# ucuapps/OpenGlue

Hardware: AMD Instinct MI355X
Metric: image-pairs/sec (1024 kpts, 256-dim, 9 GNN layers) (higher is better)
Workload: dtype f32; 1 GPU; BASELINE configs[1]: 1024x1024 kpts, 256-dim, 9 self+cross stages, 4 heads, 100 Sinkhorn iters, batch=32 pairs/GPU, random-init weights, seeded synthetic keypoints/descriptors; global_batch=32, pairs_per_gpu=32, parallelism=pairs sharded over 1 GPU(s), 1 RCCL gather

## Files before the change

include/openglue_amd.h:

```cpp
#ifndef OPENGLUE_AMD_H
#define OPENGLUE_AMD_H

#include <stddef.h>
#include <stdint.h>

#ifdef __cplusplus
extern "C" {
#endif

#define OG_ABI_VERSION 14

#define OG_E_INVALID   (-1)
#define OG_E_SHAPE     (-2)
#define OG_E_ALIGN     (-3)
#define OG_E_FLAG      (-4)
#define OG_E_RANGE     (-5)

#define OG_FLAG_RESIDUAL        1
#define OG_FLAG_USE_OFFSET      2
#define OG_FLAG_NO_DESCRIPTORS  4
#define OG_FLAG_LINEAR_ATTENTION 16
#define OG_FLAG_FAVOR_RELU      32
#define OG_FLAG_SIREN_ENCODER   8

// ... 79 lines not shown
    int64_t enc_w[OG_MAX_HIDDEN + 1], enc_b[OG_MAX_HIDDEN + 1];
    int64_t layer0, layer_stride, o_wqkv, o_bqkv, o_w0, o_b0, o_w3, o_b3;
    int64_t wp, bp, alpha, dustbin, total;
    int64_t o_scale;
    int64_t scales;
    int64_t o_wmlp;
    int64_t o_wqkvs;
    int64_t o_wqkvb;
} og_packed_layout_t;
int og_packed_layout(const og_shape* shape, og_packed_layout_t* layout);

int og_forward(const og_shape* shape, const og_inputs* in, const void* packed_dev,
               void* workspace_dev, const og_outputs* out, void* stream);

int og_forward_tap(const og_shape* shape, const og_inputs* in, const void* packed_dev, void* workspace_dev,
                   const og_outputs* out, void* stream, int32_t tap, float* tap_x);

int og_keypoint_encoder(const og_shape* shape, const og_inputs* in, const void* packed_dev, void* workspace_dev, float* x_out, void* stream);
int og_scores(const float* g0, const float* g1, int32_t batch, int32_t m, int32_t n, int32_t D, float* S, int64_t lds, void* stream);

#define OG_MAX_RAGGED 64
int og_forward_ragged(const og_shape* shape, const int32_t* lens0, const int32_t* lens1, const float* image0_wh,
                      const float* image1_wh, const og_inputs* in, const void* packed_dev, void* workspace_dev,
                      const og_outputs* out, void* stream);

#define OG_STAGE_ENCODER_INPUT 0
#define OG_STAGE_GEMM          1
#define OG_STAGE_ATTENTION     2
#define OG_STAGE_SINKHORN      3
#define OG_STAGE_MATCHES       4
#define OG_STAGE_GEMM_F16X3    5
#define OG_STAGE_MLP_FUSED     6
#define OG_NUM_STAGES          7
int og_forward_profiled(const og_shape* shape, const og_inputs* in, const void* packed_dev,
                        void* workspace_dev, const og_outputs* out, void* stream,
                        float* stage_ms , int32_t* stage_launches );
int og_forward_ragged_profiled(const og_shape* shape, const int32_t* lens0, const int32_t* lens1, const float* image0_wh,
                               const float* image1_wh, const og_inputs* in, const void* packed_dev, void* workspace_dev,
                               const og_outputs* out, void* stream, float* stage_ms, int32_t* stage_launches);


int og_gemm_nt(const float* A, int64_t lda, int64_t strideA, const float* B, int64_t ldb, int64_t strideB,
               float* C, int64_t ldc, int64_t strideC, int32_t M, int32_t N, int32_t K, int32_t batch,
               const float* bias, int32_t relu, const float* res, int64_t ldr, const float* alpha,
               float scale, void* stream);

int og_gemm_kmajor(const float* A, int64_t lda, int64_t strideA, int32_t a_kmajor, const float* B, int64_t ldb, int64_t strideB,
                   float* C, int64_t ldc, int64_t strideC, int32_t M, int32_t N, int32_t K, int32_t batch, int32_t k_total,
                   int32_t a_colsum, float scale, void* stream);

int og_split_f16(const float* x, int64_t n, void* hi, void* lo, void* stream);
int og_split_f16_hl(const float* x, int64_t rows, int32_t cols, int64_t ldx, void* out, int64_t ldo, void* stream);

int og_gemm_nt_f16x3(const void* A, int64_t lda, const void* B, int64_t ldb, int32_t M, int32_t N, int32_t K,
                     float scale, const float* bias, int32_t relu, const float* res, int64_t ldr, float* C32, int64_t ldc,
                     void* Ch, void* Cl, int64_t ldch, int32_t c_hl, void* stream);
int og_gemm_nt_f16x3_reshl(const void* A, int64_t lda, const void* B, int64_t ldb, int32_t M, int32_t N, int32_t K,
                           float scale, const float* bias, int32_t relu, const void* res_hl, int64_t ldrh, float* C32, int64_t ldc,
                           void* Ch, void* Cl, int64_t ldch, int32_t c_hl, void* stream);

size_t og_proj_block_stream_bytes(int32_t N, int32_t K);
int og_proj_block_pack(int32_t N, int32_t K, const float* W, void* stream_host);
int og_proj_block(const void* x_rows, int64_t ld, int32_t M, int32_t K, int32_t N, const void* stream_dev, const float* bias, const float* inv_scale_dev,
                  void* yh, void* yl, int64_t ldy, int32_t split_row, int32_t a0, int32_t a1, int32_t b0, int32_t b1, void* stream);

size_t og_mlp_block_stream_bytes(int32_t D);
int og_mlp_block_pack(int32_t D, const float* W0, const float* W3, void* stream_host);
int og_mlp_block(int32_t D, void* xo_rows, int64_t ld, int32_t M, const void* stream_dev, const float* b0, const float* b3,
                 void* stream);

int og_attention(const void* qh, const void* ql, int64_t ldq, const void* kh, const void* kl, int64_t ldk,
                 const void* vh, const void* vl, int64_t ldv, void* oh, void* ol, int64_t ldo, int32_t batch,
                 int32_t nq, int32_t nk, int32_t num_heads, int32_t dh, float* lse, void* stream);

size_t og_sinkhorn_workspace_bytes(int32_t batch, int32_t m, int32_t n);
int og_sinkhorn(const float* S, int64_t lds, float dustbin, int32_t batch, int32_t m, int32_t n,
                int32_t iters, float reg, float* scores, void* workspace_dev, void* stream);

int og_sinkhorn_status(const void* sinkhorn_workspace_dev, int32_t batch, int32_t m, int32_t n);
int og_sinkhorn_schedule(int32_t batch, int32_t m, int32_t n, int32_t iters);
int og_sinkhorn_schedule_ragged(int32_t batch, const int32_t* lens0, const int32_t* lens1, int32_t iters);
int og_sinkhorn_resident_geometry(int32_t m, int32_t n, int32_t* out4);
int og_sinkhorn_resident_rows_per_wave(int32_t batch, int32_t m, int32_t n);
int og_sinkhorn_resident_ragged_footprint(int32_t batch, const int32_t* lens0, const int32_t* lens1, int64_t* out2);
int og_forward_status(const og_shape* shape, const void* workspace_dev);

size_t og_sinkhorn_train_workspace_bytes(int32_t batch, int32_t m, int32_t n, int32_t iters);
int og_sinkhorn_train_forward(const float* S, int64_t lds, float dustbin, const float* dustbin_dev, int32_t batch, int32_t m, int32_t n,
                              int32_t iters, float reg, float* scores, void* train_workspace_dev, void* stream);
int og_sinkhorn_backward(const float* S, int64_t lds, float dustbin, const float* dustbin_dev, int32_t batch, int32_t m, int32_t n, int32_t iters,
                         float reg, const float* grad_scores, void* train_workspace_dev, float* dS, int64_t ldds,
                         float* d_dustbin, void* stream);

size_t og_batchnorm_train_workspace_bytes(int64_t rows, int32_t channels);
int og_batchnorm_train_forward(const float* x, int64_t ldx, int64_t rows, int32_t channels, const float* weight,
                               const float* bias, float eps, float momentum, float* running_mean, float* running_var,
                               float* y, int64_t ldy, float* save_mean, float* save_invstd, void* workspace_dev,
                               void* stream);

int og_batchnorm_train_backward(const float* a, int64_t lda, const float* dy, int64_t lddy, int64_t rows, int32_t channels,
                                const float* weight, const float* save_mean, const float* save_invstd, int32_t relu_mask,
                                float* dz, int64_t lddz, float* dweight, float* dbias, void* workspace_dev, void* stream);
int og_transpose_f32(const float* src, int64_t ld_src, int64_t rows, int32_t cols, float* dst, int64_t ld_dst, void* stream);
int og_colsum_f32(const float* x, int64_t ldx, int64_t rows, int32_t channels, float* out, void* workspace_dev, void* stream);

int og_transpose_f32_batched(const float* src, int64_t ld_src, int64_t stride_src, int64_t rows, int32_t cols, float* dst,
                             int64_t ld_dst, int64_t stride_dst, int32_t batch, void* stream);
int og_softmax_rows(float* S, int64_t ld, int64_t rows, int32_t cols, void* stream);
int og_softmax_rows_backward(const float* P, float* dP, int64_t ld, int64_t rows, int32_t cols, float scale, void* stream);

int og_attention_train_lse(const float* q, const float* k, int32_t batch, int32_t nq, int32_t nk, int32_t num_heads, int32_t dh,
                           float scale, float* lse, void* stream);
int og_attention_backward_parts(int32_t nk);
int og_attention_backward(const float* q, const float* k, const float* v, const float* dout, const float* lse, const float* delta,
                          int32_t batch, int32_t nq, int32_t nk, int32_t num_heads, int32_t dh, float scale, float* dq_part, float* dk,
                          float* dv, void* stream);
int og_attention_backward_ld(const float* q, int64_t ldq, const float* k, int64_t ldk, const float* v, int64_t ldv, const float* dout,
                             const float* lse, const float* delta, int32_t batch, int32_t nq, int32_t nk, int32_t num_heads, int32_t dh,
                             float scale, float* dq_part, float* dk, int64_t lddk, float* dv, int64_t lddv, void* stream);
int og_attention_delta(const float* dout, const float* out, int64_t rows, int32_t num_heads, int32_t dh, float* delta, void* stream);
int og_split_f16_rows(const float* x, int64_t ldx, int64_t rows, int32_t cols, int32_t scale_cols, float s1, float s2, void* hi, void* lo,
                      int64_t ldo, void* stream);
int og_merge_f16(const void* hi, const void* lo, int64_t n, float* out, void* stream);
int og_splitk_reduce(const float* part, int32_t parts, int32_t rows, int64_t ld, int32_t cols, float* dW, float* db, void* stream);

size_t og_matches_workspace_bytes(int32_t batch, int32_t m, int32_t n);
int og_extract_matches(const float* scores, int32_t batch, int32_t m, int32_t n, float match_threshold,
                       int64_t* matches0, float* matching_scores0, int64_t* matches1,
                       float* matching_scores1, void* workspace_dev, void* stream);


int og_prepare_features(const float* lafs, const float* responses, int64_t tokens, int32_t method, int32_t log_response,
                        float* keypoints, float* side_info, void* stream);

size_t og_compact_workspace_bytes(int32_t batch, int32_t m);
int og_compact_matches(const int64_t* matches0, const float* matching_scores0, const float* lafs0, const float* lafs1,
                       int32_t batch, int32_t m, int32_t n, int64_t* matching_idxs, int64_t* batch_indexes,
                       float* confidence, float* mlafs0, float* mlafs1, float* keypoints0, float* keypoints1,
                       int32_t* count_dev, void* workspace_dev, void* stream);


size_t og_gt_matches_workspace_bytes(int32_t batch, int32_t m, int32_t n);
int og_gt_matches(int32_t batch, int32_t m, int32_t n, const float* keypoints0, const float* keypoints1, int32_t transform,
                  const float* H, const float* K0, const float* K1, const float* R, const float* T,
                  const float* depth0, int32_t depth0_h, int32_t depth0_w, const float* depth1, int32_t depth1_h, int32_t depth1_w,
                  int32_t apply_thresholds, double positive_threshold, double negative_threshold,
                  int64_t* gt_matches0, int64_t* gt_matches1, int32_t* status_dev, void* workspace_dev, void* stream);

size_t og_criterion_workspace_bytes(int32_t batch, int32_t m, int32_t n, int32_t with_margin);
int og_criterion_forward(const float* scores, const int64_t* gt_matches0, const int64_t* gt_matches1,
                         const float* context_descriptors0, const float* context_descriptors1,
                         int32_t batch, int32_t m, int32_t n, int32_t D, int32_t with_margin, float margin,
                         float* losses, void* workspace_dev, void* stream);
int og_criterion_backward(const int64_t* gt_matches0, const int64_t* gt_matches1,
                          const float* context_descriptors0, const float* context_descriptors1,
                          int32_t batch, int32_t m, int32_t n, int32_t D, int32_t with_margin, float margin,
                          const float* grad_losses, const void* workspace_dev, float* grad_scores,
                          float* grad_context_descriptors0, float* grad_context_descriptors1, void* stream);

int og_epipolar_precision(int32_t batch, int32_t m, int32_t n, const float* keypoints0, const float* keypoints1,
                          const int64_t* matches0, const int32_t* num_keypoints0, const float* K0, const float* K1,
                          const float* R, const float* T, double threshold, float* precision, float* matching_score,
                          int32_t* num_correct, void* stream);
int og_essential_5pt(int32_t count, const double* x0, const double* x1, double* E, int32_t* num_solutions, void* stream);
size_t og_relative_pose_workspace_bytes(int32_t batch, int32_t m, int32_t hypotheses);
int og_relative_pose(int32_t batch, int32_t m, int32_t n, const float* keypoints0, const float* keypoints1,
                     const int64_t* matches0, const int32_t* num_keypoints0, const float* K0, const float* K1,
                     const float* R, const float* T, float ransac_threshold, int32_t hypotheses, uint64_t seed,
                     int64_t pair_offset, float* error, float* R_pred, float* t_pred, uint8_t* inliers,
                     int32_t* num_inliers, void* workspace_dev, void* stream);

int og_fundamental_7pt(int32_t count, const double* x0, const double* x1, double* F, int32_t* num_solutions, void* stream);
size_t og_fundamental_matrix_workspace_bytes(int32_t batch, int32_t m, int32_t hypotheses);
int og_fundamental_matrix(int32_t batch, int32_t m, int32_t n, const float* keypoints0, const float* keypoints1,
                          const int64_t* matches0, const int32_t* num_keypoints0, float threshold, int32_t hypotheses,
                          int32_t refine, uint64_t seed, int64_t pair_offset, double* F, uint8_t* inliers,
                          int32_t* num_inliers, int32_t* best_model, void* workspace_dev, void* stream);

size_t og_superpoint_packed_bytes(int32_t descriptor_dim);
int og_superpoint_pack(int32_t descriptor_dim, int32_t batch_norm, float bn_eps, const float* const* params, void* packed_host);
int og_superpoint_capacity(int32_t H, int32_t W, int32_t max_kpts);
size_t og_superpoint_workspace_bytes(int32_t batch, int32_t H, int32_t W, int32_t nms_kernel, int32_t max_kpts);
int og_superpoint_dense(int32_t batch, int32_t H, int32_t W, const float* image, const void* packed_dev, float* heatmap,
                        float* coarse_desc, void* workspace_dev, void* stream);
int og_superpoint_detect(int32_t batch, int32_t Hh, int32_t Wh, int32_t nms_kernel, int32_t border, float threshold, int32_t max_kpts,
                         const float* heatmap, int32_t* counts, int32_t* sel_idx, float* sel_score, int64_t sel_ld,
                         void* workspace_dev, void* stream);
int og_superpoint_describe(int32_t batch, int32_t Hc, int32_t Wc, int32_t n, const int32_t* sel_idx, const float* sel_score,
                           int64_t sel_ld, const float* coarse_desc, float* lafs, float* scores, float* descriptors, void* stream);

#define OG_ADAM_CHUNK         4096
#define OG_ADAM_NORM_CHUNK    8192
#define OG_ADAM_SCALARS       8
#define OG_ADAM_TOTAL_NORM    0
#define OG_ADAM_CLIP_COEF     1
#define OG_ADAM_STEP          2
#define OG_ADAM_LR            3
#define OG_ADAM_STEP_SIZE     4
#define OG_ADAM_INV_SQRT_BC2  5
typedef struct og_adam_layout_t {
    int64_t total;
    int64_t table_bytes;
    int64_t workspace_bytes;
    int32_t num_chunks;
    int32_t num_partials;
    int32_t chunk;
    int32_t reserved;
} og_adam_layout_t;
int og_adam_layout(int32_t count, const int64_t* numel, int64_t* offsets, int32_t* chunk_map, og_adam_layout_t* layout);
int og_adam_step(int32_t count, const void* const* params, const void* table_dev, const int32_t* chunk_map_dev, int32_t num_chunks,
                 int64_t total, float* grad, float* exp_avg, float* exp_avg_sq, double* workspace_dev, double lr, double gamma,
                 double beta1, double beta2, double eps, int32_t clip, double max_norm, void* stream);
// ... 30 lines not shown
```

openglue_amd/_lib.py:

```python
from __future__ import annotations

import ctypes as C
import os
from typing import Optional, Tuple

import torch

HERE = os.path.dirname(os.path.abspath(__file__))
LIB_PATH = os.environ.get("OPENGLUE_AMD_LIB") or os.path.join(HERE, "lib", "libopenglue_amd.so")

OG_ABI_VERSION = 14
OG_FLAG_RESIDUAL, OG_FLAG_USE_OFFSET, OG_FLAG_NO_DESCRIPTORS, OG_FLAG_SIREN_ENCODER, OG_FLAG_LINEAR_ATTENTION = 1, 2, 4, 8, 16
OG_FLAG_FAVOR_RELU = 32
OG_MAX_HIDDEN = 8
OG_MAX_RAGGED = 64
OG_ADAM_CHUNK, OG_ADAM_NORM_CHUNK, OG_ADAM_SCALARS = 4096, 8192, 8
OG_ADAM_TOTAL_NORM, OG_ADAM_CLIP_COEF, OG_ADAM_STEP, OG_ADAM_LR, OG_ADAM_STEP_SIZE, OG_ADAM_INV_SQRT_BC2 = range(6)
OG_STAGES = ("encoder_input", "gemm_f32", "attention", "sinkhorn", "matches", "gemm_f16x3", "mlp_fused")

_ERRORS = {-1: "OG_E_INVALID (null pointer / bad size)", -2: "OG_E_SHAPE (unsupported shape)",
           -3: "OG_E_ALIGN (pointer or leading dimension not 16-byte aligned)", -4: "OG_E_FLAG (unknown flag)",
           -5: "OG_E_RANGE (a folded weight is not finite)"}

c_float_p = C.POINTER(C.c_float)
# ... 21 lines not shown


class og_params(C.Structure):
    _fields_ = [("enc_conv", og_conv * (OG_MAX_HIDDEN + 1)), ("enc_bn", og_bn * OG_MAX_HIDDEN),
                ("layers", C.POINTER(og_layer_params)), ("linear_proj", og_conv), ("mix_coefs", C.c_void_p),
                ("dustbin_score", C.c_float)]


class og_inputs(C.Structure):
    _fields_ = [("keypoints0", C.c_void_p), ("keypoints1", C.c_void_p), ("descriptors0", C.c_void_p),
                ("descriptors1", C.c_void_p), ("side_info0", C.c_void_p), ("side_info1", C.c_void_p),
                ("image0_wh", C.c_float * 2), ("image1_wh", C.c_float * 2)]


class og_outputs(C.Structure):
    _fields_ = [("scores", C.c_void_p), ("context_descriptors0", C.c_void_p), ("context_descriptors1", C.c_void_p),
                ("matches0", C.c_void_p), ("matching_scores0", C.c_void_p), ("matches1", C.c_void_p),
                ("matching_scores1", C.c_void_p)]


class og_packed_layout_t(C.Structure):
    _fields_ = [("n_enc", C.c_int32), ("enc_k", C.c_int32 * (OG_MAX_HIDDEN + 1)), ("enc_out", C.c_int32 * (OG_MAX_HIDDEN + 1)),
                ("enc_w", C.c_int64 * (OG_MAX_HIDDEN + 1)), ("enc_b", C.c_int64 * (OG_MAX_HIDDEN + 1))] + \
               [(k, C.c_int64) for k in ("layer0", "layer_stride", "o_wqkv", "o_bqkv", "o_w0", "o_b0", "o_w3", "o_b3",
                                         "wp", "bp", "alpha", "dustbin", "total", "o_scale", "scales", "o_wmlp", "o_wqkvs", "o_wqkvb")]


class og_adam_layout_t(C.Structure):
    _fields_ = [("total", C.c_int64), ("table_bytes", C.c_int64), ("workspace_bytes", C.c_int64), ("num_chunks", C.c_int32),
                ("num_partials", C.c_int32), ("chunk", C.c_int32), ("reserved", C.c_int32)]


_i32, _i64, _f, _vp, _sz = C.c_int32, C.c_int64, C.c_float, C.c_void_p, C.c_size_t
SYMBOLS = {
    "og_abi_version": (C.c_int, []),
    "og_check_shape": (C.c_int, [C.POINTER(og_shape)]),
    "og_packed_weights_bytes": (_sz, [C.POINTER(og_shape)]),
    "og_workspace_bytes": (_sz, [C.POINTER(og_shape)]),
    "og_packed_layout": (C.c_int, [C.POINTER(og_shape), C.POINTER(og_packed_layout_t)]),
    "og_pack_weights": (C.c_int, [C.POINTER(og_shape), C.POINTER(og_params), _vp]),
    "og_forward": (C.c_int, [C.POINTER(og_shape), C.POINTER(og_inputs), _vp, _vp, C.POINTER(og_outputs), _vp]),
    "og_forward_tap": (C.c_int, [C.POINTER(og_shape), C.POINTER(og_inputs), _vp, _vp, C.POINTER(og_outputs), _vp, _i32, _vp]),
    "og_forward_ragged": (C.c_int, [C.POINTER(og_shape), C.POINTER(C.c_int32), C.POINTER(C.c_int32), C.POINTER(C.c_float),
                                    C.POINTER(C.c_float), C.POINTER(og_inputs), _vp, _vp, C.POINTER(og_outputs), _vp]),
    "og_forward_profiled": (C.c_int, [C.POINTER(og_shape), C.POINTER(og_inputs), _vp, _vp, C.POINTER(og_outputs), _vp,
                                      C.POINTER(C.c_float), C.POINTER(C.c_int32)]),
    "og_forward_ragged_profiled": (C.c_int, [C.POINTER(og_shape), C.POINTER(C.c_int32), C.POINTER(C.c_int32), C.POINTER(C.c_float),
                                             C.POINTER(C.c_float), C.POINTER(og_inputs), _vp, _vp, C.POINTER(og_outputs), _vp,
                                             C.POINTER(C.c_float), C.POINTER(C.c_int32)]),
    "og_gemm_nt": (C.c_int, [_vp, _i64, _i64, _vp, _i64, _i64, _vp, _i64, _i64, _i32, _i32, _i32, _i32, _vp, _i32,
                             _vp, _i64, _vp, _f, _vp]),
    "og_gemm_kmajor": (C.c_int, [_vp, _i64, _i64, _i32, _vp, _i64, _i64, _vp, _i64, _i64, _i32, _i32, _i32, _i32, _i32, _i32, _f, _vp]),
    "og_attention_train_lse": (C.c_int, [_vp, _vp, _i32, _i32, _i32, _i32, _i32, _f, _vp, _vp]),
    "og_attention_backward_parts": (C.c_int, [_i32]),
    "og_attention_backward": (C.c_int, [_vp, _vp, _vp, _vp, _vp, _vp, _i32, _i32, _i32, _i32, _i32, _f, _vp, _vp, _vp, _vp]),
    "og_attention_backward_ld": (C.c_int, [_vp, _i64, _vp, _i64, _vp, _i64, _vp, _vp, _vp, _i32, _i32, _i32, _i32, _i32, _f, _vp, _vp, _i64, _vp, _i64, _vp]),
    "og_attention_delta": (C.c_int, [_vp, _vp, _i64, _i32, _i32, _vp, _vp]),
    "og_split_f16_rows": (C.c_int, [_vp, _i64, _i64, _i32, _i32, _f, _f, _vp, _vp, _i64, _vp]),
    "og_merge_f16": (C.c_int, [_vp, _vp, _i64, _vp, _vp]),
    "og_splitk_reduce": (C.c_int, [_vp, _i32, _i32, _i64, _i32, _vp, _vp, _vp]),
    "og_split_f16": (C.c_int, [_vp, _i64, _vp, _vp, _vp]),
    "og_split_f16_hl": (C.c_int, [_vp, _i64, _i32, _i64, _vp, _i64, _vp]),
    "og_gemm_nt_f16x3": (C.c_int, [_vp, _i64, _vp, _i64, _i32, _i32, _i32, _f, _vp, _i32, _vp, _i64, _vp, _i64,
                                   _vp, _vp, _i64, _i32, _vp]),
    "og_gemm_nt_f16x3_reshl": (C.c_int, [_vp, _i64, _vp, _i64, _i32, _i32, _i32, _f, _vp, _i32, _vp, _i64, _vp, _i64,
                                         _vp, _vp, _i64, _i32, _vp]),
    "og_proj_block_stream_bytes": (_sz, [_i32, _i32]),
    "og_proj_block_pack": (C.c_int, [_i32, _i32, _vp, _vp]),
    "og_proj_block": (C.c_int, [_vp, _i64, _i32, _i32, _i32, _vp, _vp, _vp, _vp, _vp, _i64, _i32, _i32, _i32, _i32, _i32, _vp]),
    "og_mlp_block_stream_bytes": (_sz, [_i32]),
    "og_mlp_block_pack": (C.c_int, [_i32, _vp, _vp, _vp]),
    "og_mlp_block": (C.c_int, [_i32, _vp, _i64, _i32, _vp, _vp, _vp, _vp]),
    "og_attention": (C.c_int, [_vp, _vp, _i64, _vp, _vp, _i64, _vp, _vp, _i64, _vp, _vp, _i64, _i32, _i32, _i32, _i32,
                               _i32, _vp, _vp]),
    "og_keypoint_encoder": (C.c_int, [_vp, _vp, _vp, _vp, _vp, _vp]),
    "og_scores": (C.c_int, [_vp, _vp, _i32, _i32, _i32, _i32, _vp, _i64, _vp]),
    "og_sinkhorn_workspace_bytes": (_sz, [_i32, _i32, _i32]),
    "og_sinkhorn_status": (C.c_int, [_vp, _i32, _i32, _i32]),
    "og_sinkhorn_schedule": (C.c_int, [_i32, _i32, _i32, _i32]),
    "og_sinkhorn_schedule_ragged": (C.c_int, [_i32, _vp, _vp, _i32]),
    "og_sinkhorn_resident_geometry": (C.c_int, [_i32, _i32, _vp]),
    "og_sinkhorn_resident_ragged_footprint": (C.c_int, [_i32, _vp, _vp, _vp]),
    "og_sinkhorn_resident_rows_per_wave": (C.c_int, [_i32, _i32, _i32]),
    "og_forward_status": (C.c_int, [_vp, _vp]),
    "og_sinkhorn_train_workspace_bytes": (_sz, [_i32, _i32, _i32, _i32]),
    "og_sinkhorn_train_forward": (C.c_int, [_vp, _i64, _f, _vp, _i32, _i32, _i32, _i32, _f, _vp, _vp, _vp]),
    "og_sinkhorn_backward": (C.c_int, [_vp, _i64, _f, _vp, _i32, _i32, _i32, _i32, _f, _vp, _vp, _vp, _i64, _vp, _vp]),
    "og_batchnorm_train_workspace_bytes": (_sz, [_i64, _i32]),
    "og_batchnorm_train_forward": (C.c_int, [_vp, _i64, _i64, _i32, _vp, _vp, _f, _f, _vp, _vp, _vp, _i64, _vp, _vp, _vp, _vp]),
    "og_batchnorm_train_backward": (C.c_int, [_vp, _i64, _vp, _i64, _i64, _i32, _vp, _vp, _vp, _i32, _vp, _i64, _vp, _vp, _vp, _vp]),
    "og_transpose_f32": (C.c_int, [_vp, _i64, _i64, _i32, _vp, _i64, _vp]),
    "og_colsum_f32": (C.c_int, [_vp, _i64, _i64, _i32, _vp, _vp, _vp]),
    "og_transpose_f32_batched": (C.c_int, [_vp, _i64, _i64, _i64, _i32, _vp, _i64, _i64, _i32, _vp]),
    "og_softmax_rows": (C.c_int, [_vp, _i64, _i64, _i32, _vp]),
    "og_softmax_rows_backward": (C.c_int, [_vp, _vp, _i64, _i64, _i32, _f, _vp]),
    "og_sinkhorn": (C.c_int, [_vp, _i64, _f, _i32, _i32, _i32, _i32, _f, _vp, _vp, _vp]),
    "og_matches_workspace_bytes": (_sz, [_i32, _i32, _i32]),
    "og_prepare_features": (C.c_int, [_vp, _vp, _i64, _i32, _i32, _vp, _vp, _vp]),
    "og_compact_workspace_bytes": (_sz, [_i32, _i32]),
    "og_compact_matches": (C.c_int, [_vp, _vp, _vp, _vp, _i32, _i32, _i32, _vp, _vp, _vp, _vp, _vp, _vp, _vp, _vp, _vp, _vp]),
    "og_extract_matches": (C.c_int, [_vp, _i32, _i32, _i32, _f, _vp, _vp, _vp, _vp, _vp, _vp]),
    "og_gt_matches_workspace_bytes": (_sz, [_i32, _i32, _i32]),
    "og_gt_matches": (C.c_int, [_i32, _i32, _i32, _vp, _vp, _i32, _vp, _vp, _vp, _vp, _vp, _vp, _i32, _i32, _vp, _i32, _i32,
                                _i32, C.c_double, C.c_double, _vp, _vp, _vp, _vp, _vp]),
    "og_criterion_workspace_bytes": (_sz, [_i32, _i32, _i32, _i32]),
    "og_criterion_forward": (C.c_int, [_vp, _vp, _vp, _vp, _vp, _i32, _i32, _i32, _i32, _i32, _f, _vp, _vp, _vp]),
    "og_criterion_backward": (C.c_int, [_vp, _vp, _vp, _vp, _i32, _i32, _i32, _i32, _i32, _f, _vp, _vp, _vp, _vp, _vp, _vp]),
    "og_epipolar_precision": (C.c_int, [_i32, _i32, _i32, _vp, _vp, _vp, _vp, _vp, _vp, _vp, _vp, C.c_double, _vp, _vp, _vp, _vp]),
    "og_essential_5pt": (C.c_int, [_i32, _vp, _vp, _vp, _vp, _vp]),
    "og_relative_pose_workspace_bytes": (_sz, [_i32, _i32, _i32]),
    "og_relative_pose": (C.c_int, [_i32, _i32, _i32, _vp, _vp, _vp, _vp, _vp, _vp, _vp, _vp, _f, _i32, C.c_uint64, _i64,
                                   _vp, _vp, _vp, _vp, _vp, _vp, _vp]),
    "og_fundamental_7pt": (C.c_int, [_i32, _vp, _vp, _vp, _vp, _vp]),
    "og_fundamental_matrix_workspace_bytes": (_sz, [_i32, _i32, _i32]),
    "og_fundamental_matrix": (C.c_int, [_i32, _i32, _i32, _vp, _vp, _vp, _vp, _f, _i32, _i32, C.c_uint64, _i64,
                                        _vp, _vp, _vp, _vp, _vp, _vp]),
    "og_superpoint_packed_bytes": (_sz, [_i32]),
    "og_superpoint_pack": (C.c_int, [_i32, _i32, _f, _vp, _vp]),
    "og_superpoint_capacity": (C.c_int, [_i32, _i32, _i32]),
    "og_superpoint_workspace_bytes": (_sz, [_i32, _i32, _i32, _i32, _i32]),
    "og_superpoint_dense": (C.c_int, [_i32, _i32, _i32, _vp, _vp, _vp, _vp, _vp, _vp]),
    "og_superpoint_detect": (C.c_int, [_i32, _i32, _i32, _i32, _i32, _f, _i32, _vp, _vp, _vp, _vp, _i64, _vp, _vp]),
    "og_superpoint_describe": (C.c_int, [_i32, _i32, _i32, _i32, _vp, _vp, _i64, _vp, _vp, _vp, _vp, _vp]),
    "og_sift_geometry": (C.c_int, [_i32, _i32, C.POINTER(C.c_int32)]),
    "og_sift_workspace_bytes": (_sz, [_i32, _i32, _i32]),
    "og_sift_pyramid": (C.c_int, [_i32, _i32, _i32, _vp, _vp, _vp, _vp, _vp]),
    "og_sift_detect": (C.c_int, [_i32, _i32, _i32, _vp, _vp, _vp, _vp, _vp, _vp]),
    "og_sift_orient": (C.c_int, [_i32, _i32, _i32, _i32, _vp, _vp, _vp, _vp, _vp, _vp, _vp, _vp]),
    "og_sift_describe": (C.c_int, [_i32, _i32, _i32, _i32, _i32, _vp, _vp, _vp, _vp, _vp, _vp]),
    "og_sift_select": (C.c_int, [_i32, _i32, _i32, _f, _i32, _vp, _vp, _vp, _vp, _vp, _vp]),
    "og_sift_gather": (C.c_int, [_i32, _i32, _i32, _i32, _vp, _vp, _vp, _vp, _vp, _vp, _vp]),
    "og_patch_geometry": (C.c_int, [_i32, _i32, C.POINTER(C.c_int32)]),
    "og_patch_workspace_bytes": (_sz, [_i32, _i32, _i32, _i32]),
    "og_patch_pyramid": (C.c_int, [_i32, _i32, _i32, _vp, _vp, _vp, _vp]),
    "og_patch_extract": (C.c_int, [_i32, _i32, _i32, _i32, _vp, _vp, _i32, _i32, _vp, _vp]),
    "og_patchnet_packed_bytes": (_sz, [_i32]),
    "og_patchnet_pack": (C.c_int, [_i32, _f, _vp, _vp]),
    "og_patchnet_forward": (C.c_int, [_i32, _i32, _vp, _i32, _vp, _vp, _vp, _vp, _vp]),
    "og_adam_layout": (C.c_int, [_i32, C.POINTER(C.c_int64), C.POINTER(C.c_int64), C.POINTER(C.c_int32), C.POINTER(og_adam_layout_t)]),
    "og_adam_step": (C.c_int, [_i32, C.POINTER(C.c_void_p), _vp, _vp, _i32, _i64, _vp, _vp, _vp, _vp, C.c_double, C.c_double, C.c_double,
                               C.c_double, C.c_double, _i32, C.c_double, _vp]),
}

_lib: Optional[C.CDLL] = None


def load() -> C.CDLL:
    global _lib
    if _lib is not None:
        return _lib
    if not os.path.exists(LIB_PATH):
        raise RuntimeError(
            f"{LIB_PATH} not found: build it with `python -m openglue_amd.build` "
            "(hipcc --offload-arch=gfx950).  openglue_amd has no CPU / eager fallback.")
    lib = C.CDLL(LIB_PATH)
    for name, (restype, argtypes) in SYMBOLS.items():
        fn = getattr(lib, name)
        fn.restype, fn.argtypes = restype, argtypes
    if lib.og_abi_version() != OG_ABI_VERSION:
        raise RuntimeError(f"libopenglue_amd ABI {lib.og_abi_version()} != binding {OG_ABI_VERSION}; rebuild")
    _lib = lib
    return lib


def check(rc: int, what: str) -> None:
    if rc == 0:
        return
    if rc < 0:
        raise RuntimeError(f"{what}: {_ERRORS.get(rc, rc)}")
    raise RuntimeError(f"{what}: HIP error {rc} at kernel launch")


STREAM = object()


def call(name: str, dev: torch.device, *args) -> None:
    fn = getattr(load(), name)
    with torch.cuda.device(dev):
        stream = torch.cuda.current_stream(dev).cuda_stream
# ... 22 lines not shown
```

openglue_amd/csrc/api.hip:

```cpp
#include <math.h>
#include <cmath>
#include <stdlib.h>
#include <string.h>
#include <vector>
#include <dlfcn.h>
#include <stdio.h>

#include "og_common.h"

namespace {

constexpr double BN_EPS = 1e-5;

struct PackedLayout {
    int n_enc;
    int enc_k[OG_MAX_HIDDEN + 1];
    int enc_out[OG_MAX_HIDDEN + 1];
    int64_t enc_w[OG_MAX_HIDDEN + 1], enc_b[OG_MAX_HIDDEN + 1];
    int64_t enc_whl;
    int64_t layer0, layer_stride;
    int64_t o_wqkv, o_bqkv, o_w0, o_b0, o_w3, o_b3;
    int64_t o_wmlp;
    int64_t o_wqkvs;
    int64_t o_wqkvb;
// ... 368 lines not shown
    }
};
struct Range {
    static const Roctx& rt() { static const Roctx r; return r; }
    bool on;
    explicit Range(const char* name) : on(rt().push != nullptr) { if (on) rt().push(name); }
    Range(const char* name, int idx) : on(rt().push != nullptr) {
        if (on) { char buf[48]; snprintf(buf, sizeof buf, "%s %d", name, idx); rt().push(buf); }
    }
    ~Range() { if (on) rt().pop(); }
    Range(const Range&) = delete;
};
struct Scope {
    Profiler* p; int i;
    Scope(Profiler* pp, int c) : p(pp), i(pp ? pp->begin(c) : -1) {}
    ~Scope() { if (p) p->end(i); }
};

int forward_impl(const og_shape* shape, const og_inputs* in, const void* packed_dev, void* workspace_dev,
                 const og_outputs* outp, void* stream, Profiler* prof, const RaggedDesc* rag = nullptr,
                 const EncoderRagged* er0 = nullptr, const EncoderRagged* er1 = nullptr, int tap = -1, float* tap_x = nullptr,
                 bool encoder_only = false) {
    static const og_outputs no_outputs{};
    if (encoder_only && !outp) outp = &no_outputs;
    if (!shape || !in || !packed_dev || !workspace_dev || !outp) return OG_E_INVALID;
    if (int e = check_shape(shape)) return e;
    og_clear_status();
    const og_shape& s = *shape;
    if (!in->keypoints0 || !in->keypoints1 || !in->descriptors0 || !in->descriptors1 || (!outp->scores && !encoder_only)) return OG_E_INVALID;
    if (s.side_info > 0 && (!in->side_info0 || !in->side_info1)) return OG_E_INVALID;
    if ((outp->matches0 == nullptr) != (outp->matching_scores0 == nullptr)) return OG_E_INVALID;
    if ((outp->matches1 == nullptr) != (outp->matching_scores1 == nullptr)) return OG_E_INVALID;
    if (outp->matches1 && !outp->matches0) return OG_E_INVALID;
    if (((uintptr_t)packed_dev & 15) || ((uintptr_t)workspace_dev & 15) || ((uintptr_t)in->descriptors0 & 15) ||
        ((uintptr_t)in->descriptors1 & 15))
        return OG_E_ALIGN;
    hipStream_t st = (hipStream_t)stream;
    const PackedLayout L = packed_layout(s);
    const WorkspaceLayout W = workspace_layout(s);
    const float* pk = (const float*)packed_dev;
    float* ws = (float*)workspace_dev;
    const int D = s.desc_dim, D2 = 2 * D, B = s.batch, m = s.m, n = s.n;
    const bool favor = s.flags & OG_FLAG_FAVOR_RELU;
    const int WQ = qk_width(s), QW = qkv_width(s);
    const int64_t T0 = rag ? rag->off0[B] : (int64_t)B * m, T1 = rag ? rag->off1[B] : (int64_t)B * n, T = T0 + T1;
    float* X32 = ws + W.x32; float* G = ws + W.g; float* Sb = ws + W.sbuf;
    const int D4 = 4 * D;
    _Float16* XO = (_Float16*)(ws + W.xo);
    _Float16* QKVh = (_Float16*)(ws + W.qkvh); _Float16* QKVl = (_Float16*)(ws + W.qkvl);
    _Float16* Hb = (_Float16*)(ws + W.h);
    int rc;

    auto gemm = [&](const float* A, int64_t lda, const float* Bm, int64_t ldb, float* C, int64_t ldc, int64_t M, int N, int K,
                    const float* bias, int relu, const float* res, int64_t ldr, _Float16* Chl, int64_t ldch) -> int {
        GemmArgs g{};
        g.A = A; g.lda = lda; g.strideA = 0; g.B = Bm; g.ldb = ldb; g.strideB = 0; g.C = C; g.ldc = ldc; g.strideC = 0;
        g.M = (int)M; g.N = N; g.K = K; g.batch = 1; g.bias = bias; g.relu = relu; g.res = res; g.ldr = ldr; g.strideR = 0;
        g.alpha = nullptr; g.scale = 1.f; g.Ct = nullptr; g.ldct = 0; g.strideCt = 0; g.ct_rows = 1;
        g.Ch = Chl; g.Cl = Chl ? Chl + 32 : nullptr; g.ldch = ldch; g.c_hl = 1;
        Scope sc(prof, OG_STAGE_GEMM);
        return og_launch_gemm(g, st);
    };
    auto gemmh = [&](const _Float16* A, const float* wbase, int64_t o_w, int64_t wrow0, int64_t M, int N, int K,
                     const float* bias, int relu, const _Float16* res_hl, float* C32, _Float16* Ch, _Float16* Cl, int64_t ldch,
                     int c_hl) -> int {
        GemmHArgs g{};
        g.scale_dev = wbase + L.o_scale + (o_w == L.o_wqkv ? 0 : o_w == L.o_w0 ? 1 : 2);
        g.A = A; g.lda = D4;
        g.B = (const _Float16*)(wbase + o_w) + wrow0 * 2 * K; g.ldb = 2 * K;
        g.M = (int)M; g.N = N; g.K = K; g.scale = (float)(1.0 / OG_W_SCALE); g.bias = bias; g.relu = relu; g.res = nullptr; g.ldr = D; g.res_hl = res_hl; g.ldrh = D4;
        g.C32 = C32; g.ldc = D; g.Ch = Ch; g.Cl = Cl; g.ldch = ldch; g.c_hl = c_hl;
        Scope sc(prof, OG_STAGE_GEMM_F16X3);
        return og_launch_gemm_f16x3(g, st);
    };

    Range r_forward("og_forward");
    {
        Range r_stage("encoder");
        float* EI = ws + W.ei;
        float* Ea = ws + W.ea;
        float* Eb = ws + W.eb;
        {
            Scope sc(prof, OG_STAGE_ENCODER_INPUT);
            if ((rc = og_launch_encoder_input(in->keypoints0, in->side_info0, T0, s.side_info, in->image0_wh[0], in->image0_wh[1], EI, st, er0))) return rc;
            if ((rc = og_launch_encoder_input(in->keypoints1, in->side_info1, T1, s.side_info, in->image1_wh[0], in->image1_wh[1], EI + T0 * 32, st, er1))) return rc;
        }
        const float* cur = EI; int64_t ldcur = 32;
        const bool tail_f16 = L.enc_whl >= 0;
        const int last = L.n_enc - 1;
        _Float16* Ehl = (_Float16*)G;
        for (int i = 0; i < L.n_enc; ++i) {
            const float* Wi = pk + L.enc_w[i]; const float* bi = pk + L.enc_b[i];
            if (i < last) {
                float* dst = (i & 1) ? Eb : Ea;
                const int act = (s.flags & OG_FLAG_SIREN_ENCODER) ? 2 : 1;
                const bool to_hl = tail_f16 && i == last - 1;
                if ((rc = gemm(cur, ldcur, Wi, L.enc_k[i], to_hl ? nullptr : dst, L.enc_maxw, T, L.enc_out[i], L.enc_k[i], bi, act, nullptr, 0,
                               to_hl ? Ehl : nullptr, to_hl ? 2 * L.enc_out[i] : 0))) return rc;
                cur = dst; ldcur = L.enc_maxw;
            } else {
                const bool nd = s.flags & OG_FLAG_NO_DESCRIPTORS;
                const float* res[2] = {nd ? nullptr : in->descriptors0, nd ? nullptr : in->descriptors1};
                const int64_t r0[2] = {0, T0}, R[2] = {T0, T1};
                for (int side = 0; side < 2; ++side) {
                    if (tail_f16) {
                        const int K = L.enc_k[i];
                        GemmHArgs g{};
                        g.A = Ehl + r0[side] * 2 * K; g.lda = 2 * K;
                        g.B = (const _Float16*)(pk + L.enc_whl); g.ldb = 2 * K;
                        g.M = (int)R[side]; g.N = D; g.K = K; g.scale = (float)(1.0 / OG_W_SCALE); g.scale_dev = pk + L.scales + 1; g.bias = bi; g.relu = 0;
                        g.res = res[side]; g.ldr = D; g.res_hl = nullptr; g.ldrh = 0;
                        g.C32 = nullptr; g.ldc = D; g.Ch = XO + r0[side] * D4; g.Cl = g.Ch + 32; g.ldch = D4; g.c_hl = 1;
                        Scope sc(prof, OG_STAGE_GEMM_F16X3);
                        if ((rc = og_launch_gemm_f16x3(g, st))) return rc;
                    } else {
                        if ((rc = gemm(cur + r0[side] * ldcur, ldcur, Wi, L.enc_k[i], X32 + r0[side] * D, D, R[side], D, L.enc_k[i], bi, 0, res[side], D,
                                       XO + r0[side] * D4, D4))) return rc;
                    }
                }
            }
        }
    }

    auto tap_here = [&](int idx) -> int {
        if (tap != idx || !tap_x) return 0;
        return og_launch_merge_f16_hl(XO, T, D, D4, tap_x, D, st);
    };
    if ((rc = tap_here(0))) return rc;
    if (encoder_only) return og_launch_status();

    const int dh = D / s.num_heads;
    if (hipMemsetAsync(ws + W.attn, 0, OG_ATTN_COUNTERS * sizeof(int), st) != hipSuccess) return OG_E_INVALID;
    auto attention = [&](int nz, int split, int64_t qb0, int64_t qs0, int nq0, int64_t kb0, int64_t ks0, int nk0,
                         int64_t qb1, int64_t qs1, int nq1, int64_t kb1, int64_t ks1, int nk1, int rag_mode) -> int {
        AttnArgs a{};
        a.rag = rag; a.rag_mode = rag_mode;
        a.qh = QKVh; a.ql = QKVl; a.ldq = QW; a.kh = QKVh + WQ; a.kl = QKVl + WQ; a.ldk = QW;
        a.vh = QKVh + 2 * WQ; a.vl = QKVl + 2 * WQ; a.ldv = QW;
        a.feat = favor ? WQ : 0;
        a.oh = XO + D2; a.ol = XO + D2 + 32; a.ldo = D4; a.o_hl = 1;
        a.nz = nz; a.num_heads = s.num_heads; a.dh = dh; a.split = split;
        a.counters = reinterpret_cast<int*>(ws + W.attn); a.partial = ws + W.attn + OG_ATTN_COUNTERS;
        a.q_base[0] = qb0; a.q_step[0] = qs0; a.nq[0] = nq0; a.kv_base[0] = kb0; a.kv_step[0] = ks0; a.nk[0] = nk0;
        a.q_base[1] = qb1; a.q_step[1] = qs1; a.nq[1] = nq1; a.kv_base[1] = kb1; a.kv_step[1] = ks1; a.nk[1] = nk1;
        Scope sc(prof, OG_STAGE_ATTENTION);
        if (favor) return og_launch_favor_attention(a, st);
        return (s.flags & OG_FLAG_LINEAR_ATTENTION) ? og_launch_linear_attention(a, st) : og_launch_attention(a, st);
    };
    auto proj_small_ok = [&](int64_t R) {
        static const int mode = [] { const char* e = getenv("OG_PROJ_SMALL"); return e ? atoi(e) : -1; }();
        return L.o_wqkvs >= 0 && !favor && (mode >= 0 ? mode != 0 : R <= 8192) && R < ((int64_t)1 << 30);
    };
    auto proj_small = [&](const float* lw, int64_t r0, int64_t R, int split_row, int a0, int a1, int b0, int b1) -> int {
        Scope sc(prof, OG_STAGE_GEMM_F16X3);
        return og_launch_proj_small(XO + r0 * D4, D4, (int)R, D, (const char*)(lw + L.o_wqkvs), lw + L.o_bqkv, lw + L.o_scale,
                                    QKVh + r0 * QW, QKVl + r0 * QW, QW, split_row, a0, a1, b0, b1, st);
    };
    auto proj_stream_ok = [&](int64_t R, bool full = false) {
        return L.o_wqkvb >= 0 && !favor && og_proj_stream_wanted((int)(R < ((int64_t)1 << 30) ? R : 0), D, full) && R < ((int64_t)1 << 30) && QW % 64 == 0 &&
               !(((uintptr_t)QKVh | (uintptr_t)QKVl) & 127);
    };
    auto proj_stream = [&](const float* lw, int64_t r0, int64_t R, int split_row, int a0, int a1, int b0, int b1) -> int {
        Scope sc(prof, OG_STAGE_GEMM_F16X3);
        return og_launch_proj_stream(XO + r0 * D4, D4, (int)R, D, (const char*)(lw + L.o_wqkvb), lw + L.o_bqkv, lw + L.o_scale,
                                     QKVh + r0 * QW, QKVl + r0 * QW, QW, split_row, a0 / 128, a1 / 128, b0 / 128, b1 / 128, st);
    };
    auto qkv_proj = [&](const float* lw, int64_t r0, int64_t R, int c0, int c1) -> int {
        if (proj_small_ok(R) && c0 % 32 == 0 && c1 % 32 == 0) return proj_small(lw, r0, R, 0, 0, 0, c0 / 32, c1 / 32);
        if (proj_stream_ok(R, c0 == 0 && c1 == QW) && c0 % 128 == 0 && c1 % 128 == 0 && ((r0 * QW * 2) % 128 == 0)) return proj_stream(lw, r0, R, 0, 0, 0, c0, c1);
        const int cut = favor ? 2 * WQ : c1;
        const int ca[2] = {c0, c0 < cut && cut < c1 ? cut : c1}, cb[2] = {ca[1], c1};
        for (int part = 0; part < 2; ++part) {
            const int a0 = part ? cb[0] : ca[0], a1 = part ? cb[1] : ca[1];
            if (a1 <= a0) continue;
            const int relu = favor && a0 < 2 * WQ;
            if (int e = gemmh(XO + r0 * D4, lw, L.o_wqkv, a0, R, a1 - a0, D, lw + L.o_bqkv + a0, relu, nullptr, nullptr, QKVh + r0 * QW + a0,
                              QKVl + r0 * QW + a0, QW, 0)) return e;
        }
        return 0;
    };
    const bool fused_mlp = og_mlp_fused_enabled(D) && L.o_wmlp >= 0;
    auto mlp = [&](const float* lw, int64_t r0, int64_t R) -> int {
        if (fused_mlp) {
            MlpFusedArgs a{};
            a.XO = XO + r0 * D4; a.ld = D4; a.M = (int)R; a.wstream = (const char*)(lw + L.o_wmlp);
            a.b0 = lw + L.o_b0; a.b3 = lw + L.o_b3; a.scale = (float)(1.0 / OG_W_SCALE); a.scales_dev = lw + L.o_scale + 1;
            Scope sc(prof, OG_STAGE_MLP_FUSED);
            return og_launch_mlp_fused(a, D, st);
        }
        int e = gemmh(XO + r0 * D4, lw, L.o_w0, 0, R, D2, D2, lw + L.o_b0, 1, nullptr, nullptr, Hb + r0 * D4, nullptr, D4, 1);
        if (e) return e;
        return gemmh(Hb + r0 * D4, lw, L.o_w3, 0, R, D, D2, lw + L.o_b3, 0, XO + r0 * D4, nullptr, XO + r0 * D4, nullptr, D4, 1);
    };
    for (int l = 0; l < s.num_stages; ++l) {
        const float* lw = pk + L.layer0 + (int64_t)(2 * l) * L.layer_stride;
        {
            Range r_stage("gnn self", l);
            if ((rc = qkv_proj(lw, 0, T, 0, QW))) return rc;
            if ((rc = attention(2 * B, B, 0, m, m, 0, m, m, T0, n, n, T0, n, n, 1))) return rc;
            if ((rc = mlp(lw, 0, T))) return rc;
        }
        if ((rc = tap_here(2 * l + 1))) return rc;
        lw = pk + L.layer0 + (int64_t)(2 * l + 1) * L.layer_stride;
        Range r_stage("gnn cross", l);
        for (int side = 0; side < 2; ++side) {
            const int64_t qr0 = side ? T0 : 0, qR = side ? T1 : T0;
            if (side == 0) {
                GemmHArgs g{};
                g.A = XO; g.lda = D4; g.B = (const _Float16*)(lw + L.o_wqkv); g.ldb = 2 * D;
                g.M = (int)T; g.N = QW; g.K = D; g.scale = (float)(1.0 / OG_W_SCALE); g.scale_dev = lw + L.o_scale; g.bias = lw + L.o_bqkv;
                g.Ch = QKVh; g.Cl = QKVl; g.ldch = QW; g.c_hl = 0; g.ldc = D; g.ldr = D; g.ldrh = D4;
                g.split_row = (int)T0; g.split_n = WQ;
                if (proj_small_ok(T) && T0 % 32 == 0 && WQ % 32 == 0) {
                    if ((rc = proj_small(lw, 0, T, (int)T0, 0, WQ / 32, 0, QW / 32))) return rc;
                } else if (proj_stream_ok(T) && T0 % 128 == 0 && WQ % 128 == 0) {
                    if ((rc = proj_stream(lw, 0, T, (int)T0, 0, WQ, 0, QW))) return rc;
                } else if (!favor && !rag && T < (int64_t)1 << 30 && og_gemm_f16x3_row_split_ok(g)) {
                    Scope sc(prof, OG_STAGE_GEMM_F16X3);
                    if ((rc = og_launch_gemm_f16x3(g, st))) return rc;
                } else {
                    if ((rc = qkv_proj(lw, T0, T1, 0, QW))) return rc;
                    if ((rc = qkv_proj(lw, 0, T0, 0, WQ))) return rc;
                }
            } else {
                if ((rc = qkv_proj(lw, 0, T0, WQ, QW))) return rc;
            }
            if (side == 0) rc = attention(B, B, 0, m, m, T0, n, n, 0, 0, 0, 0, 0, 0, 2);
            else rc = attention(B, B, T0, n, n, 0, m, m, 0, 0, 0, 0, 0, 0, 3);
            if (rc) return rc;
            if ((rc = mlp(lw, qr0, qR))) return rc;
        }
        if ((rc = tap_here(2 * l + 2))) return rc;
    }

    _Float16* Gh = (_Float16*)G;
    for (int side = 0; side < 2; ++side) {
        Range r_stage("final_proj", side);
        const int64_t r0 = side ? T0 : 0, R = side ? T1 : T0;
        const bool resid = s.flags & OG_FLAG_RESIDUAL;
        GemmHArgs g{};
        g.A = XO + r0 * D4; g.lda = D4; g.B = (const _Float16*)(pk + L.wp); g.ldb = D2;
        g.M = (int)R; g.N = D; g.K = D; g.scale = (float)(1.0 / OG_W_SCALE); g.scale_dev = pk + L.scales; g.bias = pk + L.bp; g.relu = 0;
        g.res = resid ? (side ? in->descriptors1 : in->descriptors0) : nullptr; g.ldr = D;
        g.alpha = resid ? pk + L.alpha : nullptr;
        g.Ch = Gh + r0 * D2; g.Cl = g.Ch + 32; g.ldch = D2; g.c_hl = 1;
        g.Ct = side ? outp->context_descriptors1 : outp->context_descriptors0;
        g.ct_rows = side ? n : m; g.ldct = g.ct_rows;
        if (rag && g.Ct) { g.rag = rag; g.ct_rag = side ? 2 : 1; }
        Scope sc(prof, OG_STAGE_GEMM_F16X3);
        if ((rc = og_launch_gemm_f16x3(g, st))) return rc;
    }

    {
        GemmHArgs g{};
        g.A = Gh; g.lda = D2; g.strideA = (int64_t)m * D2; g.B = Gh + T0 * D2; g.ldb = D2; g.strideB = (int64_t)n * D2;
        g.C32 = Sb; g.ldc = W.lds; g.strideC32 = (int64_t)m * W.lds; g.M = m; g.N = n; g.K = D; g.batch = B;
        g.scale = (float)pow((double)D, -0.5);
        g.rag = rag;
        if (rag) g.B = Gh;
        Range r_stage("scores");
        Scope sc(prof, OG_STAGE_GEMM_F16X3);
        if (B > 1 || rag) rc = og_launch_gemm_f16x3(g, st);
        else { g.batch = 0; rc = og_launch_gemm_f16x3(g, st); }
        if (rc) return rc;
    }

    {
        Range r_stage("sinkhorn");
        Scope sc(prof, OG_STAGE_SINKHORN);
        RowBest rb{nullptr, nullptr, 0};
        if (outp->matches0) rb = og_matches_row_best(ws + W.match, B, m, n);
        if ((rc = og_launch_sinkhorn(Sb, W.lds, pk + L.dustbin, 0.f, B, m, n, s.sinkhorn_iters, s.sinkhorn_reg, outp->scores,
                                     ws + W.sink, st, rag, outp->matches0 ? &rb : nullptr))) return rc;
    }

    if (outp->matches0) {
        Range r_stage("matches");
        Scope sc(prof, OG_STAGE_MATCHES);
        if ((rc = og_launch_matches(outp->scores, B, m, n, s.match_threshold, outp->matches0, outp->matching_scores0,
                                    outp->matches1, outp->matching_scores1, ws + W.match, st, rag, true))) return rc;
    }
    return 0;
}

}

extern "C" int og_forward(const og_shape* shape, const og_inputs* in, const void* packed_dev, void* workspace_dev,
                          const og_outputs* outp, void* stream) {
    return forward_impl(shape, in, packed_dev, workspace_dev, outp, stream, nullptr);
}

extern "C" int og_forward_ragged(const og_shape* shape, const int32_t* lens0, const int32_t* lens1, const float* image0_wh,
                                 const float* image1_wh, const og_inputs* in, const void* packed_dev, void* workspace_dev,
                                 const og_outputs* outp, void* stream);

extern "C" int og_forward_tap(const og_shape* shape, const og_inputs* in, const void* packed_dev, void* workspace_dev,
                              const og_outputs* outp, void* stream, int32_t tap, float* tap_x) {
    if (!shape || tap < 0 || tap > 2 * shape->num_stages || !tap_x || ((uintptr_t)tap_x & 15)) return OG_E_INVALID;
    return forward_impl(shape, in, packed_dev, workspace_dev, outp, stream, nullptr, nullptr, nullptr, nullptr, tap, tap_x);
}

extern "C" int og_keypoint_encoder(const og_shape* shape, const og_inputs* in, const void* packed_dev, void* workspace_dev, float* x_out,
                                   void* stream) {
    if (!shape || !x_out || ((uintptr_t)x_out & 15)) return OG_E_INVALID;
    return forward_impl(shape, in, packed_dev, workspace_dev, nullptr, stream, nullptr, nullptr, nullptr, nullptr, 0, x_out, true);
}

extern "C" int og_scores(const float* g0, const float* g1, int32_t batch, int32_t m, int32_t n, int32_t D, float* S, int64_t lds, void* stream) {
    if (!g0 || !g1 || !S || batch <= 0 || m <= 0 || n <= 0 || D <= 0) return OG_E_INVALID;
    if ((D & 3) || lds < n || (lds & 3)) return OG_E_SHAPE;
    return og_gemm_nt(g0, D, (int64_t)m * D, g1, D, (int64_t)n * D, S, lds, (int64_t)m * lds, m, n, D, batch, nullptr, 0, nullptr, 0, nullptr,
                      (float)pow((double)D, -0.5), stream);
// ... 75 lines not shown
```

openglue_amd/csrc/attention.hip:

```cpp
#include <atomic>
#include <cstdlib>
#include <type_traits>

#include "og_common.h"

namespace {

typedef short s16x4 __attribute__((__vector_size__(4 * sizeof(short))));
typedef __attribute__((address_space(3))) s16x4 og_lds_s16x4;
typedef __attribute__((address_space(3))) void og_lds_void;
typedef __attribute__((address_space(1))) const void og_glb_void;

constexpr int KV_TILE = 64;
constexpr int Q_TILE = 128;
constexpr float RESCALE_THR = 11.f;
#ifndef OG_ATTN_SUMLIMIT
#define OG_ATTN_SUMLIMIT 32768.f
#endif
constexpr float SUM_LIMIT = OG_ATTN_SUMLIMIT;

#ifndef OG_ATTN_PKSUM
#define OG_ATTN_PKSUM 0
#endif
#ifndef OG_ATTN_MAXFIRST
// ... 1630 lines not shown
            static_for<48>([&](auto M) { behind(std::integral_constant<int, 48 + decltype(M)::value>{}); });
#pragma unroll
            for (int i = 0; i < 4; ++i) asm volatile("" : "=v"(sn[i][0]), "=v"(sn[i][1]));
        }
        if (has_soft) {
            if (moved) {
#pragma unroll
                for (int tt = 0; tt < 4; ++tt)
#pragma unroll
                    for (int r = 0; r < 4; ++r) { oacc[tt][0][r] *= alpha[0]; oacc[tt][1][r] *= alpha[1]; }
            }
            l_run[0] = l_run[0] * alpha[0] + (psum[0][0] + psum[0][1]);
            l_run[1] = l_run[1] * alpha[1] + (psum[1][0] + psum[1][1]);
        }
        if (t < ntiles) {
            set_v_slot(vslot_off(vslot_next));
            static_for<8>([&](auto Q) { read_v(std::integral_constant<int, 0>{}, Q); });
            fence();
            vslot_cur = vslot_next;
            asm volatile("s_waitcnt vmcnt(0)" ::: "memory");
            __syncthreads();
        }
    };

    qk_alone(0, sB, 0);
    {
        const float mt0 = row_max(sB, 0), mt1 = row_max(sB, 1);
        m_run[0] = mt0; m_run[1] = mt1;
#pragma unroll
        for (int i = 0; i < 4; ++i)
#pragma unroll
            for (int r = 0; r < 4; ++r) { sB[i][0][r] -= mt0; sB[i][1][r] -= mt1; }
        exp_split_all(sB, pfA, plA, l_run);
    }
    if (ntiles > 1) {
        __syncthreads();
        if (ntiles > 2) static_for<NPI>([&](auto I) { dma(2, I, std::integral_constant<int, 0>{}, 0); });
        qk_alone(2 * PLANE, sA, 1);
    }
    set_v_slot(vslot_off(0));
    static_for<8>([&](auto Q) { read_v(std::integral_constant<int, 0>{}, Q); });
    fence();
    if (ntiles > 1) {
        asm volatile("s_waitcnt vmcnt(0)" ::: "memory");
        __syncthreads();
    }
    int t = 1;
    for (; t + 1 <= ntiles; t += 2) {
        step(t, sA, pfA, plA, sB, pfB, plB);
        step(t + 1, sB, pfB, plB, sA, pfA, plA);
    }
    if (t <= ntiles) step(t, sA, pfA, plA, sB, pfB, plB);

#pragma unroll
    for (int j = 0; j < 2; ++j) {
        const float l_tot = sum_over_groups(l_run[j]);
        const float inv = 1.f / l_tot;
        const int qi = q0 + wave * 32 + 16 * j + c16;
        if (a.lse && g == 0 && qi < nq) a.lse[((int64_t)z * a.num_heads + h) * nq + qi] = (m_run[j] + __builtin_amdgcn_logf(l_tot)) * 0.6931471805599453f;
        if (qi < nq) {
            const int64_t orow = (q_row0 + qi) * a.ldo;
#pragma unroll
            for (int tt = 0; tt < 4; ++tt) {
                const int dv = 16 * tt + 4 * g;
                f16x4 vh, vl;
#pragma unroll
                for (int e = 0; e < 4; ++e) {
                    float o = oacc[tt][j][e] * inv;
                    asm("" : "+v"(o));
                    _Float16 th, tl;
                    og_split(o, th, tl);
                    vh[e] = th; vl[e] = tl;
                }
                const int64_t oo = orow + (a.o_hl ? og_hl_col(h * DH + dv) : (int64_t)(h * DH + dv));
                *reinterpret_cast<f16x4*>(a.oh + oo) = vh;
                *reinterpret_cast<f16x4*>(a.ol + oo) = vl;
            }
        }
    }
}

}

int og_launch_attention(const AttnArgs& a, hipStream_t stream) {
    if (!a.qh || !a.ql || !a.kh || !a.kl || !a.vh || !a.vl || !a.oh || !a.ol || a.nz <= 0 || a.num_heads <= 0) return OG_E_INVALID;
    if ((a.ldq & 7) || (a.ldk & 7) || (a.ldv & 7) || (a.ldo & 3)) return OG_E_ALIGN;
    const void* ps[8] = {a.qh, a.ql, a.kh, a.kl, a.vh, a.vl, a.oh, a.ol};
    for (int i = 0; i < 8; ++i)
        if ((uintptr_t)ps[i] & 15) return OG_E_ALIGN;
    int nqmax = 0;
    for (int g = 0; g < 2; ++g) {
        const bool used = g == 0 ? a.split > 0 : a.split < a.nz;
        if (!used) continue;
        if (a.nq[g] <= 0 || a.nk[g] <= 0) return OG_E_INVALID;
        if (a.nq[g] > nqmax) nqmax = a.nq[g];
    }
    AttnArgs a2 = a;
    a2.qtiles = (nqmax + Q_TILE - 1) / Q_TILE;
    RaggedDesc rd;
    rd.B = 0;
    if (a.rag) rd = *a.rag;
    a2.rag = nullptr;
    static const bool dma_on = [] { const char* e = getenv("OG_ATTN_DMA"); return !(e && e[0] == '0'); }();
    const bool dma = dma_on && (a.dh == 64 || a.dh == 32);
    const int groups8 = (a.nz * a.num_heads + 7) / 8 * 8;
    dim3 grid(groups8 * a2.qtiles), block(256);
    static const int ks_mode = [] { const char* e = getenv("OG_ATTN_KSPLIT"); return e ? atoi(e) : -1; }();
    int nkmin = 1 << 30;
    for (int g = 0; g < 2; ++g) {
        const bool used = g == 0 ? a.split > 0 : a.split < a.nz;
        if (used && a.nk[g] < nkmin) nkmin = a.nk[g];
    }
    static const int gs_mode = [] { const char* e = getenv("OG_ATTN_GSPLIT"); return e ? atoi(e) : -1; }();
    int gs = 1;
    if (!a.mx && dma && (a.dh == 64 || a.dh == 32) && a.partial && a.counters && (int)grid.x <= OG_ATTN_COUNTERS) {
        static const int maxwg_env = [] { const char* e = getenv("OG_ATTN_GS_MAXWG"); return e ? atoi(e) : 0; }();
        const int maxwg = maxwg_env > 0 ? maxwg_env : (a.dh == 32 ? 512 : 256);
        if (gs_mode >= 0) gs = gs_mode == 2 || gs_mode == 4 ? gs_mode : 1;
        else if ((int)grid.x * 4 <= maxwg && (a.rag || nkmin >= 16 * KV_TILE)) gs = 4;
        else if ((int)grid.x * 2 <= maxwg && (a.rag || nkmin >= 8 * KV_TILE)) gs = 2;
        if ((int)grid.x * gs > maxwg && gs_mode < 0) gs = 1;
        if ((int64_t)grid.x * gs * 4 * 34 * 64 > OG_ATTN_PARTIAL_FLOATS) gs = 1;
    }
    if (gs > 1) {
        dim3 g2(grid.x * gs);
        const char* const sc = getenv("OG_ATTN_GS_SCATTER");
        a2.gs_scatter = sc && sc[0] == '1' ? 1 : 0;
        if (a.dh == 64) {
            if (a.rag) {
                if (gs == 4) hipLaunchKernelGGL((attention_dma_kernel<64, RaggedDesc, 1, 4>), g2, block, 0, stream, a2, rd);
                else hipLaunchKernelGGL((attention_dma_kernel<64, RaggedDesc, 1, 2>), g2, block, 0, stream, a2, rd);
            } else {
                if (gs == 4) hipLaunchKernelGGL((attention_dma_kernel<64, RaggedNone, 1, 4>), g2, block, 0, stream, a2, RaggedNone{});
                else hipLaunchKernelGGL((attention_dma_kernel<64, RaggedNone, 1, 2>), g2, block, 0, stream, a2, RaggedNone{});
            }
        } else {
            if (a.rag) {
                if (gs == 4) hipLaunchKernelGGL((attention_dma_kernel<32, RaggedDesc, 1, 4>), g2, block, 0, stream, a2, rd);
                else hipLaunchKernelGGL((attention_dma_kernel<32, RaggedDesc, 1, 2>), g2, block, 0, stream, a2, rd);
            } else {
                if (gs == 4) hipLaunchKernelGGL((attention_dma_kernel<32, RaggedNone, 1, 4>), g2, block, 0, stream, a2, RaggedNone{});
                else hipLaunchKernelGGL((attention_dma_kernel<32, RaggedNone, 1, 2>), g2, block, 0, stream, a2, RaggedNone{});
            }
        }
        return og_launch_status();
    }
    const bool ksplit = !a.mx && dma && a.dh == 64 && (ks_mode >= 0 ? ks_mode != 0 : ((int)grid.x <= 256 && (a.rag || nkmin >= 4 * KV_TILE)));
    if (ksplit) {
        if (a.rag) hipLaunchKernelGGL((attention_dma_kernel<64, RaggedDesc, 2>), grid, dim3(512), 0, stream, a2, rd);
        else hipLaunchKernelGGL((attention_dma_kernel<64, RaggedNone, 2>), grid, dim3(512), 0, stream, a2, RaggedNone{});
        return og_launch_status();
    }
    if (a.mx) {
        if (!dma) return OG_E_SHAPE;
        const int e = 127 + a.mx_sv - 11;
        a2.mx_scale_a = e | (e << 8) | (e << 16) | (e << 24);
        if (a.rag) {
            if (a.dh == 64) hipLaunchKernelGGL((attention_dma_kernel<64, RaggedDesc, 1, 1, 1>), grid, block, 0, stream, a2, rd);
            else hipLaunchKernelGGL((attention_dma_kernel<32, RaggedDesc, 1, 1, 1>), grid, block, 0, stream, a2, rd);
        } else {
            if (a.dh == 64) hipLaunchKernelGGL((attention_dma_kernel<64, RaggedNone, 1, 1, 1>), grid, block, 0, stream, a2, RaggedNone{});
            else hipLaunchKernelGGL((attention_dma_kernel<32, RaggedNone, 1, 1, 1>), grid, block, 0, stream, a2, RaggedNone{});
        }
        return og_launch_status();
    }
    static const int p16_mode = [] { const char* e = getenv("OG_ATTN_P16"); return e ? atoi(e) : -1; }();
    if (dma && a.dh == 64 && (p16_mode >= 0 ? p16_mode != 0 : false)) {
        if (a.rag) hipLaunchKernelGGL((attention_p16_kernel<RaggedDesc>), grid, block, 0, stream, a2, rd);
        else hipLaunchKernelGGL((attention_p16_kernel<RaggedNone>), grid, block, 0, stream, a2, RaggedNone{});
        return og_launch_status();
    }
    static const int pipe_mode = [] { const char* e = getenv("OG_ATTN_PIPE"); return e ? atoi(e) : -1; }();
    const bool pipe = dma && (pipe_mode >= 0 ? pipe_mode != 0 : false);
#ifndef OG_ATTN_PIPE8
#define OG_ATTN_PIPE8 0
#endif
#if OG_ATTN_PIPE8
    if (pipe && pipe_mode == 2 && a.dh == 64) {
        a2.qtiles = (nqmax + 2 * Q_TILE - 1) / (2 * Q_TILE);
        dim3 grid8(groups8 * a2.qtiles);
        if (a.rag) hipLaunchKernelGGL((attention_dma_kernel<64, RaggedDesc, 1, 1, 0, 2>), grid8, dim3(512), 0, stream, a2, rd);
        else hipLaunchKernelGGL((attention_dma_kernel<64, RaggedNone, 1, 1, 0, 2>), grid8, dim3(512), 0, stream, a2, RaggedNone{});
        return og_launch_status();
    }
#endif
    if (pipe) {
        if (a.rag) {
            if (a.dh == 64) hipLaunchKernelGGL((attention_dma_kernel<64, RaggedDesc, 1, 1, 0, 1>), grid, block, 0, stream, a2, rd);
            else hipLaunchKernelGGL((attention_dma_kernel<32, RaggedDesc, 1, 1, 0, 1>), grid, block, 0, stream, a2, rd);
        } else {
            if (a.dh == 64) hipLaunchKernelGGL((attention_dma_kernel<64, RaggedNone, 1, 1, 0, 1>), grid, block, 0, stream, a2, RaggedNone{});
            else hipLaunchKernelGGL((attention_dma_kernel<32, RaggedNone, 1, 1, 0, 1>), grid, block, 0, stream, a2, RaggedNone{});
        }
        return og_launch_status();
    }
    if (a.rag) {
        switch (a.dh) {
            case 16: hipLaunchKernelGGL((attention_kernel<16, RaggedDesc>), grid, block, 0, stream, a2, rd); break;
            case 128: hipLaunchKernelGGL((attention_kernel<128, RaggedDesc>), grid, block, 0, stream, a2, rd); break;
            case 32:
                if (dma) hipLaunchKernelGGL((attention_dma_kernel<32, RaggedDesc>), grid, block, 0, stream, a2, rd);
                else hipLaunchKernelGGL((attention_kernel<32, RaggedDesc>), grid, block, 0, stream, a2, rd);
                break;
            case 64:
                if (dma) hipLaunchKernelGGL((attention_dma_kernel<64, RaggedDesc>), grid, block, 0, stream, a2, rd);
                else hipLaunchKernelGGL((attention_kernel<64, RaggedDesc>), grid, block, 0, stream, a2, rd);
                break;
            default: return OG_E_SHAPE;
        }
    } else {
        switch (a.dh) {
            case 16: hipLaunchKernelGGL((attention_kernel<16, RaggedNone>), grid, block, 0, stream, a2, RaggedNone{}); break;
            case 128: hipLaunchKernelGGL((attention_kernel<128, RaggedNone>), grid, block, 0, stream, a2, RaggedNone{}); break;
            case 32:
                if (dma) hipLaunchKernelGGL((attention_dma_kernel<32, RaggedNone>), grid, block, 0, stream, a2, RaggedNone{});
                else hipLaunchKernelGGL((attention_kernel<32, RaggedNone>), grid, block, 0, stream, a2, RaggedNone{});
                break;
            case 64:
                if (dma) hipLaunchKernelGGL((attention_dma_kernel<64, RaggedNone>), grid, block, 0, stream, a2, RaggedNone{});
                else hipLaunchKernelGGL((attention_kernel<64, RaggedNone>), grid, block, 0, stream, a2, RaggedNone{});
                break;
            default: return OG_E_SHAPE;
        }
    }
    return og_launch_status();
}

#if OG_ATTN_TRACE
extern "C" int og_debug_attn_trace(void* host_dst, size_t bytes) {
    if (bytes > sizeof(og_attn_trace_buf)) bytes = sizeof(og_attn_trace_buf);
    return (int)hipMemcpyFromSymbol(host_dst, HIP_SYMBOL(og_attn_trace_buf), bytes);
}
#endif

extern "C" int og_attention(const void* qh, const void* ql, int64_t ldq, const void* kh, const void* kl, int64_t ldk,
                            const void* vh, const void* vl, int64_t ldv, void* oh, void* ol, int64_t ldo, int32_t batch,
                            int32_t nq, int32_t nk, int32_t num_heads, int32_t dh, float* lse, void* stream) {
    og_clear_status();
    AttnArgs a{};
    a.lse = lse;
    a.qh = (const _Float16*)qh; a.ql = (const _Float16*)ql; a.ldq = ldq;
    a.kh = (const _Float16*)kh; a.kl = (const _Float16*)kl; a.ldk = ldk;
    a.vh = (const _Float16*)vh; a.vl = (const _Float16*)vl; a.ldv = ldv;
    a.oh = (_Float16*)oh; a.ol = (_Float16*)ol; a.ldo = ldo; a.o_hl = 0;
    a.nz = batch; a.num_heads = num_heads; a.dh = dh; a.split = batch;
    a.q_base[0] = 0; a.q_step[0] = nq; a.kv_base[0] = 0; a.kv_step[0] = nk;
    a.nq[0] = nq; a.nk[0] = nk;
    a.q_base[1] = a.q_step[1] = a.kv_base[1] = a.kv_step[1] = 0; a.nq[1] = a.nk[1] = 0;
    if (const char* e = getenv("OG_ATTN_MX_SV")) { a.mx = 1; a.mx_sv = atoi(e); }
    return og_launch_attention(a, (hipStream_t)stream);
}
```

openglue_amd/csrc/matches.hip:

```cpp
#include "og_common.h"

namespace {

struct MatchWs {
    int* idx0;
    float* max0;
    unsigned long long* colbest;
};

static MatchWs mw_layout(void* ws, int B, int m, int n) {
    MatchWs w{};
    char* p = (char*)ws;
    w.colbest = (unsigned long long*)p; p += sizeof(unsigned long long) * (size_t)B * n;
    w.idx0 = (int*)p; p += sizeof(int) * (size_t)B * m;
    w.max0 = (float*)p;
    return w;
}

__device__ __forceinline__ unsigned int orderable(float v) {
    const unsigned int b = __float_as_uint(v);
    return (b & 0x80000000u) ? ~b : (b | 0x80000000u);
}
__device__ __forceinline__ float unorderable(unsigned int k) {
    return __uint_as_float((k & 0x80000000u) ? (k & 0x7FFFFFFFu) : ~k);
}

template <class RD>
__global__ __launch_bounds__(256) void row_argmax_kernel(const float* __restrict__ scores, int M, int N,
                                                         int* __restrict__ idx0, float* __restrict__ max0, RD rd) {
    const int b = blockIdx.y;
    const int row = blockIdx.x * 4 + (threadIdx.x >> 6);
    const int lane = threadIdx.x & 63;
    const int Mmax = M;
    int64_t so = (int64_t)b * (M + 1) * (N + 1);
    if (rd.B > 0) { M = rd.off0[b + 1] - rd.off0[b]; N = rd.off1[b + 1] - rd.off1[b]; so = rd.soff[b]; }
    if (row >= M) return;
    const float* sp = scores + so + (int64_t)row * (N + 1);
    float best = OG_NEG_INF;
    int bi = 0x7FFFFFFF;
    for (int j = lane; j < N; j += 64) {
        const float v = sp[j];
        if (v > best || bi == 0x7FFFFFFF) { best = v; bi = j; }
    }
#pragma unroll
    for (int o = 32; o > 0; o >>= 1) {
        const float ov = __shfl_xor(best, o, 64);
        const int oi = __shfl_xor(bi, o, 64);
        if (ov > best || (ov == best && oi < bi)) { best = ov; bi = oi; }
    }
    if (lane == 0) { idx0[(int64_t)b * Mmax + row] = bi; max0[(int64_t)b * Mmax + row] = best; }
}

template <class RD>
__global__ __launch_bounds__(256) void col_argmax_kernel(const float* __restrict__ scores, int M, int N,
                                                         unsigned long long* __restrict__ colbest, RD rd) {
    const int b = blockIdx.z;
    const int j = blockIdx.x * 256 + threadIdx.x;
    const int Nmax = N;
    int64_t so = (int64_t)b * (M + 1) * (N + 1);
    if (rd.B > 0) { M = rd.off0[b + 1] - rd.off0[b]; N = rd.off1[b + 1] - rd.off1[b]; so = rd.soff[b]; }
    const int i0 = blockIdx.y * 64;
    if (j >= N || i0 >= M) return;
    const int i1 = min(i0 + 64, M);
    const float* sp = scores + so + j;
    float best = sp[(int64_t)i0 * (N + 1)];
    int bi = i0;
    int i = i0 + 1;
    for (; i + 8 <= i1; i += 8) {
        float v[8];
#pragma unroll
        for (int k = 0; k < 8; ++k) v[k] = sp[(int64_t)(i + k) * (N + 1)];
#pragma unroll
        for (int k = 0; k < 8; ++k)
            if (v[k] > best) { best = v[k]; bi = i + k; }
    }
    for (; i < i1; ++i) {
        const float v = sp[(int64_t)i * (N + 1)];
        if (v > best) { best = v; bi = i; }
    }
    const unsigned long long key = ((unsigned long long)orderable(best) << 32) | (unsigned long long)(0xFFFFFFFFu - (unsigned)bi);
    atomicMax(colbest + (int64_t)b * Nmax + j, key);
}

template <class RD>
__global__ __launch_bounds__(256) void mutual_kernel(int M, int N, float thr, const int* __restrict__ idx0,
                                                     const float* __restrict__ max0,
                                                     const unsigned long long* __restrict__ colbest,
                                                     int64_t* __restrict__ matches0, float* __restrict__ ms0,
                                                     int64_t* __restrict__ matches1, float* __restrict__ ms1, RD rd) {
    const int b = blockIdx.y;
    const int t = blockIdx.x * 256 + threadIdx.x;
    const int Mmax = M, Nmax = N;
    int64_t o0 = (int64_t)b * M, o1 = (int64_t)b * N;
    if (rd.B > 0) { M = rd.off0[b + 1] - rd.off0[b]; N = rd.off1[b + 1] - rd.off1[b]; o0 = rd.off0[b]; o1 = rd.off1[b]; }
    if (t < M) {
        const int j = idx0[(int64_t)b * Mmax + t];
        const int i1 = (int)(0xFFFFFFFFu - (unsigned)(colbest[(int64_t)b * Nmax + j] & 0xFFFFFFFFull));
        const bool mutual = i1 == t;
        const float s = mutual ? expf(max0[(int64_t)b * Mmax + t]) : 0.f;
        const bool valid = mutual && s > thr;
        matches0[o0 + t] = valid ? (int64_t)j : (int64_t)-1;
        ms0[o0 + t] = s;
    }
    if (matches1 && t < N) {
        const int i = (int)(0xFFFFFFFFu - (unsigned)(colbest[(int64_t)b * Nmax + t] & 0xFFFFFFFFull));
        const bool mutual = idx0[(int64_t)b * Mmax + i] == t;
        const float s = mutual ? expf(max0[(int64_t)b * Mmax + i]) : 0.f;
        const bool valid = mutual && s > thr;
        matches1[o1 + t] = valid ? (int64_t)i : (int64_t)-1;
        ms1[o1 + t] = s;
    }
}

__global__ __launch_bounds__(256) void encoder_input_kernel(const float* __restrict__ kpts, const float* __restrict__ side,
                                                            int64_t tokens, int s, float wm1, float hm1,
                                                            float* __restrict__ out, EncoderRagged er) {
    const int64_t g = (int64_t)blockIdx.x * 256 + threadIdx.x;
    const int64_t t = g >> 3;
    const int c4 = (int)(g & 7) * 4;
    if (t >= tokens) return;
    if (er.B > 0) {
        int lo = 0, hi = er.B - 1;
        while (lo < hi) {
            const int mid = (lo + hi + 1) >> 1;
            if (er.off[mid] <= (int)t) lo = mid; else hi = mid - 1;
        }
        wm1 = er.wm1[lo]; hm1 = er.hm1[lo];
    }
    f32x4 o;
#pragma unroll
    for (int e = 0; e < 4; ++e) {
        const int c = c4 + e;
        float v = 0.f;
        if (c == 0) v = 2.f * kpts[2 * t] / wm1 - 1.f;
        else if (c == 1) v = 2.f * kpts[2 * t + 1] / hm1 - 1.f;
        else if (c < 2 + s) v = side[t * s + (c - 2)];
        o[e] = v;
    }
    *reinterpret_cast<f32x4*>(out + t * 32 + c4) = o;
}

}

extern "C" size_t og_matches_workspace_bytes(int32_t batch, int32_t m, int32_t n) {
    if (batch <= 0 || m <= 0 || n <= 0) return 0;
    return sizeof(unsigned long long) * (size_t)batch * n + (sizeof(int) + sizeof(float)) * (size_t)batch * m + 16;
}

namespace {
template <class RD>
int matches_run(const float* scores, int B, int m, int n, float thr, int64_t* matches0, float* ms0,
                int64_t* matches1, float* ms1, void* workspace, hipStream_t st, const RD& rd, bool rows_done) {
    if (!scores || !matches0 || !ms0 || !workspace || B <= 0 || m <= 0 || n <= 0) return OG_E_INVALID;
    if ((matches1 == nullptr) != (ms1 == nullptr)) return OG_E_INVALID;
    if ((uintptr_t)workspace & 15) return OG_E_ALIGN;
    const MatchWs w = mw_layout(workspace, B, m, n);
    hipError_t e = hipMemsetAsync(w.colbest, 0, sizeof(unsigned long long) * (size_t)B * n, st);
    if (e != hipSuccess) return (int)e;
    if (!rows_done) hipLaunchKernelGGL(row_argmax_kernel<RD>, dim3((m + 3) / 4, B), dim3(256), 0, st, scores, m, n, w.idx0, w.max0, rd);
    hipLaunchKernelGGL(col_argmax_kernel<RD>, dim3((n + 255) / 256, (m + 63) / 64, B), dim3(256), 0, st, scores, m, n, w.colbest, rd);
    const int mx = m > n ? m : n;
    hipLaunchKernelGGL(mutual_kernel<RD>, dim3((mx + 255) / 256, B), dim3(256), 0, st, m, n, thr, w.idx0, w.max0, w.colbest,
                       matches0, ms0, matches1, ms1, rd);
    return og_launch_status();
}
}

int og_launch_matches(const float* scores, int B, int m, int n, float thr, int64_t* matches0, float* ms0,
                      int64_t* matches1, float* ms1, void* workspace, hipStream_t st, const RaggedDesc* rag, bool rows_done) {
    if (rag) {
        if (rag->B != B) return OG_E_INVALID;
        return matches_run<RaggedDesc>(scores, B, m, n, thr, matches0, ms0, matches1, ms1, workspace, st, *rag, rows_done);
    }
    return matches_run<RaggedNone>(scores, B, m, n, thr, matches0, ms0, matches1, ms1, workspace, st, RaggedNone{}, rows_done);
}

RowBest og_matches_row_best(void* matches_workspace, int B, int m, int n) {
    const MatchWs w = mw_layout(matches_workspace, B, m, n);
    return RowBest{w.idx0, w.max0, m};
}

extern "C" int og_extract_matches(const float* scores, int32_t batch, int32_t m, int32_t n, float match_threshold,
                                  int64_t* matches0, float* matching_scores0, int64_t* matches1,
                                  float* matching_scores1, void* workspace_dev, void* stream) {
    og_clear_status();
    return og_launch_matches(scores, batch, m, n, match_threshold, matches0, matching_scores0, matches1,
                             matching_scores1, workspace_dev, (hipStream_t)stream, nullptr, false);
}

int og_launch_encoder_input(const float* kpts, const float* side, int64_t tokens, int s, float wx, float wy,
                            float* out, hipStream_t st, const EncoderRagged* er) {
    if (!kpts || !out || tokens <= 0 || s < 0 || 2 + s > 32 || (s > 0 && !side)) return OG_E_INVALID;
    const int64_t threads = tokens * 8;
    EncoderRagged e;
    e.B = 0;
    if (er) e = *er;
    hipLaunchKernelGGL(encoder_input_kernel, dim3((unsigned)((threads + 255) / 256)), dim3(256), 0, st, kpts, side, tokens,
                       s, wx - 1.f, wy - 1.f, out, e);
    return og_launch_status();
}
```

openglue_amd/csrc/og_common.h:

```cpp
#pragma once
#include <hip/hip_runtime.h>
#include <stdint.h>
#include "../../include/openglue_amd.h"

typedef float f32x4 __attribute__((ext_vector_type(4)));
typedef float f32x16 __attribute__((ext_vector_type(16)));
typedef _Float16 f16x4 __attribute__((ext_vector_type(4)));
typedef _Float16 f16x8 __attribute__((ext_vector_type(8)));

#define OG_WAVE 64
#define OG_NEG_INF (-__builtin_huge_valf())

__device__ __forceinline__ int mfma32_row(int r, int lane) { return (r & 3) + 8 * (r >> 2) + 4 * (lane >> 5); }

__device__ __forceinline__ float wave_max(float v) {
#pragma unroll
    for (int o = 32; o > 0; o >>= 1) v = fmaxf(v, __shfl_xor(v, o, 64));
    return v;
}
__device__ __forceinline__ float wave_sum(float v) {
#pragma unroll
    for (int o = 32; o > 0; o >>= 1) v += __shfl_xor(v, o, 64);
    return v;
}
// ... 81 lines not shown
    int ta, tb;
    int a_colsum;
    int ktot;
};
int og_launch_gemm(const GemmArgs& a, hipStream_t stream);

struct GemmHArgs {
    const _Float16* A; int64_t lda;
    const _Float16* B; int64_t ldb;
    int M, N, K;
    float scale;
    float inv_scale;
    const float* scale_dev;
    const float* bias; int relu;
    const float* res; int64_t ldr;
    const _Float16* res_hl; int64_t ldrh;
    float* C32; int64_t ldc;
    _Float16* Ch; _Float16* Cl; int64_t ldch;
    int c_hl;
    const float* alpha;
    float* Ct; int64_t ldct; int ct_rows;
    int ct_rag;
    int batch;
    int64_t strideA, strideB, strideC32;
    const RaggedDesc* rag;
    int split_row, split_n;
};
int og_launch_gemm_f16x3(const GemmHArgs& a, hipStream_t stream);
bool og_gemm_f16x3_row_split_ok(const GemmHArgs& a);
int og_launch_split_f16(const float* x, int64_t n, void* hi, void* lo, hipStream_t stream);
int og_launch_split_f16_hl(const float* x, int64_t rows, int cols, int64_t ldx, void* out, int64_t ldo, hipStream_t stream);
int og_launch_merge_f16_hl(const void* in, int64_t rows, int cols, int64_t ldi, float* out, int64_t ldo, hipStream_t stream);

struct MlpFusedArgs {
    _Float16* XO; int64_t ld;
    int M;
    const char* wstream;
    const float* b0;
    const float* b3;
    float scale;
    const float* scales_dev;
};
bool og_mlp_fused_supported(int D);
bool og_mlp_fused_enabled(int D);
size_t og_mlp_stream_bytes(int D);
bool og_pack_mlp_stream(int D, const double* W0, const double* W3, void* out, double S0 = OG_W_SCALE, double S3 = OG_W_SCALE);
int og_launch_mlp_fused(const MlpFusedArgs& a, int D, hipStream_t stream);
bool og_mlp_small_wanted(int M);
size_t og_proj_stream_bytes(int N, int K);
bool og_pack_proj_stream(int N, int K, const double* W, void* out, double S);
size_t og_proj_stream_big_bytes(int N, int K);
bool og_pack_proj_stream_big(int N, int K, const double* W, void* out, double S);
bool og_proj_stream_wanted(int M, int K, bool full);
int og_launch_proj_stream(const _Float16* X, int64_t ld, int M, int K, const char* wstream, const float* bias, const float* scale_dev,
                          _Float16* Ch, _Float16* Cl, int64_t ldc, int split_row, int a0, int a1, int b0, int b1, hipStream_t stream);
int og_launch_proj_small(const _Float16* X, int64_t ld, int M, int K, const char* wstream, const float* bias, const float* scale_dev,
                         _Float16* Ch, _Float16* Cl, int64_t ldc, int split_row, int a0, int a1, int b0, int b1, hipStream_t stream);

constexpr int OG_ATTN_COUNTERS = 256;
constexpr int64_t OG_ATTN_PARTIAL_FLOATS = (int64_t)512 * 4 * 34 * 64;
struct AttnArgs {
    const _Float16* qh; const _Float16* ql; int64_t ldq;
    const _Float16* kh; const _Float16* kl; int64_t ldk;
    const _Float16* vh; const _Float16* vl; int64_t ldv;
    _Float16* oh; _Float16* ol; int64_t ldo;
    int o_hl;
    int nz, num_heads, dh;
    int split;
    int64_t q_base[2], q_step[2], kv_base[2], kv_step[2];
    int nq[2], nk[2];
    int qtiles;
    const RaggedDesc* rag;
    int rag_mode;
    int feat;
    float* lse;
    float* partial;
    int* counters;
    int gs_scatter;
    int mx;
    int mx_scale_a;
    int mx_sv;
};
int og_launch_attention(const AttnArgs& a, hipStream_t stream);
int og_launch_linear_attention(const AttnArgs& a, hipStream_t stream);
int og_launch_favor_attention(const AttnArgs& a, hipStream_t stream);

struct RowBest { int* idx; float* val; int stride; };
int og_launch_sinkhorn(const float* S, int64_t lds, const float* dustbin_dev , float dustbin_host, int batch, int m, int n, int iters,
                       float reg, float* scores, void* workspace, hipStream_t stream, const RaggedDesc* rag = nullptr,
                       const RowBest* row_best = nullptr, bool trusted_padding = true);
bool og_sinkhorn_resident_shape_ok(int B, int m, int n);
size_t og_sinkhorn_resident_ws_bytes(int B, int m, int n);
bool og_sinkhorn_resident_wanted(int B, int m, int n, int mode);
int og_sinkhorn_resident_rounds(int B, int m, int n);
bool og_sinkhorn_resident_ragged_wanted(const RaggedDesc& rd, int mode);
int og_launch_sinkhorn_resident_ragged(const float* S, int64_t lds, const float* zdev, float zhost, const RaggedDesc& rd, int m_max, int n_max, int iters,
                                       float inv_reg, float* u, int ldu, const float* v_in, float* v_out, int ldv, void* xws, unsigned* status,
                                       hipStream_t st, bool trusted_padding = true, int* count_only = nullptr);
static inline bool og_sinkhorn_resident_ragged_wanted(const RaggedNone&, int) { return false; }
int og_launch_sinkhorn_resident(const float* S, int64_t lds, const float* zdev, float zhost, int B, int m, int n, int iters,
                                float inv_reg, float la, float la_bin, float lb, float lb_bin, float* u, int ldu, const float* v_in,
                                float* v_out, int ldv, void* xws, unsigned* status , hipStream_t st, bool trusted_padding = true);
int og_launch_matches(const float* scores, int batch, int m, int n, float thr, int64_t* matches0,
                      float* ms0, int64_t* matches1, float* ms1, void* workspace, hipStream_t stream,
                      const RaggedDesc* rag = nullptr, bool rows_done = false);
RowBest og_matches_row_best(void* matches_workspace, int batch, int m, int n);
struct EncoderRagged {
    int B;
    int off[OG_MAX_RAGGED + 1];
    float wm1[OG_MAX_RAGGED], hm1[OG_MAX_RAGGED];
};
int og_launch_encoder_input(const float* kpts, const float* side, int64_t tokens, int s, float wx, float wy,
                            float* out , hipStream_t stream, const EncoderRagged* er = nullptr);
```

openglue_amd/csrc/sinkhorn.hip:

```cpp
#include <stdlib.h>
#include <type_traits>

#include "og_common.h"

namespace {

constexpr int SK_ROWS = 32;

struct SinkhornGeom { int CPL, WPR; };
inline SinkhornGeom sk_geom(int n) {
    if (n <= 256) return {1, 1};
    if (n <= 512) return {2, 1};
    if (n <= 1024) return {4, 1};
    if (n <= 2048) return {4, 2};
    if (n <= 4096) return {4, 4};
    return {8, 4};
}

struct SinkhornWs {
    float* u;
    float* v[2];
    unsigned* flags;
    float* pm;
    float* ps;
    int ldu, ldv, ldp, RB;
};

static SinkhornWs sk_layout(void* ws, int B, int m, int n) {
    SinkhornWs w{};
    w.RB = (m + SK_ROWS - 1) / SK_ROWS;
    w.ldu = (int)og_round_up(m + 1, 4);
    w.ldv = (int)og_round_up(n + 1, 4);
    w.ldp = (int)og_round_up(n, 4);
    float* p = (float*)ws;
    w.u = p; p += (int64_t)B * w.ldu;
    w.v[0] = p; p += (int64_t)B * w.ldv;
    w.v[1] = p; p += (int64_t)B * w.ldv;
    w.flags = (unsigned*)p; p += 4;
    w.pm = p; p += (int64_t)B * w.RB * w.ldp;
    w.ps = p;
    return w;
}

__device__ __forceinline__ float block_max(float v, float* sm) {
    v = wave_max(v);
    if ((threadIdx.x & 63) == 0) sm[threadIdx.x >> 6] = v;
    __syncthreads();
    v = fmaxf(fmaxf(sm[0], sm[1]), fmaxf(sm[2], sm[3]));
    __syncthreads();
    return v;
}
__device__ __forceinline__ float block_sum(float v, float* sm) {
    v = wave_sum(v);
    if ((threadIdx.x & 63) == 0) sm[threadIdx.x >> 6] = v;
    __syncthreads();
    v = (sm[0] + sm[1]) + (sm[2] + sm[3]);
    __syncthreads();
    return v;
}

__device__ __forceinline__ float exp_rel(float a, float b) { return a == OG_NEG_INF ? 0.f : __expf(a - b); }

template <int CPL, int RG, int WPR, class RD>
__global__ __launch_bounds__(256) void sinkhorn_sweep_kernel(const float* __restrict__ S, int64_t lds, int M, int N,
                                                             const float* __restrict__ zdev, float zhost, float inv_reg,
                                                             float la, const float* __restrict__ v_in, int ldv,
                                                             float* __restrict__ u, int ldu, float* __restrict__ pm,
                                                             float* __restrict__ ps, int ldp, int RB, int64_t strideS,
                                                             RD rd) {
    constexpr int NRS = 4 / WPR;
    constexpr int RW = SK_ROWS / NRS;
    constexpr int NCW = 256 * CPL;
    constexpr int NCB = NCW * WPR;
    extern __shared__ __attribute__((aligned(16))) float sm[];
    float* xch = sm + NRS * 2 * NCB;

    const int b = blockIdx.y, rb = blockIdx.x;
    if (rd.B > 0) {
        M = rd.off0[b + 1] - rd.off0[b];
        N = rd.off1[b + 1] - rd.off1[b];
        if (rb * SK_ROWS >= M) return;
        la = -__logf((float)(M + N));
    }
    S += (int64_t)b * strideS;
    const int tid = threadIdx.x, lane = tid & 63, wave = tid >> 6;
    const int cp = wave % WPR, rs = wave / WPR;
    const int cbase = cp * NCW + 4 * lane;
    const float zr = (zdev ? zdev[0] : zhost) * inv_reg;
    const float* vb = v_in + (int64_t)b * ldv;
    const float dcol = zr + vb[N];

    float vv[CPL][4], cm[CPL][4], cs[CPL][4];
#pragma unroll
    for (int k = 0; k < CPL; ++k) {
        const int c0 = cbase + 256 * k;
        f32x4 t = {0.f, 0.f, 0.f, 0.f};
        if (c0 < N) t = *reinterpret_cast<const f32x4*>(vb + c0);
#pragma unroll
        for (int e = 0; e < 4; ++e) { vv[k][e] = t[e]; cm[k][e] = OG_NEG_INF; cs[k][e] = 0.f; }
    }

    const int srow0 = rb * SK_ROWS + rs * RW;
    int parity = 0;
    f32x4 nx[RG][CPL];
    auto fetch = [&](int row0) {
#pragma unroll
        for (int r = 0; r < RG; ++r) {
            const int row = row0 + r;
            const float* sp = S + (int64_t)row * lds;
#pragma unroll
            for (int k = 0; k < CPL; ++k) {
                const int c0 = cbase + 256 * k;
                if (row < M && c0 < N) nx[r][k] = *reinterpret_cast<const f32x4*>(sp + c0);
                else nx[r][k] = f32x4{OG_NEG_INF, OG_NEG_INF, OG_NEG_INF, OG_NEG_INF};
            }
        }
    };
    fetch(srow0);
#pragma unroll 1
    for (int g0 = 0; g0 < RW; g0 += RG) {
        const int row0 = srow0 + g0;
        float x[RG][CPL][4];
#pragma unroll
// ... 40 lines not shown
                for (int w = 0; w < WPR; ++w) st += xs[(r * WPR + w) * 2 + 1] * exp_rel(xs[(r * WPR + w) * 2], mt);
                ur[r] = la - (mt + __logf(st));
            }
            parity ^= 1;
        } else {
#pragma unroll
            for (int r = 0; r < RG; ++r) {
                const float mt = fmaxf(mx[r], dcol);
                const float st = sum[r] * exp_rel(mx[r], mt) + __expf(dcol - mt);
                ur[r] = la - (mt + __logf(st));
            }
        }
        if (cp == 0 && lane == 0) {
#pragma unroll
            for (int r = 0; r < RG; ++r)
                if (row0 + r < M) u[(int64_t)b * ldu + row0 + r] = ur[r];
        }
#pragma unroll
        for (int k = 0; k < CPL; ++k)
#pragma unroll
            for (int e = 0; e < 4; ++e) {
                float gm = cm[k][e];
#pragma unroll
                for (int r = 0; r < RG; ++r) gm = fmaxf(gm, x[r][k][e] + ur[r]);
                const float gs = gm == OG_NEG_INF ? 0.f : gm;
                float acc = cs[k][e] * exp_rel(cm[k][e], gs);
#pragma unroll
                for (int r = 0; r < RG; ++r) acc += __expf(x[r][k][e] + ur[r] - gs);
                cm[k][e] = gm; cs[k][e] = acc;
            }
    }

    float* pmb = pm + ((int64_t)b * RB + rb) * ldp;
    float* psb = ps + ((int64_t)b * RB + rb) * ldp;
    if (NRS == 1) {
#pragma unroll
        for (int k = 0; k < CPL; ++k) {
            const int c0 = cbase + 256 * k;
            if (c0 < N) {
                *reinterpret_cast<f32x4*>(pmb + c0) = f32x4{cm[k][0], cm[k][1], cm[k][2], cm[k][3]};
                *reinterpret_cast<f32x4*>(psb + c0) = f32x4{cs[k][0], cs[k][1], cs[k][2], cs[k][3]};
            }
        }
        return;
    }
    float* smm = sm + (size_t)rs * 2 * NCB;
#pragma unroll
    for (int k = 0; k < CPL; ++k) {
        const int c0 = cbase + 256 * k;
        *reinterpret_cast<f32x4*>(smm + c0) = f32x4{cm[k][0], cm[k][1], cm[k][2], cm[k][3]};
        *reinterpret_cast<f32x4*>(smm + NCB + c0) = f32x4{cs[k][0], cs[k][1], cs[k][2], cs[k][3]};
    }
    __syncthreads();
    for (int c0 = 4 * tid; c0 < N; c0 += 1024) {
        f32x4 wm[NRS], wsum[NRS];
#pragma unroll
        for (int w = 0; w < NRS; ++w) {
            wm[w] = *reinterpret_cast<const f32x4*>(sm + (size_t)w * 2 * NCB + c0);
            wsum[w] = *reinterpret_cast<const f32x4*>(sm + (size_t)w * 2 * NCB + NCB + c0);
        }
        f32x4 om, os;
#pragma unroll
        for (int e = 0; e < 4; ++e) {
            float mxe = wm[0][e];
#pragma unroll
            for (int w = 1; w < NRS; ++w) mxe = fmaxf(mxe, wm[w][e]);
            float acc = 0.f;
#pragma unroll
            for (int w = 0; w < NRS; ++w) acc += wsum[w][e] * exp_rel(wm[w][e], mxe);
            om[e] = mxe; os[e] = acc;
        }
        *reinterpret_cast<f32x4*>(pmb + c0) = om;
        *reinterpret_cast<f32x4*>(psb + c0) = os;
    }
}

template <class RD>
__global__ __launch_bounds__(256) void sinkhorn_combine_kernel(int M, int N, const float* __restrict__ zdev,
                                                               float zhost, float inv_reg, float la_bin, float lb,
                                                               float lb_bin, const float* __restrict__ v_in,
                                                               float* __restrict__ v_out, int ldv,
                                                               float* __restrict__ u, int ldu,
                                                               const float* __restrict__ pm,
                                                               const float* __restrict__ ps, int ldp, int RB, RD rd) {
    __shared__ float sm[4];
    const int b = blockIdx.y, tid = threadIdx.x;
    int RBv = RB;
    if (rd.B > 0) {
        M = rd.off0[b + 1] - rd.off0[b];
        N = rd.off1[b + 1] - rd.off1[b];
        if ((int)blockIdx.x * 256 > N) return;
        RBv = (M + SK_ROWS - 1) / SK_ROWS;
        const float norm = -__logf((float)(M + N));
        lb = norm; la_bin = norm + __logf((float)N); lb_bin = norm + __logf((float)M);
    }
    const float zr = (zdev ? zdev[0] : zhost) * inv_reg;
    const float* vb = v_in + (int64_t)b * ldv;
    float m = OG_NEG_INF;
    for (int j = tid; j <= N; j += 256) m = fmaxf(m, vb[j]);
    m = block_max(m, sm);
    float s = 0.f;
    for (int j = tid; j <= N; j += 256) s += __expf(vb[j] - m);
    s = block_sum(s, sm);
    const float uM = la_bin - (zr + m + __logf(s));
    if (blockIdx.x == 0 && tid == 0) u[(int64_t)b * ldu + M] = uM;

    const int j = blockIdx.x * 256 + tid;
    if (j < N) {
        const float* pmb = pm + (int64_t)b * RB * ldp + j;
        const float* psb = ps + (int64_t)b * RB * ldp + j;
        float cm = zr + uM;
        float cs = 1.f;
        for (int rb0 = 0; rb0 < RBv; rb0 += 8) {
            float pmv[8], psv[8];
#pragma unroll
            for (int q = 0; q < 8; ++q) {
                const bool ok = rb0 + q < RBv;
                pmv[q] = ok ? pmb[(int64_t)(rb0 + q) * ldp] : OG_NEG_INF;
                psv[q] = ok ? psb[(int64_t)(rb0 + q) * ldp] : 0.f;
            }
            float mx = cm;
#pragma unroll
            for (int q = 0; q < 8; ++q) mx = fmaxf(mx, pmv[q]);
            cs *= __expf(cm - mx);
#pragma unroll
            for (int q = 0; q < 8; ++q) cs += psv[q] * __expf(pmv[q] - mx);
            cm = mx;
        }
        v_out[(int64_t)b * ldv + j] = lb - (cm + __logf(cs));
    }
    if ((int)blockIdx.x == N / 256) {
        const float* ub = u + (int64_t)b * ldu;
        float um = uM;
        for (int i = tid; i < M; i += 256) um = fmaxf(um, ub[i]);
        um = block_max(um, sm);
        float us = 0.f;
        for (int i = tid; i < M; i += 256) us += __expf(ub[i] - um);
        us = block_sum(us, sm) + __expf(uM - um);
        if (tid == 0) v_out[(int64_t)b * ldv + N] = lb_bin - (zr + um + __logf(us));
    }
}

constexpr float LOG2E = 1.4426950408889634f;
constexpr float LN2 = 0.6931471805599453f;

template <int CPL, int RG, int WPR, class RD, int ROWS = SK_ROWS, bool NT = false>
__global__ __launch_bounds__(256) void sinkhorn_sweep_fast_kernel(const float* __restrict__ S, int64_t lds, int M, int N,
                                                                  const float* __restrict__ zdev, float zhost, float inv_reg,
                                                                  float la, const float* __restrict__ v_in, int ldv,
                                                                  float* __restrict__ u, int ldu, float* __restrict__ ps,
                                                                  int ldp, int RB, int64_t strideS, float in_scale,
                                                                  float out_scale, RD rd) {
    constexpr int rows = ROWS;
    constexpr int NRS = 4 / WPR;
    constexpr int RW = ROWS / NRS;
    constexpr int NCW = 256 * CPL;
    constexpr int NCB = NCW * WPR;
    extern __shared__ __attribute__((aligned(16))) float sm[];
    float* xch = sm + NRS * NCB;

    const int b = blockIdx.y, rb = blockIdx.x;
    if (rd.B > 0) {
        M = rd.off0[b + 1] - rd.off0[b];
        N = rd.off1[b + 1] - rd.off1[b];
        if (rb * rows >= M) return;
        la = -__logf((float)(M + N));
    }
    S += (int64_t)b * strideS;
    const int tid = threadIdx.x, lane = tid & 63, wave = tid >> 6;
    const int cp = wave % WPR, rs = wave / WPR;
    const int cbase = cp * NCW + 4 * lane;
    const float c2 = inv_reg * LOG2E;
    const float zr2 = (zdev ? zdev[0] : zhost) * c2;
    const float* vb = v_in + (int64_t)b * ldv;
    float* ub = u + (int64_t)b * ldu;
    const float dcol2 = zr2 + vb[N] * in_scale;
    const float la2 = la * LOG2E;

    float vv[CPL][4], cs[CPL][4];
#pragma unroll
    for (int k = 0; k < CPL; ++k) {
        const int c0 = cbase + 256 * k;
        f32x4 t = {0.f, 0.f, 0.f, 0.f};
        if (c0 < N) t = *reinterpret_cast<const f32x4*>(vb + c0);
#pragma unroll
        for (int e = 0; e < 4; ++e) { vv[k][e] = t[e] * in_scale; cs[k][e] = 0.f; }
    }

    const int srow0 = rb * rows + rs * RW;
    int parity = 0;
    f32x4 nx[RG][CPL];
    float nu[RG];
    auto fetch = [&](int row0) {
#pragma unroll
        for (int r = 0; r < RG; ++r) {
            const int row = row0 + r;
            const float* sp = S + (int64_t)row * lds;
            nu[r] = row < M ? ub[row] : 0.f;
#pragma unroll
            for (int k = 0; k < CPL; ++k) {
                const int c0 = cbase + 256 * k;
                if (row < M && c0 < N) nx[r][k] = NT ? __builtin_nontemporal_load(reinterpret_cast<const f32x4*>(sp + c0))
                                                     : *reinterpret_cast<const f32x4*>(sp + c0);
                else nx[r][k] = f32x4{OG_NEG_INF, OG_NEG_INF, OG_NEG_INF, OG_NEG_INF};
            }
        }
    };
    fetch(srow0);
#pragma unroll 1
    for (int g0 = 0; g0 < RW; g0 += RG) {
        const int row0 = srow0 + g0;
        float p[RG][CPL][4], uo[RG], sum[RG];
// ... 65 lines not shown
    }
    __syncthreads();
    for (int c0 = 4 * tid; c0 < N; c0 += 1024) {
        f32x4 acc = *reinterpret_cast<const f32x4*>(sm + c0);
#pragma unroll
        for (int w = 1; w < NRS; ++w) acc += *reinterpret_cast<const f32x4*>(sm + (size_t)w * NCB + c0);
        *reinterpret_cast<f32x4*>(psb + c0) = acc;
    }
}

template <class RD>
__global__ __launch_bounds__(256) void sinkhorn_combine_fast_kernel(int M, int N, const float* __restrict__ zdev, float zhost,
                                                                    float inv_reg, float la_bin, float lb, float lb_bin,
                                                                    const float* __restrict__ v_in, float* __restrict__ v_out,
                                                                    int ldv, float* __restrict__ u, int ldu,
                                                                    const float* __restrict__ ps, int ldp, int RB, float in_scale,
                                                                    float out_scale, int rows, RD rd) {
    const int b = blockIdx.y, tid = threadIdx.x;
    const float u_scale = out_scale == 1.f ? 1.f : LOG2E;
    int RBv = RB;
    if (rd.B > 0) {
        M = rd.off0[b + 1] - rd.off0[b];
        N = rd.off1[b + 1] - rd.off1[b];
        if ((int)blockIdx.x * 256 > N) return;
        RBv = (M + rows - 1) / rows;
        const float norm = -__logf((float)(M + N));
        lb = norm; la_bin = norm + __logf((float)N); lb_bin = norm + __logf((float)M);
    }
    const float zr2 = (zdev ? zdev[0] : zhost) * inv_reg * LOG2E;
    const float* vb = v_in + (int64_t)b * ldv;
    float* ub = u + (int64_t)b * ldu;
    __shared__ float smx[3][4];
    const int lane = tid & 63, wave = tid >> 6;
    const bool owns_bin = (int)blockIdx.x == N / 256;

    const int j = blockIdx.x * 256 + tid;
    float colsum = 0.f, vo = 0.f;
    if (j < N) {
        const float* psb = ps + (int64_t)b * RB * ldp + j;
        vo = vb[j] * in_scale;
        for (int rb0 = 0; rb0 < RBv; rb0 += 8) {
            float t[8];
#pragma unroll
            for (int q = 0; q < 8; ++q) t[q] = rb0 + q < RBv ? psb[(int64_t)(rb0 + q) * ldp] : 0.f;
#pragma unroll
            for (int q = 0; q < 8; ++q) colsum += t[q];
        }
    }
    const float vNo = vb[N] * in_scale;
    float us = 0.f;
    if (owns_bin)
        for (int i = tid; i < M; i += 256) us += __builtin_amdgcn_exp2f(zr2 + vNo + ub[i] * u_scale);

    float m = OG_NEG_INF;
    for (int jj = tid; jj <= N; jj += 256) m = fmaxf(m, vb[jj]);
    m = wave_max(m) * in_scale;
    float sv = 0.f;
    if (m != OG_NEG_INF)
        for (int jj = tid; jj <= N; jj += 256) sv += __builtin_amdgcn_exp2f(vb[jj] * in_scale - m);
    sv = wave_sum(sv);
    us = wave_sum(us);
    if (lane == 0) { smx[0][wave] = m; smx[1][wave] = sv; smx[2][wave] = us; }
    __syncthreads();
    const float mm = fmaxf(fmaxf(smx[0][0], smx[0][1]), fmaxf(smx[0][2], smx[0][3]));
    float st = 0.f, ust = 0.f;
#pragma unroll
    for (int w = 0; w < 4; ++w) {
        st += smx[0][w] == OG_NEG_INF ? 0.f : smx[1][w] * __builtin_amdgcn_exp2f(smx[0][w] - mm);
        ust += smx[2][w];
    }
    const float uM = la_bin * LOG2E - (zr2 + mm + __builtin_amdgcn_logf(st));
    if (blockIdx.x == 0 && tid == 0) ub[M] = uM * out_scale;

    if (j < N) {
        const float cs = colsum + __builtin_amdgcn_exp2f(zr2 + vo + uM);
        v_out[(int64_t)b * ldv + j] = (vo + lb * LOG2E - __builtin_amdgcn_logf(cs)) * out_scale;
    }
    if (owns_bin && tid == 0) {
        const float tot = ust + __builtin_amdgcn_exp2f(zr2 + vNo + uM);
        v_out[(int64_t)b * ldv + N] = (vNo + lb_bin * LOG2E - __builtin_amdgcn_logf(tot)) * out_scale;
    }
}

template <class RD>
__global__ __launch_bounds__(256) void sinkhorn_scores_kernel(const float* __restrict__ S, int64_t lds, int M, int N,
                                                              const float* __restrict__ zdev, float zhost,
                                                              float inv_reg, float norm,
                                                              const float* __restrict__ u, int ldu,
                                                              const float* __restrict__ v, int ldv,
                                                              float* __restrict__ scores, int64_t strideS, RD rd, RowBest rb,
                                                              unsigned* __restrict__ nonfinite) {
    const int b = blockIdx.y;
    int64_t so = (int64_t)b * (M + 1) * (N + 1);
    if (rd.B > 0) {
        M = rd.off0[b + 1] - rd.off0[b];
        N = rd.off1[b + 1] - rd.off1[b];
        norm = -__logf((float)(M + N));
        so = rd.soff[b];
    }
    S += (int64_t)b * strideS;
    const int row = blockIdx.x * 4 + (threadIdx.x >> 6);
    const int lane = threadIdx.x & 63;
    if (row > M) return;
    const float zr = (zdev ? zdev[0] : zhost) * inv_reg;
    const float ui = u[(int64_t)b * ldu + row];
    const float* vb = v + (int64_t)b * ldv;
    float* out = scores + so + (int64_t)row * (N + 1);
    float chk = 0.f;
    if (row < M) {
        const float* sp = S + (int64_t)row * lds;
        if (rb.idx) {
            float best = OG_NEG_INF;
            int bi = 0x7FFFFFFF;
            for (int j = lane; j < N; j += 64) {
                const float val = ((sp[j] * inv_reg + ui) + vb[j]) - norm;
                out[j] = val;
                chk = fmaf(val, 0.f, chk);
                if (val > best || bi == 0x7FFFFFFF) { best = val; bi = j; }
            }
#pragma unroll
            for (int o = 32; o > 0; o >>= 1) {
                const float ov = __shfl_xor(best, o, 64);
                const int oi = __shfl_xor(bi, o, 64);
                if (ov > best || (ov == best && oi < bi)) { best = ov; bi = oi; }
            }
            if (lane == 0) { rb.idx[(int64_t)b * rb.stride + row] = bi; rb.val[(int64_t)b * rb.stride + row] = best; }
        } else {
            for (int j = lane; j < N; j += 64) { const float val = ((sp[j] * inv_reg + ui) + vb[j]) - norm; out[j] = val; chk = fmaf(val, 0.f, chk); }
        }
    } else {
        for (int j = lane; j < N; j += 64) { const float val = ((zr + ui) + vb[j]) - norm; out[j] = val; chk = fmaf(val, 0.f, chk); }
    }
    if (lane == 0) { const float val = ((zr + ui) + vb[N]) - norm; out[N] = val; chk = fmaf(val, 0.f, chk); }
    if (nonfinite && __any(chk != chk) && lane == 0) atomicOr(nonfinite, 1u);
}

template <int CPL, int RG, int WPR, class RD>
void launch_sweep(const float* S, int64_t lds, int B, int m, int n, const float* zdev, float zhost, float inv_reg, float la,
                  const float* v_in, const SinkhornWs& w, hipStream_t st, const RD& rd) {
    constexpr int NRS = 4 / WPR;
    const size_t shmem = sizeof(float) * ((size_t)NRS * 2 * 256 * CPL * WPR + 2 * NRS * RG * WPR * 2);
    hipLaunchKernelGGL((sinkhorn_sweep_kernel<CPL, RG, WPR, RD>), dim3(w.RB, B), dim3(256), shmem, st, S, lds, m, n, zdev, zhost,
                       inv_reg, la, v_in, w.ldv, w.u, w.ldu, w.pm, w.ps, w.ldp, w.RB, (int64_t)m * lds, rd);
}

template <int CPL, int RG, int WPR, class RD, int ROWS, bool NT>
void launch_sweep_fast_g(const float* S, int64_t lds, int B, int m, int n, const float* zdev, float zhost, float inv_reg, float la,
                         const float* v_in, const SinkhornWs& w, hipStream_t st, const RD& rd, float in_scale, float out_scale) {
    constexpr int NRS = 4 / WPR;
    const size_t shmem = sizeof(float) * ((size_t)NRS * 256 * CPL * WPR + 2 * NRS * RG * WPR);
    const int RB = (m + ROWS - 1) / ROWS;
    hipLaunchKernelGGL((sinkhorn_sweep_fast_kernel<CPL, RG, WPR, RD, ROWS, NT>), dim3(RB, B), dim3(256), shmem, st, S, lds, m, n, zdev, zhost,
                       inv_reg, la, v_in, w.ldv, w.u, w.ldu, w.ps, w.ldp, RB, (int64_t)m * lds, in_scale, out_scale, rd);
}
template <int CPL, int RG, int WPR, class RD>
void launch_sweep_fast(const float* S, int64_t lds, int B, int m, int n, const float* zdev, float zhost, float inv_reg, float la,
                       const float* v_in, const SinkhornWs& w, hipStream_t st, const RD& rd, float in_scale, float out_scale, int rows,
                       int nt) {
#define OG_SKF(ROWS_, NT_) launch_sweep_fast_g<CPL, RG, WPR, RD, ROWS_, NT_>(S, lds, B, m, n, zdev, zhost, inv_reg, la, v_in, w, st, rd, in_scale, out_scale)
    if constexpr (std::is_same<RD, RaggedNone>::value && WPR > 1) {
        if (rows == 128) { if (nt) OG_SKF(128, true); else OG_SKF(128, false); return; }
        if (rows == 64) { if (nt) OG_SKF(64, true); else OG_SKF(64, false); return; }
        if (nt) { OG_SKF(SK_ROWS, true); return; }
    }
    OG_SKF(SK_ROWS, false);
#undef OG_SKF
}

template <class RD>
__global__ __launch_bounds__(1024) void sinkhorn_fallback_kernel(const float* __restrict__ S, int64_t lds, int64_t strideS, int M, int N,
                                                                 const float* __restrict__ zdev, float zhost, float inv_reg, float la,
                                                                 float la_bin, float lb, float lb_bin, float* __restrict__ u, int ldu,
                                                                 float* __restrict__ v, int ldv, int iters, unsigned* status, RD rd) {
    if (__hip_atomic_load(status, __ATOMIC_RELAXED, __HIP_MEMORY_SCOPE_AGENT) == 0u) return;
    __shared__ float uL[8196];
    __shared__ float vL[4100];
    __shared__ float red[2][16];
    const int b = blockIdx.x, tid = threadIdx.x, lane = tid & 63, wave = tid >> 6;
    if (rd.B > 0) {
        M = rd.off0[b + 1] - rd.off0[b];
        N = rd.off1[b + 1] - rd.off1[b];
        const float norm = -__logf((float)(M + N));
        la = norm; lb = norm; la_bin = norm + __logf((float)N); lb_bin = norm + __logf((float)M);
    }
    const float* Sb = S + (int64_t)b * strideS;
    float* ub = u + (int64_t)b * ldu;
    float* vb = v + (int64_t)b * ldv;
    float* uw = M + 1 <= 8196 ? uL : ub;
    const float zr = (zdev ? zdev[0] : zhost) * inv_reg;
    for (int j = tid; j <= N; j += 1024) vL[j] = 0.f;
    __syncthreads();
    auto block_lse = [&](float mx, float sm) -> float {
        float m2 = wave_max(mx);
        sm = wave_sum(sm * (mx == OG_NEG_INF ? 0.f : expf(mx - m2)));
        if (lane == 0) { red[0][wave] = m2; red[1][wave] = sm; }
        __syncthreads();
        float bm = OG_NEG_INF, bs = 0.f;
        for (int w = 0; w < 16; ++w) bm = fmaxf(bm, red[0][w]);
        for (int w = 0; w < 16; ++w) bs += red[1][w] * (red[0][w] == OG_NEG_INF ? 0.f : expf(red[0][w] - bm));
        __syncthreads();
        return bm + logf(bs);
    };
    for (int it = 0; it < iters; ++it) {
        for (int i = wave; i < M; i += 16) {
            const float* sp = Sb + (int64_t)i * lds;
            float mx = OG_NEG_INF;
            for (int j = lane; j < N; j += 64) mx = fmaxf(mx, sp[j] * inv_reg + vL[j]);
            mx = wave_max(fmaxf(mx, zr + vL[N]));
            float sm = 0.f;
            for (int j = lane; j < N; j += 64) sm += expf(sp[j] * inv_reg + vL[j] - mx);
            sm = wave_sum(sm) + expf(zr + vL[N] - mx);
            if (lane == 0) uw[i] = la - (mx + logf(sm));
        }
        {
            float mx = OG_NEG_INF, sm = 0.f;
            for (int j = tid; j <= N; j += 1024) { const float x = zr + vL[j]; const float nm = fmaxf(mx, x); sm = sm * (mx == OG_NEG_INF ? 0.f : expf(mx - nm)) + expf(x - nm); mx = nm; }
            const float l = block_lse(mx, sm);
            if (tid == 0) uw[M] = la_bin - l;
        }
        __syncthreads();
        for (int j = tid; j < N; j += 1024) {
            float mx = zr + uw[M], sm = 1.f;
            for (int i = 0; i < M; ++i) {
                const float x = Sb[(int64_t)i * lds + j] * inv_reg + uw[i];
                const float nm = fmaxf(mx, x);
                sm = sm * expf(mx - nm) + expf(x - nm);
                mx = nm;
            }
            vb[j] = lb - (mx + logf(sm));
        }
        float nv;
        {
            float mx = OG_NEG_INF, sm = 0.f;
            for (int i = tid; i <= M; i += 1024) { const float x = zr + uw[i]; const float nm = fmaxf(mx, x); sm = sm * (mx == OG_NEG_INF ? 0.f : expf(mx - nm)) + expf(x - nm); mx = nm; }
            nv = lb_bin - block_lse(mx, sm);
        }
        __syncthreads();
        for (int j = tid; j < N; j += 1024) vL[j] = vb[j];
        if (tid == 0) { vL[N] = nv; vb[N] = nv; }
        __syncthreads();
    }
    if (uw != ub) for (int i = tid; i <= M; i += 1024) ub[i] = uw[i];
    __syncthreads();
    if (tid == 0 && b == 0) { __threadfence(); __hip_atomic_store(status, 2u, __ATOMIC_RELAXED, __HIP_MEMORY_SCOPE_AGENT); }
}

}

extern "C" size_t og_sinkhorn_workspace_bytes(int32_t batch, int32_t m, int32_t n) {
    if (batch <= 0 || m <= 0 || n <= 0 || n > 8192) return 0;
    const int64_t RB = (m + SK_ROWS - 1) / SK_ROWS;
    const int64_t ldu = og_round_up(m + 1, 4), ldv = og_round_up(n + 1, 4), ldp = og_round_up(n, 4);
    const int64_t floats = (int64_t)batch * (ldu + 2 * ldv) + 4 + 2 * (int64_t)batch * RB * ldp;
    return (size_t)og_round_up(floats * (int64_t)sizeof(float), 256) + og_sinkhorn_resident_ws_bytes(batch, m, n);
}

static inline void* sk_resident_ws(void* ws, int B, int m, int n) {
    const int64_t RB = (m + SK_ROWS - 1) / SK_ROWS;
    const int64_t ldu = og_round_up(m + 1, 4), ldv = og_round_up(n + 1, 4), ldp = og_round_up(n, 4);
    const int64_t floats = (int64_t)B * (ldu + 2 * ldv) + 4 + 2 * (int64_t)B * RB * ldp;
    return (char*)ws + og_round_up(floats * (int64_t)sizeof(float), 256);
}

namespace {
template <class RD>
int sinkhorn_run(const float* S, int64_t lds, const float* zdev, float dustbin, int B, int m, int n, int iters, float reg,
                 float* scores, void* workspace, hipStream_t st, const RD& rd, const RowBest* row_best, bool trusted_padding) {
    if (!S || !scores || !workspace || B <= 0 || m <= 0 || n <= 0 || iters < 0 || !(reg > 0.f)) return OG_E_INVALID;
    if (n > 8192) return OG_E_SHAPE;
    if ((lds & 3) || ((uintptr_t)S & 15) || ((uintptr_t)workspace & 15)) return OG_E_ALIGN;
    const SinkhornWs w = sk_layout(workspace, B, m, n);
    const float inv_reg = 1.f / reg;
    const double norm = -log((double)m + (double)n);
    const float la = (float)norm, lb = (float)norm;
    const float la_bin = (float)norm + (float)log((double)n);
    const float lb_bin = (float)norm + (float)log((double)m);
    hipError_t e = hipMemsetAsync(w.u, 0, sizeof(float) * ((size_t)B * (w.ldu + 2 * (size_t)w.ldv) + 4), st);
    if (e != hipSuccess) return (int)e;
    const SinkhornGeom g = sk_geom(n);
    int cur = 0;
    static const bool robust_only = [] { const char* e = getenv("OG_SINKHORN_ROBUST"); return e && atoi(e) != 0; }();
    const char* rm_env = getenv("OG_SINKHORN_RESIDENT");
    const int resident_mode = rm_env ? atoi(rm_env) : 1;
    bool resident = !robust_only && iters > 1;
    if constexpr (std::is_same<RD, RaggedNone>::value) resident = resident && og_sinkhorn_resident_wanted(B, m, n, resident_mode);
    else resident = resident && og_sinkhorn_resident_ws_bytes(B, m, n) > 0 && og_sinkhorn_resident_ragged_wanted(rd, resident_mode);
    int fast_rows = SK_ROWS, fast_nt = 0;
    if (std::is_same<RD, RaggedNone>::value) {
        for (int r = 2 * SK_ROWS; r <= 4 * SK_ROWS; r *= 2)
            if ((int64_t)((m + r - 1) / r) * B >= 512) fast_rows = r;
        fast_nt = (int64_t)B * m * lds * (int64_t)sizeof(float) > ((int64_t)256 << 20);
    }
    { const char* e = getenv("OG_SK_FAST_ROWS"); if (e && (atoi(e) == 32 || atoi(e) == 64 || atoi(e) == 128)) fast_rows = atoi(e); }
    { const char* e = getenv("OG_SK_FAST_NT"); if (e) fast_nt = atoi(e) != 0; }
    for (int it = 0; it < iters; ++it) {
        const float* vin = w.v[cur];
        if (it > 0 && resident) {
            unsigned* status = w.flags + 1;
            void* xws = sk_resident_ws(workspace, B, m, n);
            const char* ft = getenv("OG_SINKHORN_FORCE_TIMEOUT");
            if (ft && atoi(ft) != 0) {
                e = hipMemsetAsync(status, 1, sizeof(unsigned), st);
                if (e != hipSuccess) return (int)e;
            } else {
                int rc;
                if constexpr (std::is_same<RD, RaggedNone>::value)
                    rc = og_launch_sinkhorn_resident(S, lds, zdev, dustbin, B, m, n, iters - 1, inv_reg, la, la_bin, lb, lb_bin, w.u, w.ldu, w.v[cur],
                                                     w.v[cur ^ 1], w.ldv, xws, status, st, trusted_padding);
                else
                    rc = og_launch_sinkhorn_resident_ragged(S, lds, zdev, dustbin, rd, m, n, iters - 1, inv_reg, w.u, w.ldu, w.v[cur], w.v[cur ^ 1],
                                                            w.ldv, xws, status, st, trusted_padding);
                if (rc) return rc;
            }
            cur ^= 1;
            hipLaunchKernelGGL(sinkhorn_fallback_kernel<RD>, dim3(B), dim3(1024), 0, st, S, lds, (int64_t)m * lds, m, n, zdev, dustbin, inv_reg, la,
                               la_bin, lb, lb_bin, w.u, w.ldu, w.v[cur], w.ldv, iters, status, rd);
            break;
        }
        if (it > 0 && !robust_only) {
            const float is = it == 1 ? LOG2E : 1.f, os = it == iters - 1 ? LN2 : 1.f;
            const int rows = (std::is_same<RD, RaggedNone>::value && g.WPR > 1) ? fast_rows : SK_ROWS, RBf = (m + rows - 1) / rows;
            if (g.CPL == 1) launch_sweep_fast<1, 4, 1>(S, lds, B, m, n, zdev, dustbin, inv_reg, la, vin, w, st, rd, is, os, rows, fast_nt);
            else if (g.CPL == 2) launch_sweep_fast<2, 4, 1>(S, lds, B, m, n, zdev, dustbin, inv_reg, la, vin, w, st, rd, is, os, rows, fast_nt);
            else if (g.CPL == 8) launch_sweep_fast<8, 1, 4>(S, lds, B, m, n, zdev, dustbin, inv_reg, la, vin, w, st, rd, is, os, rows, fast_nt);
            else if (g.WPR == 1) launch_sweep_fast<4, 2, 1>(S, lds, B, m, n, zdev, dustbin, inv_reg, la, vin, w, st, rd, is, os, rows, fast_nt);
            else if (g.WPR == 2) launch_sweep_fast<4, 2, 2>(S, lds, B, m, n, zdev, dustbin, inv_reg, la, vin, w, st, rd, is, os, rows, fast_nt);
            else launch_sweep_fast<4, 2, 4>(S, lds, B, m, n, zdev, dustbin, inv_reg, la, vin, w, st, rd, is, os, rows, fast_nt);
            hipLaunchKernelGGL(sinkhorn_combine_fast_kernel<RD>, dim3((n + 1 + 255) / 256, B), dim3(256), 0, st, m, n, zdev, dustbin,
                               inv_reg, la_bin, lb, lb_bin, w.v[cur], w.v[cur ^ 1], w.ldv, w.u, w.ldu, w.ps, w.ldp, RBf, is, os, rows, rd);
            cur ^= 1;
            continue;
        }
        if (g.CPL == 1) launch_sweep<1, 4, 1>(S, lds, B, m, n, zdev, dustbin, inv_reg, la, vin, w, st, rd);
        else if (g.CPL == 2) launch_sweep<2, 4, 1>(S, lds, B, m, n, zdev, dustbin, inv_reg, la, vin, w, st, rd);
        else if (g.CPL == 8) launch_sweep<8, 1, 4>(S, lds, B, m, n, zdev, dustbin, inv_reg, la, vin, w, st, rd);
        else if (g.WPR == 1) launch_sweep<4, 2, 1>(S, lds, B, m, n, zdev, dustbin, inv_reg, la, vin, w, st, rd);
        else if (g.WPR == 2) launch_sweep<4, 2, 2>(S, lds, B, m, n, zdev, dustbin, inv_reg, la, vin, w, st, rd);
        else launch_sweep<4, 2, 4>(S, lds, B, m, n, zdev, dustbin, inv_reg, la, vin, w, st, rd);
        hipLaunchKernelGGL(sinkhorn_combine_kernel<RD>, dim3((n + 1 + 255) / 256, B), dim3(256), 0, st, m, n, zdev, dustbin, inv_reg, la_bin,
                           lb, lb_bin, w.v[cur], w.v[cur ^ 1], w.ldv, w.u, w.ldu, w.pm, w.ps, w.ldp, w.RB, rd);
        cur ^= 1;
    }
    hipLaunchKernelGGL(sinkhorn_scores_kernel<RD>, dim3((m + 1 + 3) / 4, B), dim3(256), 0, st, S, lds, m, n, zdev, dustbin, inv_reg,
                       (float)norm, w.u, w.ldu, w.v[cur], w.ldv, scores, (int64_t)m * lds, rd, row_best ? *row_best : RowBest{nullptr, nullptr, 0}, w.flags);
    return og_launch_status();
}
}

int og_launch_sinkhorn_trajectory(const float* S, int64_t lds, const float* dustbin_dev, float dustbin, int B, int m, int n, int iters, float reg, float* scores,
                                  void* workspace, float* U, float* V, hipStream_t st) {
    if (n > 8192) return OG_E_SHAPE;
    SinkhornWs w = sk_layout(workspace, B, m, n);
    const float inv_reg = 1.f / reg;
    const double norm = -log((double)m + (double)n);
    const float la = (float)norm, lb = (float)norm;
    const float la_bin = (float)norm + (float)log((double)n), lb_bin = (float)norm + (float)log((double)m);
    hipError_t e = hipMemsetAsync(V, 0, sizeof(float) * (size_t)(iters + 1) * B * w.ldv, st);
    if (e != hipSuccess) return (int)e;
    const SinkhornGeom g = sk_geom(n);
    const RaggedNone rd{};
    for (int it = 0; it < iters; ++it) {
        const float* vin = V + (size_t)it * B * w.ldv;
        float* vout = V + (size_t)(it + 1) * B * w.ldv;
        w.u = U + (size_t)it * B * w.ldu;
        if (g.CPL == 1) launch_sweep<1, 4, 1>(S, lds, B, m, n, dustbin_dev, dustbin, inv_reg, la, vin, w, st, rd);
        else if (g.CPL == 2) launch_sweep<2, 4, 1>(S, lds, B, m, n, dustbin_dev, dustbin, inv_reg, la, vin, w, st, rd);
        else if (g.CPL == 8) launch_sweep<8, 1, 4>(S, lds, B, m, n, dustbin_dev, dustbin, inv_reg, la, vin, w, st, rd);
        else if (g.WPR == 1) launch_sweep<4, 2, 1>(S, lds, B, m, n, dustbin_dev, dustbin, inv_reg, la, vin, w, st, rd);
        else if (g.WPR == 2) launch_sweep<4, 2, 2>(S, lds, B, m, n, dustbin_dev, dustbin, inv_reg, la, vin, w, st, rd);
        else launch_sweep<4, 2, 4>(S, lds, B, m, n, dustbin_dev, dustbin, inv_reg, la, vin, w, st, rd);
        hipLaunchKernelGGL(sinkhorn_combine_kernel<RaggedNone>, dim3((n + 1 + 255) / 256, B), dim3(256), 0, st, m, n, dustbin_dev, dustbin,
                           inv_reg, la_bin, lb, lb_bin, vin, vout, w.ldv, w.u, w.ldu, w.pm, w.ps, w.ldp, w.RB, rd);
    }
    hipLaunchKernelGGL(sinkhorn_scores_kernel<RaggedNone>, dim3((m + 1 + 3) / 4, B), dim3(256), 0, st, S, lds, m, n, dustbin_dev, dustbin,
                       inv_reg, (float)norm, U + (size_t)(iters - 1) * B * w.ldu, w.ldu, V + (size_t)iters * B * w.ldv, w.ldv, scores,
                       (int64_t)m * lds, rd, RowBest{nullptr, nullptr, 0}, (unsigned*)nullptr);
    return og_launch_status();
}

int og_launch_sinkhorn(const float* S, int64_t lds, const float* zdev, float dustbin, int B, int m, int n, int iters, float reg,
                       float* scores, void* workspace, hipStream_t st, const RaggedDesc* rag, const RowBest* row_best, bool trusted_padding) {
    if (rag) {
        if (rag->B != B) return OG_E_INVALID;
        return sinkhorn_run<RaggedDesc>(S, lds, zdev, dustbin, B, m, n, iters, reg, scores, workspace, st, *rag, row_best, trusted_padding);
    }
    return sinkhorn_run<RaggedNone>(S, lds, zdev, dustbin, B, m, n, iters, reg, scores, workspace, st, RaggedNone{}, row_best, trusted_padding);
}

extern "C" int og_sinkhorn_schedule(int32_t batch, int32_t m, int32_t n, int32_t iters) {
    static const bool robust_only = [] { const char* e = getenv("OG_SINKHORN_ROBUST"); return e && atoi(e) != 0; }();
    const char* rm_env = getenv("OG_SINKHORN_RESIDENT");
    const int resident_mode = rm_env ? atoi(rm_env) : 1;
    return (!robust_only && iters > 1 && og_sinkhorn_resident_wanted(batch, m, n, resident_mode)) ? og_sinkhorn_resident_rounds(batch, m, n) : 0;
}

extern "C" int og_sinkhorn_schedule_ragged(int32_t batch, const int32_t* lens0, const int32_t* lens1, int32_t iters) {
    static const bool robust_only = [] { const char* e = getenv("OG_SINKHORN_ROBUST"); return e && atoi(e) != 0; }();
    if (batch <= 0 || batch > OG_MAX_RAGGED || !lens0 || !lens1 || robust_only || iters <= 1) return 0;
    const char* rm_env = getenv("OG_SINKHORN_RESIDENT");
    const int resident_mode = rm_env ? atoi(rm_env) : 1;
    RaggedDesc rd{};
    rd.B = batch;
    int mmax = 0, nmax = 0;
    for (int b = 0; b < batch; ++b) {
        rd.off0[b + 1] = rd.off0[b] + lens0[b]; rd.off1[b + 1] = rd.off1[b] + lens1[b];
        if (lens0[b] > mmax) mmax = lens0[b];
        if (lens1[b] > nmax) nmax = lens1[b];
    }
    if (og_sinkhorn_resident_ws_bytes(batch, mmax, nmax) == 0 || !og_sinkhorn_resident_ragged_wanted(rd, resident_mode)) return 0;
    int launches = 0;
    if (og_launch_sinkhorn_resident_ragged(nullptr, 0, nullptr, 0.f, rd, mmax, nmax, iters - 1, 1.f, nullptr, 0, nullptr, nullptr, 0, nullptr, nullptr, nullptr, true, &launches)) return 0;
    return launches;
}

extern "C" int og_sinkhorn_status(const void* workspace_dev, int32_t batch, int32_t m, int32_t n) {
    if (!workspace_dev || batch <= 0 || m <= 0 || n <= 0 || n > 8192) return -1;
    const SinkhornWs w = sk_layout(const_cast<void*>(workspace_dev), batch, m, n);
    const bool has_res = og_sinkhorn_resident_ws_bytes(batch, m, n) != 0;
    unsigned words[2] = {0, 0};
    hipStream_t q = nullptr;
    if (hipStreamCreateWithFlags(&q, hipStreamNonBlocking) != hipSuccess) return -1;
    int rc = 0;
    hipEvent_t ev = nullptr;
    if (hipEventCreateWithFlags(&ev, hipEventDisableTiming) != hipSuccess || hipEventRecord(ev, nullptr) != hipSuccess ||
        hipStreamWaitEvent(q, ev, 0) != hipSuccess) rc = -1;
    if (!rc && hipMemcpyAsync(&words[0], w.flags, sizeof(unsigned) * (has_res ? 2 : 1), hipMemcpyDeviceToHost, q) != hipSuccess) rc = -1;
    if (hipStreamSynchronize(q) != hipSuccess) rc = -1;
    if (ev) (void)hipEventDestroy(ev);
    (void)hipStreamDestroy(q);
    if (rc) return rc;
    if (words[0]) return 3;
    if (!has_res) return 0;
    return words[1] == 0 ? 0 : words[1] == 2 ? 2 : 1;
}

extern "C" int og_sinkhorn(const float* S, int64_t lds, float dustbin, int32_t batch, int32_t m, int32_t n,
                           int32_t iters, float reg, float* scores, void* workspace_dev, void* stream) {
    og_clear_status();
    return og_launch_sinkhorn(S, lds, nullptr, dustbin, batch, m, n, iters, reg, scores, workspace_dev, (hipStream_t)stream, nullptr, nullptr, false);
}
```

openglue_amd/csrc/sinkhorn_resident.hip:

```cpp
#include <stdlib.h>
#include <math.h>
#include <type_traits>

#include "og_common.h"

namespace {

constexpr int RS_RW = 16;
constexpr int RS_RR = 12;
constexpr int RS_LR = 4;
static_assert(RS_RR + RS_LR == RS_RW, "sixteen row slots per wave");
constexpr int RS_NW = 8;
constexpr int RS_SEG = 1024;
constexpr int RS_PAD = 64;
constexpr int RS_RREC = 136;
constexpr int RS_MAXWG = 256;
constexpr int RS_MAXPAIRS = 128;
constexpr unsigned RS_SPIN_LIMIT = 1u << 21;
constexpr float RS_DRIFT_BITS = 40.f;
constexpr float RS_LOG2E = 1.4426950408889634f;
constexpr float RS_LN2 = 0.6931471805599453f;

typedef unsigned long long rs_u64;
typedef float rs_f32x2 __attribute__((ext_vector_type(2)));
// ... 710 lines not shown
    RsGeom q{0, 0, 0, 1};
    if (m <= 0 || n <= 0 || n > 4 * RS_SEG) return q;
    auto rows = [&](int W) { const int RB = rw * RS_NW / W; int g = (m + RB - 1) / RB; return g < 2 * W ? 2 * W : g; };
    if (n <= RS_SEG) { q.W = 1; q.X = 1; }
    else if (n <= 2 * RS_SEG) { if (rows(2) <= 32) { q.W = 2; q.X = 1; } else { q.W = 1; q.X = 2; } }
    else { if (rows(4) <= 32) { q.W = 4; q.X = 1; } else if (rows(2) <= 32) { q.W = 2; q.X = 2; } else { q.W = 1; q.X = 4; } }
    q.Gx = rows(q.W);
    if (q.Gx > 32) { q.W = 0; return q; }
    q.G = q.X * q.Gx;
    return q;
}
int rs_pairs_per_round(const RsGeom& q, int cus) {
    if (q.W == 0 || cus < 8) return 0;
    if (cus >= 256) return (8 / q.X) * (32 / q.Gx);
    return q.X == 1 ? cus / q.G : 0;
}

size_t rs_area_bytes(int W, int slots, int groups) {
    const size_t NCX = (size_t)RS_SEG * W + RS_PAD;
    return 256 + (size_t)RS_MAXWG * sizeof(unsigned) + (size_t)2 * slots * NCX * 8 + (size_t)2 * groups * NCX * 8 + (size_t)2 * groups * 32 * RS_RREC * 8;
}

template <int W, class MAP>
void rs_launch(const SkResArgs& a, const MAP& map, int grid, hipStream_t st) {
    hipLaunchKernelGGL((sinkhorn_resident_kernel<W, MAP>), dim3(grid), dim3(512), 0, st, a, map);
}

int rs_rows_per_wave(int B, int m, int n, int cus) {
    if (cus < 256 || n > RS_SEG) return RS_RW;
    const RsGeom q16 = rs_geom(m, n);
    if (q16.W == 0) return RS_RW;
    const char* e = getenv("OG_SINKHORN_FEW");
    const int want = e ? atoi(e) : -1;
    if (want == 0) return RS_RW;
    for (int rw = 4; rw <= 8; rw *= 2) {
        if (want > 1 && want != rw) continue;
        const RsGeom q = rs_geom(m, n, rw);
        if (q.W != 1 || q.X != 1 || (int64_t)B * q.G > 256 || B > rs_pairs_per_round(q, cus)) continue;
        if (want < 0 && (int64_t)B * rs_geom(m, n, 2 * rw).G > 128) continue;
        return rw;
    }
    return RS_RW;
}

}

bool og_sinkhorn_resident_shape_ok(int B, int m, int n) {
    return B > 0 && rs_geom(m, n).W != 0;
}

size_t og_sinkhorn_resident_ws_bytes(int B, int m, int n) {
    if (!og_sinkhorn_resident_shape_ok(B, m, n)) return 0;
    const int Wmax = n <= RS_SEG ? 1 : n <= 2 * RS_SEG ? 2 : 4;
    return rs_area_bytes(Wmax, RS_MAXWG, RS_MAXPAIRS);
}

extern "C" int og_sinkhorn_resident_geometry(int32_t m, int32_t n, int32_t* out4) {
    if (!out4) return OG_E_INVALID;
    const RsGeom q = rs_geom(m, n);
    if (q.W == 0) return OG_E_SHAPE;
    out4[0] = q.W; out4[1] = q.X; out4[2] = q.Gx; out4[3] = rs_pairs_per_round(q, 256);
    return 0;
}

extern "C" int og_sinkhorn_resident_rows_per_wave(int32_t batch, int32_t m, int32_t n) {
    if (batch <= 0 || rs_geom(m, n).W == 0) return 0;
    return rs_rows_per_wave(batch, m, n, 256);
}

int og_sinkhorn_resident_rounds(int B, int m, int n) {
    if (!og_sinkhorn_resident_shape_ok(B, m, n)) return 0;
    const int ppr = rs_pairs_per_round(rs_geom(m, n, rs_rows_per_wave(B, m, n, rs_num_cus())), rs_num_cus());
    return ppr > 0 ? (B + ppr - 1) / ppr : 0;
}

bool og_sinkhorn_resident_wanted(int B, int m, int n, int mode) {
    if (mode <= 0) return false;
    const int rounds = og_sinkhorn_resident_rounds(B, m, n);
    if (rounds <= 0) return false;
    if (mode >= 2) return true;
    return (int64_t)B * m * n >= (int64_t)1 << 18;
}

int og_launch_sinkhorn_resident(const float* S, int64_t lds, const float* zdev, float zhost, int B, int m, int n, int iters,
                                float inv_reg, float la, float la_bin, float lb, float lb_bin, float* u, int ldu, const float* v_in,
                                float* v_out, int ldv, void* xws, unsigned* status, hipStream_t st, bool trusted_padding) {
    if (!S || !u || !v_in || !v_out || !xws || !status || iters < 1 || !og_sinkhorn_resident_shape_ok(B, m, n)) return OG_E_INVALID;
    const int rw = rs_rows_per_wave(B, m, n, rs_num_cus());
    const RsGeom q = rs_geom(m, n, rw);
    const int ppr = rs_pairs_per_round(q, rs_num_cus());
    if (ppr <= 0) return OG_E_SHAPE;
    const int rounds = (B + ppr - 1) / ppr, per = (B + rounds - 1) / rounds;
    hipError_t e = hipSuccess;
    SkResArgs a{};
    a.S = S; a.lds = lds; a.strideS = (int64_t)m * lds;
    a.u = u; a.ldu = ldu; a.v_in = v_in; a.v_out = v_out; a.ldv = ldv;
    a.status = status;
    a.xcc = (unsigned*)((char*)xws + 256);
    a.xa = (char*)xws + 256 + RS_MAXWG * sizeof(unsigned);
    { const char* ev = getenv("OG_SINKHORN_AGENT_SCOPE"); a.force_agent_scope = ev && atoi(ev) != 0; }
    a.zdev = zdev; a.zhost = zhost; a.inv_reg = inv_reg; a.la = la; a.la_bin = la_bin; a.lb = lb; a.lb_bin = lb_bin;
    a.m = m; a.n = n; a.iters = iters;
    a.sanitize_pad = (n & 3) && !trusted_padding;
    const size_t NCX = (size_t)RS_SEG * q.W + RS_PAD;
    const bool xcd_map = rs_num_cus() >= 256;
    for (int b0 = 0; b0 < B; b0 += per) {
        const int np = B - b0 < per ? B - b0 : per;
        a.b0 = b0; a.npairs = np; a.slots = np * q.G; a.groups = np * q.X;
        a.xb = a.xa + (size_t)2 * a.slots * NCX * 8;
        a.xc = a.xb + (size_t)2 * a.groups * NCX * 8;
        e = hipMemsetAsync(a.xcc, 0, RS_MAXWG * sizeof(unsigned) + (size_t)2 * a.slots * NCX * 8 + (size_t)2 * a.groups * NCX * 8 + (size_t)2 * a.groups * 32 * RS_RREC * 8, st);
        if (e != hipSuccess) return (int)e;
        RsUniform map{q.G, q.Gx, q.X, 0};
        int grid = np * q.G;
        a.local_ok = 0;
        if (xcd_map) {
            const int ppl = 8 / q.X;
            map.layers = (np + ppl - 1) / ppl; grid = 8 * map.layers * q.Gx; a.local_ok = 1;
        }
        if (rw == 4) hipLaunchKernelGGL((sinkhorn_resident_kernel<1, RsUniform, 4>), dim3(grid), dim3(512), 0, st, a, map);
        else if (rw == 8) hipLaunchKernelGGL((sinkhorn_resident_kernel<1, RsUniform, 8>), dim3(grid), dim3(512), 0, st, a, map);
        else if (q.W == 1) rs_launch<1>(a, map, grid, st);
        else if (q.W == 2) rs_launch<2>(a, map, grid, st);
        else rs_launch<4>(a, map, grid, st);
    }
    return og_launch_status();
}

namespace {
struct RsPlanPair { int b, W, G; };
bool rs_ragged_plan(const RaggedDesc& rd, RsPlanPair* pp, int cus) {
    if (rd.B <= 0 || rd.B > OG_MAX_RAGGED || cus < 256) return false;
    for (int b = 0; b < rd.B; ++b) {
        const RsGeom q = rs_geom(rd.off0[b + 1] - rd.off0[b], rd.off1[b + 1] - rd.off1[b]);
        if (q.W == 0 || q.X != 1) return false;
        pp[b] = RsPlanPair{b, q.W, q.G};
    }
    return true;
}
size_t rs_ragged_launch_bytes(int W, int slots, int groups) {
    const size_t NCX = (size_t)RS_SEG * W + RS_PAD;
    return 256 + (size_t)RS_MAXWG * sizeof(unsigned) + (size_t)2 * slots * NCX * 8 + (size_t)2 * groups * NCX * 8;
}
template <class F>
void rs_ragged_for_each_launch(const RaggedDesc& rd, RsPlanPair* pp, F&& f) {
    for (int i = 1; i < rd.B; ++i) { const RsPlanPair t = pp[i]; int j = i; while (j > 0 && pp[j - 1].G < t.G) { pp[j] = pp[j - 1]; --j; } pp[j] = t; }
    bool done[OG_MAX_RAGGED] = {};
    for (int W = 4; W >= 1; W /= 2) {
        for (;;) {
            RsRagged map;
            for (int i = 0; i < RS_MAXWG; ++i) map.wg[i] = -1;
            int used[8] = {0, 0, 0, 0, 0, 0, 0, 0}, np = 0, slots = 0, qmax = 0;
            auto place = [&](int i, int G) {
                int x = -1;
                for (int k = 0; k < 8; ++k) if (used[k] + G <= 32 && (x < 0 || used[k] < used[x])) x = k;
                if (x < 0) return;
                const int b = pp[i].b;
                map.gb[np] = b; map.G[np] = G; map.gbase[np] = slots;
                map.m[np] = rd.off0[b + 1] - rd.off0[b]; map.n[np] = rd.off1[b + 1] - rd.off1[b];
                for (int g = 0; g < G; ++g) map.wg[x + 8 * (used[x] + g)] = (np << 8) | g;
                used[x] += G; if (used[x] > qmax) qmax = used[x];
                slots += G; ++np; done[i] = true;
            };
            for (int i = 0; i < rd.B; ++i)
                if (!done[i] && pp[i].W == W) place(i, pp[i].G);
            if (np > 0) {
                const int RB = RS_RW * RS_NW / W;
                for (int i = 0; i < rd.B; ++i) {
                    if (done[i] || pp[i].W >= W) continue;
                    const int b = pp[i].b, mrows = rd.off0[b + 1] - rd.off0[b];
                    int G = (mrows + RB - 1) / RB;
                    if (G < 2 * W) G = 2 * W;
                    if (G <= 32) place(i, G);
                }
            }
            if (np == 0) break;
            f(W, map, np, slots, qmax);
        }
    }
}
}

bool og_sinkhorn_resident_ragged_wanted(const RaggedDesc& rd, int mode) {
    if (mode <= 0) return false;
    RsPlanPair pp[OG_MAX_RAGGED];
    if (!rs_ragged_plan(rd, pp, rs_num_cus())) return false;
    if (mode >= 2) return true;
    int64_t elems = 0;
    for (int b = 0; b < rd.B; ++b) elems += (int64_t)(rd.off0[b + 1] - rd.off0[b]) * (rd.off1[b + 1] - rd.off1[b]);
    return elems >= (int64_t)1 << 18;
}

extern "C" int og_sinkhorn_resident_ragged_footprint(int32_t batch, const int32_t* lens0, const int32_t* lens1, int64_t* out2) {
    if (!lens0 || !lens1 || !out2 || batch <= 0 || batch > OG_MAX_RAGGED) return OG_E_INVALID;
    RaggedDesc rd{};
    rd.B = batch;
    for (int b = 0; b < batch; ++b) {
        if (lens0[b] <= 0 || lens1[b] <= 0) return OG_E_SHAPE;
        rd.off0[b + 1] = rd.off0[b] + lens0[b]; rd.off1[b + 1] = rd.off1[b] + lens1[b];
    }
    RsPlanPair pp[OG_MAX_RAGGED];
    if (!rs_ragged_plan(rd, pp, 256)) return OG_E_SHAPE;
    int64_t launches = 0, bytes = 0;
    rs_ragged_for_each_launch(rd, pp, [&](int W, const RsRagged&, int np, int slots, int) {
        ++launches;
        const int64_t by = (int64_t)rs_ragged_launch_bytes(W, slots, np);
        if (by > bytes) bytes = by;
    });
    out2[0] = launches; out2[1] = bytes;
    return 0;
}

int og_launch_sinkhorn_resident_ragged(const float* S, int64_t lds, const float* zdev, float zhost, const RaggedDesc& rd, int m_max, int n_max, int iters,
                                       float inv_reg, float* u, int ldu, const float* v_in, float* v_out, int ldv, void* xws, unsigned* status,
                                       hipStream_t st, bool trusted_padding, int* count_only) {
    if (!count_only && (!S || !u || !v_in || !v_out || !xws || !status || iters < 1)) return OG_E_INVALID;
    RsPlanPair pp[OG_MAX_RAGGED];
    if (!rs_ragged_plan(rd, pp, rs_num_cus())) return OG_E_SHAPE;
    if (count_only) *count_only = 0;
    const size_t ws_bytes = og_sinkhorn_resident_ws_bytes(rd.B, m_max, n_max);
    SkResArgs a{};
    a.S = S; a.lds = lds; a.strideS = (int64_t)m_max * lds;
    a.u = u; a.ldu = ldu; a.v_in = v_in; a.v_out = v_out; a.ldv = ldv;
    a.status = status;
    a.xcc = (unsigned*)((char*)xws + 256);
    a.xa = (char*)xws + 256 + RS_MAXWG * sizeof(unsigned);
    { const char* ev = getenv("OG_SINKHORN_AGENT_SCOPE"); a.force_agent_scope = ev && atoi(ev) != 0; }
    a.zdev = zdev; a.zhost = zhost; a.inv_reg = inv_reg;
    a.m = m_max; a.n = n_max; a.iters = iters; a.local_ok = 1;
    (void)trusted_padding;
    a.sanitize_pad = 1;
    int rc = 0;
    rs_ragged_for_each_launch(rd, pp, [&](int W, const RsRagged& map, int np, int slots, int qmax) {
        if (count_only) { ++*count_only; return; }
        if (rc) return;
        if (rs_ragged_launch_bytes(W, slots, np) > ws_bytes) { rc = OG_E_SHAPE; return; }
        const size_t NCX = (size_t)RS_SEG * W + RS_PAD;
        a.b0 = 0; a.npairs = np; a.slots = slots; a.groups = np;
        a.xb = a.xa + (size_t)2 * a.slots * NCX * 8;
        a.xc = a.xb + (size_t)2 * a.groups * NCX * 8;
        const hipError_t e = hipMemsetAsync(a.xcc, 0, rs_ragged_launch_bytes(W, slots, np) - 256, st);
        if (e != hipSuccess) { rc = (int)e; return; }
        const int grid = 8 * qmax;
        if (W == 1) rs_launch<1>(a, map, grid, st);
        else if (W == 2) rs_launch<2>(a, map, grid, st);
        else rs_launch<4>(a, map, grid, st);
    });
    if (rc) return rc;
    return count_only ? 0 : og_launch_status();
}
```

openglue_amd/ops.py:

```python
from __future__ import annotations

from typing import Dict, Optional

import torch

from . import _lib


def gemm_nt(a: torch.Tensor, b: torch.Tensor, bias: Optional[torch.Tensor] = None, relu: bool = False,
            res: Optional[torch.Tensor] = None, alpha: Optional[torch.Tensor] = None, scale: float = 1.0) -> torch.Tensor:
    a, b = _lib.gpu_tensor(a, "a"), _lib.gpu_tensor(b, "b")
    batched = a.dim() == 3
    Z = a.shape[0] if batched else 1
    M, K = a.shape[-2:]
    N = b.shape[-2]
    out = torch.empty((Z, M, N) if batched else (M, N), device=a.device, dtype=torch.float32)
    if bias is not None: bias = _lib.gpu_tensor(bias, "bias")
    if res is not None: res = _lib.gpu_tensor(res, "res")
    if alpha is not None: alpha = _lib.gpu_tensor(alpha, "alpha")
    _lib.call("og_gemm_nt", a.device, a.data_ptr(), K, M * K if batched else 0, b.data_ptr(), K, N * K if b.dim() == 3 else 0,
              out.data_ptr(), N, M * N, M, N, K, Z, _lib.ptr(bias), int(relu), _lib.ptr(res), N, _lib.ptr(alpha),
              float(scale), _lib.STREAM)
    return out

# ... 65 lines not shown
    if planes:
        ch = torch.empty(M, N, device=a.device, dtype=torch.float16); cl = torch.empty_like(ch); ldch = N
    else:
        ch = torch.empty(M, 2 * N, device=a.device, dtype=torch.float16); cl = None; ldch = 2 * N
    _lib.call("og_gemm_nt_f16x3_reshl", a.device, a_hl.data_ptr(), 2 * K, b_hl.data_ptr(), 2 * K, M, N, K, 1.0 / 256.0, _lib.ptr(bias), int(relu),
              _lib.ptr(res_hl), 2 * N, None, N, ch.data_ptr(), _lib.ptr(cl), ldch, int(not planes), _lib.STREAM)
    return merge_f16(ch, cl) if planes else merge_f16_hl(ch)


def mlp_block(x: torch.Tensor, o: torch.Tensor, w0: torch.Tensor, b0: torch.Tensor, w3: torch.Tensor, b3: torch.Tensor,
              return_rows: bool = False):
    lib = _lib.load()
    x, o = _lib.gpu_tensor(x, "x"), _lib.gpu_tensor(o, "o")
    M, D = x.shape
    nbytes = lib.og_mlp_block_stream_bytes(D)
    if nbytes == 0:
        raise RuntimeError(f"og_mlp_block: no fused message-MLP kernel for D = {D}")
    w0h, w3h = w0.detach().float().cpu().contiguous(), w3.detach().float().cpu().contiguous()
    stream_host = torch.empty(nbytes, dtype=torch.uint8)
    _lib.check(lib.og_mlp_block_pack(D, w0h.data_ptr(), w3h.data_ptr(), stream_host.data_ptr()), "og_mlp_block_pack")
    stream_dev = stream_host.to(x.device)
    rows = split_f16_hl(torch.cat([x, o], dim=1).contiguous())
    b0, b3 = _lib.gpu_tensor(b0, "b0"), _lib.gpu_tensor(b3, "b3")
    _lib.call("og_mlp_block", x.device, D, rows.data_ptr(), 4 * D, M, stream_dev.data_ptr(), b0.data_ptr(), b3.data_ptr(), _lib.STREAM)
    out = merge_f16_hl(rows)[:, :D].contiguous()
    return (out, rows) if return_rows else out


def proj_block(x: torch.Tensor, w: torch.Tensor, bias: torch.Tensor, split_row: int = 0, cols_a=None, cols_b=None):
    lib = _lib.load()
    x = _lib.gpu_tensor(x, "x")
    M, K = x.shape
    N = w.shape[0]
    nbytes = lib.og_proj_block_stream_bytes(N, K)
    if nbytes == 0:
        raise RuntimeError(f"og_proj_block: no kernel for N = {N}, K = {K}")
    wh = w.detach().float().cpu().contiguous()
    stream_host = torch.empty(nbytes, dtype=torch.uint8)
    _lib.check(lib.og_proj_block_pack(N, K, wh.data_ptr(), stream_host.data_ptr()), "og_proj_block_pack")
    stream_dev = stream_host.to(x.device)
    rows = split_f16_hl(x)
    bias = _lib.gpu_tensor(bias, "bias")
    inv = torch.full((1,), 1.0 / 256.0, device=x.device, dtype=torch.float32)
    yh = torch.zeros(M, N, device=x.device, dtype=torch.float16)
    yl = torch.zeros_like(yh)
    a, b = cols_a or (0, N), cols_b or (0, N)
    _lib.call("og_proj_block", x.device, rows.data_ptr(), 2 * K, M, K, N, stream_dev.data_ptr(), bias.data_ptr(), inv.data_ptr(), yh.data_ptr(), yl.data_ptr(), N,
              split_row, a[0] // 32, a[1] // 32, b[0] // 32, b[1] // 32, _lib.STREAM)
    return merge_f16(yh, yl)


def attention(q: torch.Tensor, k: torch.Tensor, v: torch.Tensor, num_heads: int, return_lse: bool = False):
    q, k, v = _lib.gpu_tensor(q * 1.4426950408889634, "q"), _lib.gpu_tensor(k, "k"), _lib.gpu_tensor(v, "v")
    Z, nq, D = q.shape
    nk = k.shape[1]
    (qh, ql), (kh, kl), (vh, vl) = split_f16(q), split_f16(k), split_f16(v)
    oh = torch.empty(Z, nq, D, device=q.device, dtype=torch.float16)
    ol = torch.empty_like(oh)
    lse = torch.empty(Z, num_heads, nq, device=q.device, dtype=torch.float32) if return_lse else None
    _lib.call("og_attention", q.device, qh.data_ptr(), ql.data_ptr(), D, kh.data_ptr(), kl.data_ptr(), D, vh.data_ptr(), vl.data_ptr(), D,
              oh.data_ptr(), ol.data_ptr(), D, Z, nq, nk, num_heads, D // num_heads, _lib.ptr(lse), _lib.STREAM)
    return (merge_f16(oh, ol), lse) if return_lse else merge_f16(oh, ol)


def sinkhorn(S: torch.Tensor, dustbin: float, iters: int, reg: float = 1.0, return_status: bool = False):
    lib = _lib.load()
    S = _lib.gpu_tensor(S, "S")
    B, m, n = S.shape
    lds = (n + 3) // 4 * 4
    if lds != n:
        Sp = torch.zeros(B, m, lds, device=S.device, dtype=torch.float32)
        Sp[:, :, :n] = S
        S = Sp
    ws = torch.empty(lib.og_sinkhorn_workspace_bytes(B, m, n), device=S.device, dtype=torch.uint8)
    out = torch.empty(B, m + 1, n + 1, device=S.device, dtype=torch.float32)
    _lib.call("og_sinkhorn", S.device, S.data_ptr(), lds, float(dustbin), B, m, n, int(iters), float(reg), out.data_ptr(),
              ws.data_ptr(), _lib.STREAM)
    if return_status:
        torch.cuda.current_stream(S.device).synchronize()
        return out, int(lib.og_sinkhorn_status(ws.data_ptr(), B, m, n))
    return out


def extract_matches(scores: torch.Tensor, match_threshold: float, both_sides: bool = True) -> Dict[str, torch.Tensor]:
    lib = _lib.load()
    scores = _lib.gpu_tensor(scores, "scores")
    B, m1, n1 = scores.shape
    m, n = m1 - 1, n1 - 1
    dev = scores.device
    ws = torch.empty(lib.og_matches_workspace_bytes(B, m, n), device=dev, dtype=torch.uint8)
    out = {"matches0": torch.empty(B, m, device=dev, dtype=torch.int64),
           "matching_scores0": torch.empty(B, m, device=dev, dtype=torch.float32)}
    if both_sides:
        out["matches1"] = torch.empty(B, n, device=dev, dtype=torch.int64)
        out["matching_scores1"] = torch.empty(B, n, device=dev, dtype=torch.float32)
    _lib.call("og_extract_matches", dev, scores.data_ptr(), B, m, n, float(match_threshold), out["matches0"].data_ptr(),
              out["matching_scores0"].data_ptr(), _lib.ptr(out.get("matches1")), _lib.ptr(out.get("matching_scores1")),
              ws.data_ptr(), _lib.STREAM)
    return out
```

Before: 3556 image-pairs/s.

## Cut small launches and memsets across encoder, attention, sinkhorn and matches

```diff
diff --git a/include/openglue_amd.h b/include/openglue_amd.h
--- a/include/openglue_amd.h
+++ b/include/openglue_amd.h
@@ -185,6 +185,7 @@
 int og_sinkhorn_schedule_ragged(int32_t batch, const int32_t* lens0, const int32_t* lens1, int32_t iters);
 int og_sinkhorn_resident_geometry(int32_t m, int32_t n, int32_t* out4);
 int og_sinkhorn_resident_rows_per_wave(int32_t batch, int32_t m, int32_t n);
+int og_sinkhorn_fill_ranges(int32_t batch, int32_t m, int32_t n, int64_t* out6);
 int og_sinkhorn_resident_ragged_footprint(int32_t batch, const int32_t* lens0, const int32_t* lens1, int64_t* out2);
 int og_forward_status(const og_shape* shape, const void* workspace_dev);
 
@@ -231,6 +232,10 @@
 int og_extract_matches(const float* scores, int32_t batch, int32_t m, int32_t n, float match_threshold,
                        int64_t* matches0, float* matching_scores0, int64_t* matches1,
                        float* matching_scores1, void* workspace_dev, void* stream);
+
+int og_sinkhorn_matches(const float* S, int64_t lds, float dustbin, int32_t batch, int32_t m, int32_t n, int32_t iters, float reg,
+                        float match_threshold, float* scores, int64_t* matches0, float* matching_scores0, int64_t* matches1,
+                        float* matching_scores1, void* sinkhorn_workspace_dev, void* matches_workspace_dev, void* stream);
 
 
 int og_prepare_features(const float* lafs, const float* responses, int64_t tokens, int32_t method, int32_t log_response,
diff --git a/openglue_amd/_lib.py b/openglue_amd/_lib.py
--- a/openglue_amd/_lib.py
+++ b/openglue_amd/_lib.py
@@ -127,6 +127,7 @@
     "og_sinkhorn_resident_geometry": (C.c_int, [_i32, _i32, _vp]),
     "og_sinkhorn_resident_ragged_footprint": (C.c_int, [_i32, _vp, _vp, _vp]),
     "og_sinkhorn_resident_rows_per_wave": (C.c_int, [_i32, _i32, _i32]),
+    "og_sinkhorn_fill_ranges": (C.c_int, [_i32, _i32, _i32, _vp]),
     "og_forward_status": (C.c_int, [_vp, _vp]),
     "og_sinkhorn_train_workspace_bytes": (_sz, [_i32, _i32, _i32, _i32]),
     "og_sinkhorn_train_forward": (C.c_int, [_vp, _i64, _f, _vp, _i32, _i32, _i32, _i32, _f, _vp, _vp, _vp]),
@@ -140,6 +141,7 @@
     "og_softmax_rows": (C.c_int, [_vp, _i64, _i64, _i32, _vp]),
     "og_softmax_rows_backward": (C.c_int, [_vp, _vp, _i64, _i64, _i32, _f, _vp]),
     "og_sinkhorn": (C.c_int, [_vp, _i64, _f, _i32, _i32, _i32, _i32, _f, _vp, _vp, _vp]),
+    "og_sinkhorn_matches": (C.c_int, [_vp, _i64, _f, _i32, _i32, _i32, _i32, _f, _f, _vp, _vp, _vp, _vp, _vp, _vp, _vp, _vp]),
     "og_matches_workspace_bytes": (_sz, [_i32, _i32, _i32]),
     "og_prepare_features": (C.c_int, [_vp, _vp, _i64, _i32, _i32, _vp, _vp, _vp]),
     "og_compact_workspace_bytes": (_sz, [_i32, _i32]),
diff --git a/openglue_amd/csrc/api.hip b/openglue_amd/csrc/api.hip
--- a/openglue_amd/csrc/api.hip
+++ b/openglue_amd/csrc/api.hip
@@ -474,8 +474,8 @@
         float* Eb = ws + W.eb;
         {
             Scope sc(prof, OG_STAGE_ENCODER_INPUT);
-            if ((rc = og_launch_encoder_input(in->keypoints0, in->side_info0, T0, s.side_info, in->image0_wh[0], in->image0_wh[1], EI, st, er0))) return rc;
-            if ((rc = og_launch_encoder_input(in->keypoints1, in->side_info1, T1, s.side_info, in->image1_wh[0], in->image1_wh[1], EI + T0 * 32, st, er1))) return rc;
+            if ((rc = og_launch_encoder_input(in->keypoints0, in->side_info0, T0, in->image0_wh[0], in->image0_wh[1], in->keypoints1, in->side_info1, T1,
+                                              in->image1_wh[0], in->image1_wh[1], s.side_info, EI, st, er0, er1))) return rc;
         }
         const float* cur = EI; int64_t ldcur = 32;
         const bool tail_f16 = L.enc_whl >= 0;
@@ -522,9 +522,8 @@
     if (encoder_only) return og_launch_status();
 
     const int dh = D / s.num_heads;
-    if (hipMemsetAsync(ws + W.attn, 0, OG_ATTN_COUNTERS * sizeof(int), st) != hipSuccess) return OG_E_INVALID;
-    auto attention = [&](int nz, int split, int64_t qb0, int64_t qs0, int nq0, int64_t kb0, int64_t ks0, int nk0,
-                         int64_t qb1, int64_t qs1, int nq1, int64_t kb1, int64_t ks1, int nk1, int rag_mode) -> int {
+    auto attention_args = [&](int nz, int split, int64_t qb0, int64_t qs0, int nq0, int64_t kb0, int64_t ks0, int nk0,
+                              int64_t qb1, int64_t qs1, int nq1, int64_t kb1, int64_t ks1, int nk1, int rag_mode) -> AttnArgs {
         AttnArgs a{};
         a.rag = rag; a.rag_mode = rag_mode;
         a.qh = QKVh; a.ql = QKVl; a.ldq = QW; a.kh = QKVh + WQ; a.kl = QKVl + WQ; a.ldk = QW;
@@ -535,10 +534,19 @@
         a.counters = reinterpret_cast<int*>(ws + W.attn); a.partial = ws + W.attn + OG_ATTN_COUNTERS;
         a.q_base[0] = qb0; a.q_step[0] = qs0; a.nq[0] = nq0; a.kv_base[0] = kb0; a.kv_step[0] = ks0; a.nk[0] = nk0;
         a.q_base[1] = qb1; a.q_step[1] = qs1; a.nq[1] = nq1; a.kv_base[1] = kb1; a.kv_step[1] = ks1; a.nk[1] = nk1;
+        return a;
+    };
+    const bool softmax_attention = !favor && !(s.flags & OG_FLAG_LINEAR_ATTENTION);
+    auto attention = [&](const AttnArgs& a) -> int {
         Scope sc(prof, OG_STAGE_ATTENTION);
         if (favor) return og_launch_favor_attention(a, st);
-        return (s.flags & OG_FLAG_LINEAR_ATTENTION) ? og_launch_linear_attention(a, st) : og_launch_attention(a, st);
-    };
+        return softmax_attention ? og_launch_attention(a, st) : og_launch_linear_attention(a, st);
+    };
+    const AttnArgs attn_self = attention_args(2 * B, B, 0, m, m, 0, m, m, T0, n, n, T0, n, n, 1);
+    const AttnArgs attn_cross0 = attention_args(B, B, 0, m, m, T0, n, n, 0, 0, 0, 0, 0, 0, 2);
+    const AttnArgs attn_cross1 = attention_args(B, B, T0, n, n, 0, m, m, 0, 0, 0, 0, 0, 0, 3);
+    if (softmax_attention && (og_attention_key_split(attn_self) > 1 || og_attention_key_split(attn_cross0) > 1 || og_attention_key_split(attn_cross1) > 1))
+        if (hipMemsetAsync(ws + W.attn, 0, OG_ATTN_COUNTERS * sizeof(int), st) != hipSuccess) return OG_E_INVALID;
     auto proj_small_ok = [&](int64_t R) {
         static const int mode = [] { const char* e = getenv("OG_PROJ_SMALL"); return e ? atoi(e) : -1; }();
         return L.o_wqkvs >= 0 && !favor && (mode >= 0 ? mode != 0 : R <= 8192) && R < ((int64_t)1 << 30);
@@ -589,7 +597,7 @@
         {
             Range r_stage("gnn self", l);
             if ((rc = qkv_proj(lw, 0, T, 0, QW))) return rc;
-            if ((rc = attention(2 * B, B, 0, m, m, 0, m, m, T0, n, n, T0, n, n, 1))) return rc;
+            if ((rc = attention(attn_self))) return rc;
             if ((rc = mlp(lw, 0, T))) return rc;
         }
         if ((rc = tap_here(2 * l + 1))) return rc;
@@ -617,9 +625,7 @@
             } else {
                 if ((rc = qkv_proj(lw, 0, T0, WQ, QW))) return rc;
             }
-            if (side == 0) rc = attention(B, B, 0, m, m, T0, n, n, 0, 0, 0, 0, 0, 0, 2);
-            else rc = attention(B, B, T0, n, n, 0, m, m, 0, 0, 0, 0, 0, 0, 3);
-            if (rc) return rc;
+            if ((rc = attention(side == 0 ? attn_cross0 : attn_cross1))) return rc;
             if ((rc = mlp(lw, qr0, qR))) return rc;
         }
         if ((rc = tap_here(2 * l + 2))) return rc;
diff --git a/openglue_amd/csrc/attention.hip b/openglue_amd/csrc/attention.hip
--- a/openglue_amd/csrc/attention.hip
+++ b/openglue_amd/csrc/attention.hip
@@ -1736,46 +1736,68 @@
 
 }
 
+namespace {
+struct AttnGeom { int qtiles, nqmax, nkmin; unsigned grid; bool dma; };
+int attn_geom(const AttnArgs& a, AttnGeom& g) {
+    if (a.nz <= 0 || a.num_heads <= 0) return OG_E_INVALID;
+    int nqmax = 0;
+    g.nkmin = 1 << 30;
+    for (int i = 0; i < 2; ++i) {
+        const bool used = i == 0 ? a.split > 0 : a.split < a.nz;
+        if (!used) continue;
+        if (a.nq[i] <= 0 || a.nk[i] <= 0) return OG_E_INVALID;
+        if (a.nq[i] > nqmax) nqmax = a.nq[i];
+        if (a.nk[i] < g.nkmin) g.nkmin = a.nk[i];
+    }
+    g.nqmax = nqmax;
+    g.qtiles = (nqmax + Q_TILE - 1) / Q_TILE;
+    static const bool dma_on = [] { const char* e = getenv("OG_ATTN_DMA"); return !(e && e[0] == '0'); }();
+    g.dma = dma_on && (a.dh == 64 || a.dh == 32);
+    const int groups8 = (a.nz * a.num_heads + 7) / 8 * 8;
+    g.grid = (unsigned)(groups8 * g.qtiles);
+    return 0;
+}
+}
+
+int og_attention_key_split(const AttnArgs& a) {
+    AttnGeom g;
+    if (attn_geom(a, g)) return 1;
+    const unsigned grid = g.grid;
+    const int nkmin = g.nkmin;
+    const bool dma = g.dma;
+    static const int gs_mode = [] { const char* e = getenv("OG_ATTN_GSPLIT"); return e ? atoi(e) : -1; }();
+    int gs = 1;
+    if (!a.mx && dma && (a.dh == 64 || a.dh == 32) && a.partial && a.counters && (int)grid <= OG_ATTN_COUNTERS) {
+        static const int maxwg_env = [] { const char* e = getenv("OG_ATTN_GS_MAXWG"); return e ? atoi(e) : 0; }();
+        const int maxwg = maxwg_env > 0 ? maxwg_env : (a.dh == 32 ? 512 : 256);
+        if (gs_mode >= 0) gs = gs_mode == 2 || gs_mode == 4 ? gs_mode : 1;
+        else if ((int)grid * 4 <= maxwg && (a.rag || nkmin >= 16 * KV_TILE)) gs = 4;
+        else if ((int)grid * 2 <= maxwg && (a.rag || nkmin >= 8 * KV_TILE)) gs = 2;
+        if ((int)grid * gs > maxwg && gs_mode < 0) gs = 1;
+        if ((int64_t)grid * gs * 4 * 34 * 64 > OG_ATTN_PARTIAL_FLOATS) gs = 1;
+    }
+    return gs;
+}
+
 int og_launch_attention(const AttnArgs& a, hipStream_t stream) {
     if (!a.qh || !a.ql || !a.kh || !a.kl || !a.vh || !a.vl || !a.oh || !a.ol || a.nz <= 0 || a.num_heads <= 0) return OG_E_INVALID;
     if ((a.ldq & 7) || (a.ldk & 7) || (a.ldv & 7) || (a.ldo & 3)) return OG_E_ALIGN;
     const void* ps[8] = {a.qh, a.ql, a.kh, a.kl, a.vh, a.vl, a.oh, a.ol};
     for (int i = 0; i < 8; ++i)
         if ((uintptr_t)ps[i] & 15) return OG_E_ALIGN;
-    int nqmax = 0;
-    for (int g = 0; g < 2; ++g) {
-        const bool used = g == 0 ? a.split > 0 : a.split < a.nz;
-        if (!used) continue;
-        if (a.nq[g] <= 0 || a.nk[g] <= 0) return OG_E_INVALID;
-        if (a.nq[g] > nqmax) nqmax = a.nq[g];
-    }
+    AttnGeom ag;
+    if (int e = attn_geom(a, ag)) return e;
+    const int nkmin = ag.nkmin;
     AttnArgs a2 = a;
-    a2.qtiles = (nqmax + Q_TILE - 1) / Q_TILE;
+    a2.qtiles = ag.qtiles;
     RaggedDesc rd;
     rd.B = 0;
     if (a.rag) rd = *a.rag;
     a2.rag = nullptr;
-    static const bool dma_on = [] { const char* e = getenv("OG_ATTN_DMA"); return !(e && e[0] == '0'); }();
-    const bool dma = dma_on && (a.dh == 64 || a.dh == 32);
-    const int groups8 = (a.nz * a.num_heads + 7) / 8 * 8;
-    dim3 grid(groups8 * a2.qtiles), block(256);
+    const bool dma = ag.dma;
+    dim3 grid(ag.grid), block(256);
     static const int ks_mode = [] { const char* e = getenv("OG_ATTN_KSPLIT"); return e ? atoi(e) : -1; }();
-    int nkmin = 1 << 30;
-    for (int g = 0; g < 2; ++g) {
-        const bool used = g == 0 ? a.split > 0 : a.split < a.nz;
-        if (used && a.nk[g] < nkmin) nkmin = a.nk[g];
-    }
-    static const int gs_mode = [] { const char* e = getenv("OG_ATTN_GSPLIT"); return e ? atoi(e) : -1; }();
-    int gs = 1;
-    if (!a.mx && dma && (a.dh == 64 || a.dh == 32) && a.partial && a.counters && (int)grid.x <= OG_ATTN_COUNTERS) {
-        static const int maxwg_env = [] { const char* e = getenv("OG_ATTN_GS_MAXWG"); return e ? atoi(e) : 0; }();
-        const int maxwg = maxwg_env > 0 ? maxwg_env : (a.dh == 32 ? 512 : 256);
-        if (gs_mode >= 0) gs = gs_mode == 2 || gs_mode == 4 ? gs_mode : 1;
-        else if ((int)grid.x * 4 <= maxwg && (a.rag || nkmin >= 16 * KV_TILE)) gs = 4;
-        else if ((int)grid.x * 2 <= maxwg && (a.rag || nkmin >= 8 * KV_TILE)) gs = 2;
-        if ((int)grid.x * gs > maxwg && gs_mode < 0) gs = 1;
-        if ((int64_t)grid.x * gs * 4 * 34 * 64 > OG_ATTN_PARTIAL_FLOATS) gs = 1;
-    }
+    const int gs = og_attention_key_split(a);
     if (gs > 1) {
         dim3 g2(grid.x * gs);
         const char* const sc = getenv("OG_ATTN_GS_SCATTER");
@@ -1831,8 +1853,8 @@
 #endif
 #if OG_ATTN_PIPE8
     if (pipe && pipe_mode == 2 && a.dh == 64) {
-        a2.qtiles = (nqmax + 2 * Q_TILE - 1) / (2 * Q_TILE);
-        dim3 grid8(groups8 * a2.qtiles);
+        a2.qtiles = (ag.nqmax + 2 * Q_TILE - 1) / (2 * Q_TILE);
+        dim3 grid8((a.nz * a.num_heads + 7) / 8 * 8 * a2.qtiles);
         if (a.rag) hipLaunchKernelGGL((attention_dma_kernel<64, RaggedDesc, 1, 1, 0, 2>), grid8, dim3(512), 0, stream, a2, rd);
         else hipLaunchKernelGGL((attention_dma_kernel<64, RaggedNone, 1, 1, 0, 2>), grid8, dim3(512), 0, stream, a2, RaggedNone{});
         return og_launch_status();
diff --git a/openglue_amd/csrc/matches.hip b/openglue_amd/csrc/matches.hip
--- a/openglue_amd/csrc/matches.hip
+++ b/openglue_amd/csrc/matches.hip
@@ -15,14 +15,6 @@
     w.idx0 = (int*)p; p += sizeof(int) * (size_t)B * m;
     w.max0 = (float*)p;
     return w;
-}
-
-__device__ __forceinline__ unsigned int orderable(float v) {
-    const unsigned int b = __float_as_uint(v);
-    return (b & 0x80000000u) ? ~b : (b | 0x80000000u);
-}
-__device__ __forceinline__ float unorderable(unsigned int k) {
-    return __uint_as_float((k & 0x80000000u) ? (k & 0x7FFFFFFFu) : ~k);
 }
 
 template <class RD>
@@ -78,8 +70,7 @@
         const float v = sp[(int64_t)i * (N + 1)];
         if (v > best) { best = v; bi = i; }
     }
-    const unsigned long long key = ((unsigned long long)orderable(best) << 32) | (unsigned long long)(0xFFFFFFFFu - (unsigned)bi);
-    atomicMax(colbest + (int64_t)b * Nmax + j, key);
+    atomicMax(colbest + (int64_t)b * Nmax + j, og_col_key(best, bi));
 }
 
 template <class RD>
@@ -112,14 +103,21 @@
     }
 }
 
-__global__ __launch_bounds__(256) void encoder_input_kernel(const float* __restrict__ kpts, const float* __restrict__ side,
-                                                            int64_t tokens, int s, float wm1, float hm1,
-                                                            float* __restrict__ out, EncoderRagged er) {
+struct EncoderImages { const float* kpts[2]; const float* side[2]; float wm1[2], hm1[2]; int64_t tokens[2]; };
+template <class ER>
+__global__ __launch_bounds__(256) void encoder_input_kernel(EncoderImages im, int s, float* __restrict__ out, ER er0, ER er1) {
     const int64_t g = (int64_t)blockIdx.x * 256 + threadIdx.x;
-    const int64_t t = g >> 3;
+    int64_t t = g >> 3;
     const int c4 = (int)(g & 7) * 4;
-    if (t >= tokens) return;
-    if (er.B > 0) {
+    if (t >= im.tokens[0] + im.tokens[1]) return;
+    out += t * 32 + c4;
+    const int img = t >= im.tokens[0];
+    if (img) t -= im.tokens[0];
+    const float* kpts = im.kpts[img];
+    const float* side = im.side[img];
+    float wm1 = im.wm1[img], hm1 = im.hm1[img];
+    if constexpr (ER::ragged) {
+        const ER& er = img ? er1 : er0;
         int lo = 0, hi = er.B - 1;
         while (lo < hi) {
             const int mid = (lo + hi + 1) >> 1;
@@ -137,7 +135,7 @@
         else if (c < 2 + s) v = side[t * s + (c - 2)];
         o[e] = v;
     }
-    *reinterpret_cast<f32x4*>(out + t * 32 + c4) = o;
+    *reinterpret_cast<f32x4*>(out) = o;
 }
 
 }
@@ -155,10 +153,12 @@
     if ((matches1 == nullptr) != (ms1 == nullptr)) return OG_E_INVALID;
     if ((uintptr_t)workspace & 15) return OG_E_ALIGN;
     const MatchWs w = mw_layout(workspace, B, m, n);
-    hipError_t e = hipMemsetAsync(w.colbest, 0, sizeof(unsigned long long) * (size_t)B * n, st);
-    if (e != hipSuccess) return (int)e;
-    if (!rows_done) hipLaunchKernelGGL(row_argmax_kernel<RD>, dim3((m + 3) / 4, B), dim3(256), 0, st, scores, m, n, w.idx0, w.max0, rd);
-    hipLaunchKernelGGL(col_argmax_kernel<RD>, dim3((n + 255) / 256, (m + 63) / 64, B), dim3(256), 0, st, scores, m, n, w.colbest, rd);
+    if (!rows_done) {
+        hipError_t e = hipMemsetAsync(w.colbest, 0, sizeof(unsigned long long) * (size_t)B * n, st);
+        if (e != hipSuccess) return (int)e;
+        hipLaunchKernelGGL(row_argmax_kernel<RD>, dim3((m + 3) / 4, B), dim3(256), 0, st, scores, m, n, w.idx0, w.max0, rd);
+        hipLaunchKernelGGL(col_argmax_kernel<RD>, dim3((n + 255) / 256, (m + 63) / 64, B), dim3(256), 0, st, scores, m, n, w.colbest, rd);
+    }
     const int mx = m > n ? m : n;
     hipLaunchKernelGGL(mutual_kernel<RD>, dim3((mx + 255) / 256, B), dim3(256), 0, st, m, n, thr, w.idx0, w.max0, w.colbest,
                        matches0, ms0, matches1, ms1, rd);
@@ -177,7 +177,7 @@
 
 RowBest og_matches_row_best(void* matches_workspace, int B, int m, int n) {
     const MatchWs w = mw_layout(matches_workspace, B, m, n);
-    return RowBest{w.idx0, w.max0, m};
+    return RowBest{w.idx0, w.max0, m, w.colbest, n};
 }
 
 extern "C" int og_extract_matches(const float* scores, int32_t batch, int32_t m, int32_t n, float match_threshold,
@@ -188,14 +188,15 @@
                              matching_scores1, workspace_dev, (hipStream_t)stream, nullptr, false);
 }
 
-int og_launch_encoder_input(const float* kpts, const float* side, int64_t tokens, int s, float wx, float wy,
-                            float* out, hipStream_t st, const EncoderRagged* er) {
-    if (!kpts || !out || tokens <= 0 || s < 0 || 2 + s > 32 || (s > 0 && !side)) return OG_E_INVALID;
-    const int64_t threads = tokens * 8;
-    EncoderRagged e;
-    e.B = 0;
-    if (er) e = *er;
-    hipLaunchKernelGGL(encoder_input_kernel, dim3((unsigned)((threads + 255) / 256)), dim3(256), 0, st, kpts, side, tokens,
-                       s, wx - 1.f, wy - 1.f, out, e);
+int og_launch_encoder_input(const float* kpts0, const float* side0, int64_t tokens0, float wx0, float wy0, const float* kpts1, const float* side1,
+                            int64_t tokens1, float wx1, float wy1, int s, float* out, hipStream_t st, const EncoderRagged* er0, const EncoderRagged* er1) {
+    if (!kpts0 || !out || tokens0 <= 0 || tokens1 < 0 || s < 0 || 2 + s > 32 || (s > 0 && !side0)) return OG_E_INVALID;
+    if (tokens1 > 0 && (!kpts1 || (s > 0 && !side1))) return OG_E_INVALID;
+    if ((er0 == nullptr) != (er1 == nullptr) && tokens1 > 0) return OG_E_INVALID;
+    const EncoderImages im{{kpts0, kpts1}, {side0, side1}, {wx0 - 1.f, wx1 - 1.f}, {wy0 - 1.f, wy1 - 1.f}, {tokens0, tokens1}};
+    const int64_t threads = (tokens0 + tokens1) * 8;
+    const dim3 grid((unsigned)((threads + 255) / 256));
+    if (er0) hipLaunchKernelGGL(encoder_input_kernel<EncoderRagged>, grid, dim3(256), 0, st, im, s, out, *er0, er1 ? *er1 : *er0);
+    else hipLaunchKernelGGL(encoder_input_kernel<EncoderUniform>, grid, dim3(256), 0, st, im, s, out, EncoderUniform{}, EncoderUniform{});
     return og_launch_status();
 }
diff --git a/openglue_amd/csrc/og_common.h b/openglue_amd/csrc/og_common.h
--- a/openglue_amd/csrc/og_common.h
+++ b/openglue_amd/csrc/og_common.h
@@ -187,10 +187,18 @@
     int mx_sv;
 };
 int og_launch_attention(const AttnArgs& a, hipStream_t stream);
+int og_attention_key_split(const AttnArgs& a);
 int og_launch_linear_attention(const AttnArgs& a, hipStream_t stream);
 int og_launch_favor_attention(const AttnArgs& a, hipStream_t stream);
 
-struct RowBest { int* idx; float* val; int stride; };
+struct RowBest { int* idx; float* val; int stride; unsigned long long* col; int cstride; };
+__device__ __forceinline__ unsigned int og_orderable(float v) {
+    const unsigned int b = __float_as_uint(v);
+    return (b & 0x80000000u) ? ~b : (b | 0x80000000u);
+}
+__device__ __forceinline__ unsigned long long og_col_key(float v, int row) {
+    return ((unsigned long long)og_orderable(v) << 32) | (unsigned long long)(0xFFFFFFFFu - (unsigned)row);
+}
 int og_launch_sinkhorn(const float* S, int64_t lds, const float* dustbin_dev , float dustbin_host, int batch, int m, int n, int iters,
                        float reg, float* scores, void* workspace, hipStream_t stream, const RaggedDesc* rag = nullptr,
                        const RowBest* row_best = nullptr, bool trusted_padding = true);
@@ -201,19 +209,27 @@
 bool og_sinkhorn_resident_ragged_wanted(const RaggedDesc& rd, int mode);
 int og_launch_sinkhorn_resident_ragged(const float* S, int64_t lds, const float* zdev, float zhost, const RaggedDesc& rd, int m_max, int n_max, int iters,
                                        float inv_reg, float* u, int ldu, const float* v_in, float* v_out, int ldv, void* xws, unsigned* status,
-                                       hipStream_t st, bool trusted_padding = true, int* count_only = nullptr);
+                                       hipStream_t st, bool trusted_padding = true, int* count_only = nullptr,
+                                       bool first_zeroed = false);
+size_t og_sinkhorn_resident_first_fill_bytes(int B, int m, int n, int cus = 0);
+size_t og_sinkhorn_resident_ragged_first_fill_bytes(const RaggedDesc& rd, int m_max, int n_max);
+static inline size_t og_sinkhorn_resident_ragged_first_fill_bytes(const RaggedNone&, int, int) { return 0; }
 static inline bool og_sinkhorn_resident_ragged_wanted(const RaggedNone&, int) { return false; }
 int og_launch_sinkhorn_resident(const float* S, int64_t lds, const float* zdev, float zhost, int B, int m, int n, int iters,
                                 float inv_reg, float la, float la_bin, float lb, float lb_bin, float* u, int ldu, const float* v_in,
-                                float* v_out, int ldv, void* xws, unsigned* status , hipStream_t st, bool trusted_padding = true);
+                                float* v_out, int ldv, void* xws, unsigned* status , hipStream_t st, bool trusted_padding = true,
+                                bool first_zeroed = false);
 int og_launch_matches(const float* scores, int batch, int m, int n, float thr, int64_t* matches0,
                       float* ms0, int64_t* matches1, float* ms1, void* workspace, hipStream_t stream,
                       const RaggedDesc* rag = nullptr, bool rows_done = false);
 RowBest og_matches_row_best(void* matches_workspace, int batch, int m, int n);
 struct EncoderRagged {
+    static constexpr bool ragged = true;
     int B;
     int off[OG_MAX_RAGGED + 1];
     float wm1[OG_MAX_RAGGED], hm1[OG_MAX_RAGGED];
 };
-int og_launch_encoder_input(const float* kpts, const float* side, int64_t tokens, int s, float wx, float wy,
-                            float* out , hipStream_t stream, const EncoderRagged* er = nullptr);
+struct EncoderUniform { static constexpr bool ragged = false; };
+int og_launch_encoder_input(const float* kpts0, const float* side0, int64_t tokens0, float wx0, float wy0, const float* kpts1, const float* side1,
+                            int64_t tokens1, float wx1, float wy1, int s, float* out, hipStream_t stream, const EncoderRagged* er0 = nullptr,
+                            const EncoderRagged* er1 = nullptr);
diff --git a/openglue_amd/csrc/sinkhorn.hip b/openglue_amd/csrc/sinkhorn.hip
--- a/openglue_amd/csrc/sinkhorn.hip
+++ b/openglue_amd/csrc/sinkhorn.hip
@@ -26,19 +26,32 @@
     int ldu, ldv, ldp, RB;
 };
 
+struct SkOffsets { int64_t duals_bytes, res_off, res_bytes, part_off, total; int ldu, ldv, ldp, RB; };
+static SkOffsets sk_offsets(int B, int m, int n) {
+    SkOffsets o{};
+    o.RB = (m + SK_ROWS - 1) / SK_ROWS;
+    o.ldu = (int)og_round_up(m + 1, 4);
+    o.ldv = (int)og_round_up(n + 1, 4);
+    o.ldp = (int)og_round_up(n, 4);
+    o.duals_bytes = (int64_t)sizeof(float) * ((int64_t)B * (o.ldu + 2 * (int64_t)o.ldv) + 4);
+    o.res_off = og_round_up(o.duals_bytes, 256);
+    o.res_bytes = (int64_t)og_sinkhorn_resident_ws_bytes(B, m, n);
+    o.part_off = o.res_off + og_round_up(o.res_bytes, 256);
+    o.total = o.part_off + og_round_up((int64_t)sizeof(float) * 2 * B * o.RB * o.ldp, 256);
+    return o;
+}
+
 static SinkhornWs sk_layout(void* ws, int B, int m, int n) {
+    const SkOffsets o = sk_offsets(B, m, n);
     SinkhornWs w{};
-    w.RB = (m + SK_ROWS - 1) / SK_ROWS;
-    w.ldu = (int)og_round_up(m + 1, 4);
-    w.ldv = (int)og_round_up(n + 1, 4);
-    w.ldp = (int)og_round_up(n, 4);
+    w.RB = o.RB; w.ldu = o.ldu; w.ldv = o.ldv; w.ldp = o.ldp;
     float* p = (float*)ws;
     w.u = p; p += (int64_t)B * w.ldu;
     w.v[0] = p; p += (int64_t)B * w.ldv;
     w.v[1] = p; p += (int64_t)B * w.ldv;
-    w.flags = (unsigned*)p; p += 4;
-    w.pm = p; p += (int64_t)B * w.RB * w.ldp;
-    w.ps = p;
+    w.flags = (unsigned*)p;
+    w.pm = (float*)((char*)ws + o.part_off);
+    w.ps = w.pm + (int64_t)B * w.RB * w.ldp;
     return w;
 }
 
@@ -245,7 +258,8 @@
                                                                float* __restrict__ v_out, int ldv,
                                                                float* __restrict__ u, int ldu,
                                                                const float* __restrict__ pm,
-                                                               const float* __restrict__ ps, int ldp, int RB, RD rd) {
+                                                               const float* __restrict__ ps, int ldp, int RB, RD rd,
+                                                               unsigned long long* __restrict__ colbest, int ldcb) {
     __shared__ float sm[4];
     const int b = blockIdx.y, tid = threadIdx.x;
     int RBv = RB;
@@ -291,6 +305,7 @@
             cm = mx;
         }
         v_out[(int64_t)b * ldv + j] = lb - (cm + __logf(cs));
+        if (colbest) colbest[(int64_t)b * ldcb + j] = 0ull;
     }
     if ((int)blockIdx.x == N / 256) {
         const float* ub = u + (int64_t)b * ldu;
@@ -522,8 +537,9 @@
     }
 }
 
-template <class RD>
-__global__ __launch_bounds__(256) void sinkhorn_scores_kernel(const float* __restrict__ S, int64_t lds, int M, int N,
+constexpr int SC_WAVES = 8, SC_RPW = 4, SC_SLAB = SC_WAVES * SC_RPW, SC_CPL = 16, SC_CHUNK = 64 * SC_CPL;
+template <class RD, bool BEST>
+__global__ __launch_bounds__(BEST ? 64 * SC_WAVES : 256, BEST ? 4 : 1) void sinkhorn_scores_kernel(const float* __restrict__ S, int64_t lds, int M, int N,
                                                               const float* __restrict__ zdev, float zhost,
                                                               float inv_reg, float norm,
                                                               const float* __restrict__ u, int ldu,
@@ -539,39 +555,99 @@
         so = rd.soff[b];
     }
     S += (int64_t)b * strideS;
-    const int row = blockIdx.x * 4 + (threadIdx.x >> 6);
     const int lane = threadIdx.x & 63;
-    if (row > M) return;
     const float zr = (zdev ? zdev[0] : zhost) * inv_reg;
-    const float ui = u[(int64_t)b * ldu + row];
     const float* vb = v + (int64_t)b * ldv;
-    float* out = scores + so + (int64_t)row * (N + 1);
     float chk = 0.f;
-    if (row < M) {
-        const float* sp = S + (int64_t)row * lds;
-        if (rb.idx) {
-            float best = OG_NEG_INF;
-            int bi = 0x7FFFFFFF;
-            for (int j = lane; j < N; j += 64) {
-                const float val = ((sp[j] * inv_reg + ui) + vb[j]) - norm;
-                out[j] = val;
-                chk = fmaf(val, 0.f, chk);
-                if (val > best || bi == 0x7FFFFFFF) { best = val; bi = j; }
-            }
+    if constexpr (!BEST) {
+        const int row = blockIdx.x * 4 + (threadIdx.x >> 6);
+        if (row > M) return;
+        const float ui = u[(int64_t)b * ldu + row];
+        float* out = scores + so + (int64_t)row * (N + 1);
+        if (row < M) {
+            const float* sp = S + (int64_t)row * lds;
+            for (int j = lane; j < N; j += 64) { const float val = ((sp[j] * inv_reg + ui) + vb[j]) - norm; out[j] = val; chk = fmaf(val, 0.f, chk); }
+        } else {
+            for (int j = lane; j < N; j += 64) { const float val = ((zr + ui) + vb[j]) - norm; out[j] = val; chk = fmaf(val, 0.f, chk); }
+        }
+        if (lane == 0) { const float val = ((zr + ui) + vb[N]) - norm; out[N] = val; chk = fmaf(val, 0.f, chk); }
+    } else {
+        __shared__ unsigned long long ckey[SC_CHUNK];
+        const int tid = threadIdx.x, wave = tid >> 6;
+        if ((int)blockIdx.x * SC_SLAB > M) return;
+        const int row0 = blockIdx.x * SC_SLAB + wave * SC_RPW;
+        constexpr int NONE = 0x7FFFFFFF;
+        float best[SC_RPW];
+        int bi[SC_RPW];
+#pragma unroll
+        for (int r = 0; r < SC_RPW; ++r) { best[r] = OG_NEG_INF; bi[r] = NONE; }
+        for (int t = tid; t < SC_CHUNK; t += 64 * SC_WAVES) ckey[t] = 0ull;
+        __syncthreads();
+        for (int c0 = 0; c0 < N; c0 += SC_CHUNK) {
+            const int jl = c0 + lane;
+            float vv[SC_CPL], cb[SC_CPL];
+            int cr[SC_CPL];
+#pragma unroll
+            for (int k = 0; k < SC_CPL; ++k) { vv[k] = jl + 64 * k < N ? vb[jl + 64 * k] : 0.f; cb[k] = OG_NEG_INF; cr[k] = NONE; }
+#pragma unroll 1
+            for (int r = 0; r < SC_RPW; ++r) {
+                const int row = row0 + r;
+                if (row > M) break;
+                const float ui = u[(int64_t)b * ldu + row];
+                float* out = scores + so + (int64_t)row * (N + 1) + jl;
+                if (row < M) {
+                    const float* sp = S + (int64_t)row * lds + jl;
+                    float sv[SC_CPL];
+#pragma unroll
+                    for (int k = 0; k < SC_CPL; ++k) sv[k] = jl + 64 * k < N ? sp[64 * k] : 0.f;
+                    float rbest = OG_NEG_INF;
+                    int rbi = NONE;
+#pragma unroll
+                    for (int k = 0; k < SC_CPL; ++k) {
+                        if (jl + 64 * k < N) {
+                            const float val = ((sv[k] * inv_reg + ui) + vv[k]) - norm;
+                            out[64 * k] = val;
+                            chk = fmaf(val, 0.f, chk);
+                            if (val > rbest || rbi == NONE) { rbest = val; rbi = jl + 64 * k; }
+                            if (val > cb[k] || cr[k] == NONE) { cb[k] = val; cr[k] = row; }
+                        }
+                    }
+#pragma unroll
+                    for (int q = 0; q < SC_RPW; ++q)
+                        if (q == r && rbi != NONE && (rbest > best[q] || bi[q] == NONE)) { best[q] = rbest; bi[q] = rbi; }
+                } else {
+#pragma unroll
+                    for (int k = 0; k < SC_CPL; ++k)
+                        if (jl + 64 * k < N) { const float val = ((zr + ui) + vv[k]) - norm; out[64 * k] = val; chk = fmaf(val, 0.f, chk); }
+                }
+            }
+#pragma unroll
+            for (int k = 0; k < SC_CPL; ++k)
+                if (cr[k] != NONE) atomicMax(&ckey[lane + 64 * k], og_col_key(cb[k], cr[k]));
+            __syncthreads();
+            for (int t = tid; t < SC_CHUNK; t += 64 * SC_WAVES) {
+                const unsigned long long key = ckey[t];
+                if (key != 0ull) { atomicMax(rb.col + (int64_t)b * rb.cstride + c0 + t, key); ckey[t] = 0ull; }
+            }
+            __syncthreads();
+        }
+#pragma unroll
+        for (int r = 0; r < SC_RPW; ++r) {
+            const int row = row0 + r;
+            if (row > M) break;
+            if (lane == 0) { const float val = ((zr + u[(int64_t)b * ldu + row]) + vb[N]) - norm; scores[so + (int64_t)row * (N + 1) + N] = val; chk = fmaf(val, 0.f, chk); }
+            if (row == M) break;
+            float bv = best[r];
+            int bj = bi[r];
 #pragma unroll
             for (int o = 32; o > 0; o >>= 1) {
-                const float ov = __shfl_xor(best, o, 64);
-                const int oi = __shfl_xor(bi, o, 64);
-                if (ov > best || (ov == best && oi < bi)) { best = ov; bi = oi; }
-            }
-            if (lane == 0) { rb.idx[(int64_t)b * rb.stride + row] = bi; rb.val[(int64_t)b * rb.stride + row] = best; }
-        } else {
-            for (int j = lane; j < N; j += 64) { const float val = ((sp[j] * inv_reg + ui) + vb[j]) - norm; out[j] = val; chk = fmaf(val, 0.f, chk); }
-        }
-    } else {
-        for (int j = lane; j < N; j += 64) { const float val = ((zr + ui) + vb[j]) - norm; out[j] = val; chk = fmaf(val, 0.f, chk); }
-    }
-    if (lane == 0) { const float val = ((zr + ui) + vb[N]) - norm; out[N] = val; chk = fmaf(val, 0.f, chk); }
+                const float ov = __shfl_xor(bv, o, 64);
+                const int oi = __shfl_xor(bj, o, 64);
+                if (ov > bv || (ov == bv && oi < bj)) { bv = ov; bj = oi; }
+            }
+            if (lane == 0) { rb.idx[(int64_t)b * rb.stride + row] = bj; rb.val[(int64_t)b * rb.stride + row] = bv; }
+        }
+    }
     if (nonfinite && __any(chk != chk) && lane == 0) atomicOr(nonfinite, 1u);
 }
 
@@ -689,17 +765,19 @@
 
 extern "C" size_t og_sinkhorn_workspace_bytes(int32_t batch, int32_t m, int32_t n) {
     if (batch <= 0 || m <= 0 || n <= 0 || n > 8192) return 0;
-    const int64_t RB = (m + SK_ROWS - 1) / SK_ROWS;
-    const int64_t ldu = og_round_up(m + 1, 4), ldv = og_round_up(n + 1, 4), ldp = og_round_up(n, 4);
-    const int64_t floats = (int64_t)batch * (ldu + 2 * ldv) + 4 + 2 * (int64_t)batch * RB * ldp;
-    return (size_t)og_round_up(floats * (int64_t)sizeof(float), 256) + og_sinkhorn_resident_ws_bytes(batch, m, n);
-}
-
-static inline void* sk_resident_ws(void* ws, int B, int m, int n) {
-    const int64_t RB = (m + SK_ROWS - 1) / SK_ROWS;
-    const int64_t ldu = og_round_up(m + 1, 4), ldv = og_round_up(n + 1, 4), ldp = og_round_up(n, 4);
-    const int64_t floats = (int64_t)B * (ldu + 2 * ldv) + 4 + 2 * (int64_t)B * RB * ldp;
-    return (char*)ws + og_round_up(floats * (int64_t)sizeof(float), 256);
+    return (size_t)sk_offsets(batch, m, n).total;
+}
+
+static inline void* sk_resident_ws(void* ws, int B, int m, int n) { return (char*)ws + sk_offsets(B, m, n).res_off; }
+
+extern "C" int og_sinkhorn_fill_ranges(int32_t batch, int32_t m, int32_t n, int64_t* out6) {
+    if (!out6 || batch <= 0 || m <= 0 || n <= 0 || n > 8192) return OG_E_INVALID;
+    const SkOffsets o = sk_offsets(batch, m, n);
+    const int64_t first = (int64_t)og_sinkhorn_resident_first_fill_bytes(batch, m, n, 256);
+    out6[0] = 0; out6[1] = o.duals_bytes;
+    out6[2] = first ? o.res_off + 256 : 0; out6[3] = first ? first - 256 : 0;
+    out6[4] = 0; out6[5] = first ? o.res_off + first : o.duals_bytes;
+    return 0;
 }
 
 namespace {
@@ -715,8 +793,6 @@
     const float la = (float)norm, lb = (float)norm;
     const float la_bin = (float)norm + (float)log((double)n);
     const float lb_bin = (float)norm + (float)log((double)m);
-    hipError_t e = hipMemsetAsync(w.u, 0, sizeof(float) * ((size_t)B * (w.ldu + 2 * (size_t)w.ldv) + 4), st);
-    if (e != hipSuccess) return (int)e;
     const SinkhornGeom g = sk_geom(n);
     int cur = 0;
     static const bool robust_only = [] { const char* e = getenv("OG_SINKHORN_ROBUST"); return e && atoi(e) != 0; }();
@@ -733,23 +809,39 @@
     }
     { const char* e = getenv("OG_SK_FAST_ROWS"); if (e && (atoi(e) == 32 || atoi(e) == 64 || atoi(e) == 128)) fast_rows = atoi(e); }
     { const char* e = getenv("OG_SK_FAST_NT"); if (e) fast_nt = atoi(e) != 0; }
+    const char* ft = getenv("OG_SINKHORN_FORCE_TIMEOUT");
+    const bool force_timeout = ft && atoi(ft) != 0;
+    const SkOffsets o = sk_offsets(B, m, n);
+    size_t slot_fill = 0;
+    if (resident && !force_timeout) {
+        if constexpr (std::is_same<RD, RaggedNone>::value) slot_fill = og_sinkhorn_resident_first_fill_bytes(B, m, n);
+        else slot_fill = og_sinkhorn_resident_ragged_first_fill_bytes(rd, m, n);
+        if ((int64_t)slot_fill > o.res_bytes) slot_fill = 0;
+    }
+    hipError_t e = hipMemsetAsync(w.u, 0, slot_fill ? (size_t)o.res_off + slot_fill : (size_t)o.duals_bytes, st);
+    if (e != hipSuccess) return (int)e;
+    unsigned long long* const colbest = row_best ? row_best->col : nullptr;
+    const int ldcb = row_best ? row_best->cstride : 0;
+    if (colbest && iters == 0) {
+        e = hipMemsetAsync(colbest, 0, sizeof(unsigned long long) * (size_t)B * ldcb, st);
+        if (e != hipSuccess) return (int)e;
+    }
     for (int it = 0; it < iters; ++it) {
         const float* vin = w.v[cur];
         if (it > 0 && resident) {
             unsigned* status = w.flags + 1;
             void* xws = sk_resident_ws(workspace, B, m, n);
-            const char* ft = getenv("OG_SINKHORN_FORCE_TIMEOUT");
-            if (ft && atoi(ft) != 0) {
+            if (force_timeout) {
                 e = hipMemsetAsync(status, 1, sizeof(unsigned), st);
                 if (e != hipSuccess) return (int)e;
             } else {
                 int rc;
                 if constexpr (std::is_same<RD, RaggedNone>::value)
                     rc = og_launch_sinkhorn_resident(S, lds, zdev, dustbin, B, m, n, iters - 1, inv_reg, la, la_bin, lb, lb_bin, w.u, w.ldu, w.v[cur],
-                                                     w.v[cur ^ 1], w.ldv, xws, status, st, trusted_padding);
+                                                     w.v[cur ^ 1], w.ldv, xws, status, st, trusted_padding, slot_fill != 0);
                 else
                     rc = og_launch_sinkhorn_resident_ragged(S, lds, zdev, dustbin, rd, m, n, iters - 1, inv_reg, w.u, w.ldu, w.v[cur], w.v[cur ^ 1],
-                                                            w.ldv, xws, status, st, trusted_padding);
+                                                            w.ldv, xws, status, st, trusted_padding, nullptr, slot_fill != 0);
                 if (rc) return rc;
             }
             cur ^= 1;
@@ -778,11 +870,17 @@
         else if (g.WPR == 2) launch_sweep<4, 2, 2>(S, lds, B, m, n, zdev, dustbin, inv_reg, la, vin, w, st, rd);
         else launch_sweep<4, 2, 4>(S, lds, B, m, n, zdev, dustbin, inv_reg, la, vin, w, st, rd);
         hipLaunchKernelGGL(sinkhorn_combine_kernel<RD>, dim3((n + 1 + 255) / 256, B), dim3(256), 0, st, m, n, zdev, dustbin, inv_reg, la_bin,
-                           lb, lb_bin, w.v[cur], w.v[cur ^ 1], w.ldv, w.u, w.ldu, w.pm, w.ps, w.ldp, w.RB, rd);
+                           lb, lb_bin, w.v[cur], w.v[cur ^ 1], w.ldv, w.u, w.ldu, w.pm, w.ps, w.ldp, w.RB, rd, it == 0 ? colbest : nullptr, ldcb);
         cur ^= 1;
     }
-    hipLaunchKernelGGL(sinkhorn_scores_kernel<RD>, dim3((m + 1 + 3) / 4, B), dim3(256), 0, st, S, lds, m, n, zdev, dustbin, inv_reg,
-                       (float)norm, w.u, w.ldu, w.v[cur], w.ldv, scores, (int64_t)m * lds, rd, row_best ? *row_best : RowBest{nullptr, nullptr, 0}, w.flags);
+    if (row_best) {
+        if (!row_best->idx || !row_best->val || !row_best->col) return OG_E_INVALID;
+        hipLaunchKernelGGL((sinkhorn_scores_kernel<RD, true>), dim3((m + 1 + SC_SLAB - 1) / SC_SLAB, B), dim3(64 * SC_WAVES), 0, st, S, lds, m, n, zdev, dustbin,
+                           inv_reg, (float)norm, w.u, w.ldu, w.v[cur], w.ldv, scores, (int64_t)m * lds, rd, *row_best, w.flags);
+    } else {
+        hipLaunchKernelGGL((sinkhorn_scores_kernel<RD, false>), dim3((m + 1 + 3) / 4, B), dim3(256), 0, st, S, lds, m, n, zdev, dustbin, inv_reg,
+                           (float)norm, w.u, w.ldu, w.v[cur], w.ldv, scores, (int64_t)m * lds, rd, RowBest{}, w.flags);
+    }
     return og_launch_status();
 }
 }
@@ -810,11 +908,11 @@
         else if (g.WPR == 2) launch_sweep<4, 2, 2>(S, lds, B, m, n, dustbin_dev, dustbin, inv_reg, la, vin, w, st, rd);
         else launch_sweep<4, 2, 4>(S, lds, B, m, n, dustbin_dev, dustbin, inv_reg, la, vin, w, st, rd);
         hipLaunchKernelGGL(sinkhorn_combine_kernel<RaggedNone>, dim3((n + 1 + 255) / 256, B), dim3(256), 0, st, m, n, dustbin_dev, dustbin,
-                           inv_reg, la_bin, lb, lb_bin, vin, vout, w.ldv, w.u, w.ldu, w.pm, w.ps, w.ldp, w.RB, rd);
-    }
-    hipLaunchKernelGGL(sinkhorn_scores_kernel<RaggedNone>, dim3((m + 1 + 3) / 4, B), dim3(256), 0, st, S, lds, m, n, dustbin_dev, dustbin,
+                           inv_reg, la_bin, lb, lb_bin, vin, vout, w.ldv, w.u, w.ldu, w.pm, w.ps, w.ldp, w.RB, rd, (unsigned long long*)nullptr, 0);
+    }
+    hipLaunchKernelGGL((sinkhorn_scores_kernel<RaggedNone, false>), dim3((m + 1 + 3) / 4, B), dim3(256), 0, st, S, lds, m, n, dustbin_dev, dustbin,
                        inv_reg, (float)norm, U + (size_t)(iters - 1) * B * w.ldu, w.ldu, V + (size_t)iters * B * w.ldv, w.ldv, scores,
-                       (int64_t)m * lds, rd, RowBest{nullptr, nullptr, 0}, (unsigned*)nullptr);
+                       (int64_t)m * lds, rd, RowBest{}, (unsigned*)nullptr);
     return og_launch_status();
 }
 
@@ -879,3 +977,16 @@
     og_clear_status();
     return og_launch_sinkhorn(S, lds, nullptr, dustbin, batch, m, n, iters, reg, scores, workspace_dev, (hipStream_t)stream, nullptr, nullptr, false);
 }
+
+extern "C" int og_sinkhorn_matches(const float* S, int64_t lds, float dustbin, int32_t batch, int32_t m, int32_t n, int32_t iters, float reg,
+                                   float match_threshold, float* scores, int64_t* matches0, float* matching_scores0, int64_t* matches1,
+                                   float* matching_scores1, void* sinkhorn_workspace_dev, void* matches_workspace_dev, void* stream) {
+    og_clear_status();
+    if (!matches0 || !matching_scores0 || !matches_workspace_dev || batch <= 0 || m <= 0 || n <= 0) return OG_E_INVALID;
+    if ((uintptr_t)matches_workspace_dev & 15) return OG_E_ALIGN;
+    const RowBest rb = og_matches_row_best(matches_workspace_dev, batch, m, n);
+    if (int rc = og_launch_sinkhorn(S, lds, nullptr, dustbin, batch, m, n, iters, reg, scores, sinkhorn_workspace_dev, (hipStream_t)stream, nullptr, &rb, false))
+        return rc;
+    return og_launch_matches(scores, batch, m, n, match_threshold, matches0, matching_scores0, matches1, matching_scores1, matches_workspace_dev,
+                             (hipStream_t)stream, nullptr, true);
+}
diff --git a/openglue_amd/csrc/sinkhorn_resident.hip b/openglue_amd/csrc/sinkhorn_resident.hip
--- a/openglue_amd/csrc/sinkhorn_resident.hip
+++ b/openglue_amd/csrc/sinkhorn_resident.hip
@@ -816,15 +816,34 @@
     return (int64_t)B * m * n >= (int64_t)1 << 18;
 }
 
+namespace {
+struct RsRounds { RsGeom q; int rw, per; };
+RsRounds rs_uniform_rounds(int B, int m, int n, int cus) {
+    RsRounds r{};
+    r.rw = rs_rows_per_wave(B, m, n, cus);
+    r.q = rs_geom(m, n, r.rw);
+    const int ppr = rs_pairs_per_round(r.q, cus);
+    if (ppr <= 0) return r;
+    const int rounds = (B + ppr - 1) / ppr;
+    r.per = (B + rounds - 1) / rounds;
+    return r;
+}
+}
+
+size_t og_sinkhorn_resident_first_fill_bytes(int B, int m, int n, int cus) {
+    if (!og_sinkhorn_resident_shape_ok(B, m, n)) return 0;
+    const RsRounds r = rs_uniform_rounds(B, m, n, cus > 0 ? cus : rs_num_cus());
+    return r.per > 0 ? rs_area_bytes(r.q.W, r.per * r.q.G, r.per * r.q.X) : 0;
+}
+
 int og_launch_sinkhorn_resident(const float* S, int64_t lds, const float* zdev, float zhost, int B, int m, int n, int iters,
                                 float inv_reg, float la, float la_bin, float lb, float lb_bin, float* u, int ldu, const float* v_in,
-                                float* v_out, int ldv, void* xws, unsigned* status, hipStream_t st, bool trusted_padding) {
+                                float* v_out, int ldv, void* xws, unsigned* status, hipStream_t st, bool trusted_padding, bool first_zeroed) {
     if (!S || !u || !v_in || !v_out || !xws || !status || iters < 1 || !og_sinkhorn_resident_shape_ok(B, m, n)) return OG_E_INVALID;
-    const int rw = rs_rows_per_wave(B, m, n, rs_num_cus());
-    const RsGeom q = rs_geom(m, n, rw);
-    const int ppr = rs_pairs_per_round(q, rs_num_cus());
-    if (ppr <= 0) return OG_E_SHAPE;
-    const int rounds = (B + ppr - 1) / ppr, per = (B + rounds - 1) / rounds;
+    const RsRounds rr = rs_uniform_rounds(B, m, n, rs_num_cus());
+    const int rw = rr.rw, per = rr.per;
+    const RsGeom q = rr.q;
+    if (per <= 0) return OG_E_SHAPE;
     hipError_t e = hipSuccess;
     SkResArgs a{};
     a.S = S; a.lds = lds; a.strideS = (int64_t)m * lds;
@@ -843,8 +862,10 @@
         a.b0 = b0; a.npairs = np; a.slots = np * q.G; a.groups = np * q.X;
         a.xb = a.xa + (size_t)2 * a.slots * NCX * 8;
         a.xc = a.xb + (size_t)2 * a.groups * NCX * 8;
-        e = hipMemsetAsync(a.xcc, 0, RS_MAXWG * sizeof(unsigned) + (size_t)2 * a.slots * NCX * 8 + (size_t)2 * a.groups * NCX * 8 + (size_t)2 * a.groups * 32 * RS_RREC * 8, st);
-        if (e != hipSuccess) return (int)e;
+        if (b0 > 0 || !first_zeroed) {
+            e = hipMemsetAsync(a.xcc, 0, rs_area_bytes(q.W, a.slots, a.groups) - 256, st);
+            if (e != hipSuccess) return (int)e;
+        }
         RsUniform map{q.G, q.Gx, q.X, 0};
         int grid = np * q.G;
         a.local_ok = 0;
@@ -945,9 +966,19 @@
     return 0;
 }
 
+size_t og_sinkhorn_resident_ragged_first_fill_bytes(const RaggedDesc& rd, int m_max, int n_max) {
+    RsPlanPair pp[OG_MAX_RAGGED];
+    if (!rs_ragged_plan(rd, pp, rs_num_cus())) return 0;
+    size_t first = 0;
+    rs_ragged_for_each_launch(rd, pp, [&](int W, const RsRagged&, int np, int slots, int) {
+        if (first == 0) first = rs_ragged_launch_bytes(W, slots, np);
+    });
+    return first <= og_sinkhorn_resident_ws_bytes(rd.B, m_max, n_max) ? first : 0;
+}
+
 int og_launch_sinkhorn_resident_ragged(const float* S, int64_t lds, const float* zdev, float zhost, const RaggedDesc& rd, int m_max, int n_max, int iters,
                                        float inv_reg, float* u, int ldu, const float* v_in, float* v_out, int ldv, void* xws, unsigned* status,
-                                       hipStream_t st, bool trusted_padding, int* count_only) {
+                                       hipStream_t st, bool trusted_padding, int* count_only, bool first_zeroed) {
     if (!count_only && (!S || !u || !v_in || !v_out || !xws || !status || iters < 1)) return OG_E_INVALID;
     RsPlanPair pp[OG_MAX_RAGGED];
     if (!rs_ragged_plan(rd, pp, rs_num_cus())) return OG_E_SHAPE;
@@ -973,8 +1004,11 @@
         a.b0 = 0; a.npairs = np; a.slots = slots; a.groups = np;
         a.xb = a.xa + (size_t)2 * a.slots * NCX * 8;
         a.xc = a.xb + (size_t)2 * a.groups * NCX * 8;
-        const hipError_t e = hipMemsetAsync(a.xcc, 0, rs_ragged_launch_bytes(W, slots, np) - 256, st);
-        if (e != hipSuccess) { rc = (int)e; return; }
+        if (!first_zeroed) {
+            const hipError_t e = hipMemsetAsync(a.xcc, 0, rs_ragged_launch_bytes(W, slots, np) - 256, st);
+            if (e != hipSuccess) { rc = (int)e; return; }
+        }
+        first_zeroed = false;
         const int grid = 8 * qmax;
         if (W == 1) rs_launch<1>(a, map, grid, st);
         else if (W == 2) rs_launch<2>(a, map, grid, st);
diff --git a/openglue_amd/ops.py b/openglue_amd/ops.py
--- a/openglue_amd/ops.py
+++ b/openglue_amd/ops.py
@@ -171,6 +171,27 @@
     return out
 
 
+def sinkhorn_matches(S: torch.Tensor, dustbin: float, iters: int, match_threshold: float, reg: float = 1.0) -> Dict[str, torch.Tensor]:
+    lib = _lib.load()
+    S = _lib.gpu_tensor(S, "S")
+    B, m, n = S.shape
+    lds = (n + 3) // 4 * 4
+    if lds != n:
+        Sp = torch.zeros(B, m, lds, device=S.device, dtype=torch.float32)
+        Sp[:, :, :n] = S
+        S = Sp
+    dev = S.device
+    ws = torch.empty(lib.og_sinkhorn_workspace_bytes(B, m, n), device=dev, dtype=torch.uint8)
+    mws = torch.empty(lib.og_matches_workspace_bytes(B, m, n), device=dev, dtype=torch.uint8)
+    out = {"scores": torch.empty(B, m + 1, n + 1, device=dev, dtype=torch.float32),
+           "matches0": torch.empty(B, m, device=dev, dtype=torch.int64), "matching_scores0": torch.empty(B, m, device=dev, dtype=torch.float32),
+           "matches1": torch.empty(B, n, device=dev, dtype=torch.int64), "matching_scores1": torch.empty(B, n, device=dev, dtype=torch.float32)}
+    _lib.call("og_sinkhorn_matches", dev, S.data_ptr(), lds, float(dustbin), B, m, n, int(iters), float(reg), float(match_threshold),
+              out["scores"].data_ptr(), out["matches0"].data_ptr(), out["matching_scores0"].data_ptr(), out["matches1"].data_ptr(),
+              out["matching_scores1"].data_ptr(), ws.data_ptr(), mws.data_ptr(), _lib.STREAM)
+    return out
+
+
 def extract_matches(scores: torch.Tensor, match_threshold: float, both_sides: bool = True) -> Dict[str, torch.Tensor]:
     lib = _lib.load()
     scores = _lib.gpu_tensor(scores, "scores")
```

Measured after the change: 3560 image-pairs/s (median of 3 runs). No clear change (+0.1%).
